# Luckick/EAGCN

Hardware: AMD Instinct MI355X
Metric: molecules/sec fwd+bwd, 2-layer 5-view EAGCN, Tox21 batch (higher is better)
Workload: dtype f32 (bf16x3 split, fp32 accumulate): every fp32 operand leaves its producer as three bf16 planes, six v_mfma_f32_32x32x16_bf16 piece products per 16 k rebuild the fp32 product (csrc/gemm_bx3.hip); aggregation, BatchNorm, head, first layer fp32

## Files before the change

### eagcn_amd/_lib.py

```python
import ctypes as C
import os

_HERE = os.path.dirname(os.path.abspath(__file__))
LIB_PATH = os.path.join(_HERE, 'lib', 'libeagcn_hip.so')

MAX_VIEWS = 8
MAX_SEGS = 8
META_WORDS = 16
META_NLOG = 8
META_T, META_NMAX, META_NTILES, META_BAD_ADJ, META_BAD_REL, META_NEDGE, META_OVERFLOW, META_EDGE_OVERFLOW = range(8)
META_NBLK = 9
STRUCT_CONCATE, STRUCT_WEIGHTED = 0, 1

_fp = C.c_void_p


class Batch(C.Structure):
    _fields_ = [('B', C.c_int32), ('N', C.c_int32), ('K', C.c_int32), ('ldc', C.c_int32),
                ('T', C.c_int32), ('n_max', C.c_int32), ('n_tiles', C.c_int32),
                ('channels', C.c_int32 * MAX_VIEWS),
                ('code', _fp), ('deg_bn', _fp), ('nat', _fp), ('row0', _fp), ('tile0', _fp),
                ('meta', _fp), ('row_mol', _fp), ('row_loc', _fp), ('row_m', _fp), ('row_deg', _fp),
                ('tile_mol', _fp), ('row_info', _fp), ('tile_info', _fp),
                ('rel_vec', _fp * MAX_VIEWS), ('rel_c', C.c_int32 * MAX_VIEWS),
# ... 63 lines not shown

class HeadParams(C.Structure):
    _fields_ = [('f_in', C.c_int32), ('n_den1', C.c_int32), ('n_den2', C.c_int32), ('nclass', C.c_int32),
                ('dropout', C.c_float), ('bn_eps', C.c_float), ('bn_momentum', C.c_float),
                ('den1_w', _fp), ('den2_w', _fp), ('den3_w', _fp),
                ('gbn_w', _fp), ('gbn_b', _fp), ('gbn_rm', _fp), ('gbn_rv', _fp),
                ('bn1_w', _fp), ('bn1_b', _fp), ('bn1_rm', _fp), ('bn1_rv', _fp),
                ('bn2_w', _fp), ('bn2_b', _fp), ('bn2_rm', _fp), ('bn2_rv', _fp)]


class HeadGrads(C.Structure):
    _fields_ = [(n, _fp) for n in ('d_den1_w', 'd_den2_w', 'd_den3_w', 'd_gbn_w', 'd_gbn_b', 'd_bn1_w', 'd_bn1_b',
                                   'd_bn2_w', 'd_bn2_b')]


class Model(C.Structure):
    _fields_ = [('n_layers', C.c_int32), ('molfp_mode', C.c_int32), ('training', C.c_int32),
                ('head_seed', C.c_uint64), ('head_seed_dev', _fp), ('input_packed', C.c_int32), ('aux_stream', _fp),
                ('layer', LayerParams * 4), ('head', HeadParams), ('stats_hook', _fp), ('stats_user', _fp),
                ('stats_world', C.c_int32), ('fuse_readout', C.c_int32), ('fwd_signal', _fp), ('wait_flag', _fp), ('start_signal', _fp)]


class StepLoss(C.Structure):
    _fields_ = [('kind', C.c_int32), ('labels', _fp), ('class_weight', _fp), ('loss', _fp), ('scale', _fp), ('dout', _fp)]


ALLREDUCE_FN = C.CFUNCTYPE(C.c_int, C.c_void_p, C.c_int, C.c_void_p, C.c_void_p)


SIGNATURES = {
    'eagcn_abi_version': (C.c_int, []),
    'eagcn_struct_size': (C.c_size_t, [C.c_int]),
    'eagcn_last_error': (C.c_char_p, []),
    'eagcn_pad16': (C.c_int, [C.c_int]),
    'eagcn_layer_out_ld': (C.c_int, [C.POINTER(LayerParams)]),
    'eagcn_layer_fp': (C.c_int, [C.POINTER(LayerParams)]),
    'eagcn_layer_packed_bytes': (C.c_size_t, [C.POINTER(Batch), C.POINTER(LayerParams)]),
    'eagcn_layer_fwd_scratch_bytes': (C.c_size_t, [C.POINTER(Batch), C.POINTER(LayerParams)]),
    'eagcn_layer_bwd_scratch_bytes': (C.c_size_t, [C.POINTER(Batch), C.POINTER(LayerParams)]),
    'eagcn_index_build': (C.c_int, [_fp, C.POINTER(_fp), C.POINTER(Batch), _fp, _fp]),
    'eagcn_index_from_bonds': (C.c_int, [_fp, _fp, _fp, _fp, C.c_int64, C.POINTER(Batch), _fp, _fp]),
    'eagcn_index_rows': (C.c_int, [C.POINTER(Batch), _fp]),
    'eagcn_set_gemm_mode': (C.c_int, [C.c_int]),
    'eagcn_stream_wait_counter': (C.c_int, [_fp, C.c_uint32, _fp]),
    'eagcn_stream_signal_flag': (C.c_int, [_fp, _fp]),
    'eagcn_stream_wait_flag': (C.c_int, [_fp, C.c_double, _fp]),
    'eagcn_stream_wait_timeouts': (C.c_int, []),
    'eagcn_stream_wait_reset': (None, []),
    'eagcn_adam_step': (C.c_int, [_fp, _fp, _fp, _fp, C.c_int64, _fp, _fp, _fp, _fp]),
    'eagcn_agg_wants_bond_lists': (C.c_int, [C.c_int, C.c_int]),
    'eagcn_agg_wants_bond_lists_for': (C.c_int, [C.c_int, C.c_int, C.c_int]),
    'eagcn_bx3_used_splits': (C.c_int, [C.c_int, C.c_int, C.c_int, C.c_int]),
    'eagcn_set_bx3_wide': (C.c_int, [C.c_int]),
    'eagcn_bx3_pair_used_splits': (C.c_int, [C.c_int] * 7),
    'eagcn_bx3_plane_elems': (C.c_size_t, [C.c_int, C.c_int]),
    'eagcn_bx3_split': (C.c_int, [_fp, C.c_int, C.c_int, _fp, C.c_size_t, C.c_int, C.c_int, _fp]),
    'eagcn_gemm_bx3': (C.c_int, [C.c_int, C.c_int, C.c_int, C.c_int, _fp, C.c_size_t, C.c_int, C.c_int, _fp, C.c_size_t, C.c_int, C.c_int,
                                 _fp, C.c_int, C.c_int, C.c_size_t, C.c_int, _fp]),
    'eagcn_gemm_bx3_pair': (C.c_int, [C.c_int, C.c_int, C.c_int, _fp, C.c_size_t, C.c_int, C.c_int, _fp, C.c_size_t, C.c_int, C.c_int, _fp, C.c_int,
                                      C.c_int, C.c_int, C.c_int, _fp, C.c_size_t, C.c_int, C.c_int, _fp, C.c_size_t, C.c_int, C.c_int, _fp, C.c_int,
                                      C.c_int, C.c_size_t, C.c_int, _fp]),
    'eagcn_pack_rows': (C.c_int, [C.POINTER(Batch), _fp, C.c_int, C.POINTER(Layout), _fp, _fp]),
    'eagcn_unpack_rows': (C.c_int, [C.POINTER(Batch), _fp, C.POINTER(Layout), _fp, _fp, C.c_int, _fp]),
    'eagcn_pad_rows': (C.c_int, [_fp, _fp, C.c_int, C.c_int, C.c_int, _fp, _fp]),
    'eagcn_gat_scratch_bytes': (C.c_size_t, [C.POINTER(Batch), C.c_int]),
    'eagcn_gat_forward': (C.c_int, [C.POINTER(Batch), C.POINTER(GatParams), _fp, _fp, _fp, _fp, _fp]),
    'eagcn_gat_backward': (C.c_int, [C.POINTER(Batch), C.POINTER(GatParams), _fp, _fp, _fp, _fp, _fp, _fp, _fp, _fp, _fp,
                                     C.c_size_t, _fp]),
    'eagcn_pool_scratch_bytes': (C.c_size_t, []),
    'eagcn_pool_attention_forward': (C.c_int, [C.POINTER(Batch), C.POINTER(PoolAtt), _fp, C.c_int, _fp, _fp, _fp]),
    'eagcn_pool_attention_backward': (C.c_int, [C.POINTER(Batch), C.POINTER(PoolAtt), _fp, C.c_int, _fp, _fp, _fp, C.c_size_t,
                                                _fp]),
    'eagcn_pool_mix_forward': (C.c_int, [C.POINTER(Batch), C.POINTER(Layout), _fp, C.c_int, _fp, _fp, _fp, _fp, C.c_int, _fp]),
    'eagcn_pool_mix_backward': (C.c_int, [C.POINTER(Batch), C.POINTER(Layout), _fp, C.c_int, _fp, _fp, _fp, _fp, C.c_int, _fp,
                                          _fp, _fp, _fp]),
    'eagcn_pool_reduce_forward': (C.c_int, [C.POINTER(Batch), _fp, C.c_int, C.c_int, C.c_int, _fp, _fp, _fp, _fp]),
    'eagcn_pool_reduce_backward': (C.c_int, [C.POINTER(Batch), _fp, C.c_int, C.c_int, C.c_int, _fp, _fp, _fp, _fp, _fp]),
    'eagcn_layer_forward': (C.c_int, [C.POINTER(Batch), C.POINTER(LayerParams), C.POINTER(LayerBufs), _fp]),
    'eagcn_layer_backward': (C.c_int, [C.POINTER(Batch), C.POINTER(LayerParams), C.POINTER(LayerBufs),
                                       _fp, _fp, _fp, C.POINTER(LayerGrads), _fp]),
    'eagcn_attention_dense': (C.c_int, [C.POINTER(Batch), C.POINTER(LayerParams), _fp, _fp]),
    'eagcn_readout_forward': (C.c_int, [C.POINTER(Batch), _fp, C.POINTER(Layout), _fp, _fp, C.c_int, _fp,
                                        C.c_int, _fp]),
    'eagcn_readout_backward': (C.c_int, [C.POINTER(Batch), _fp, C.POINTER(Layout), _fp, C.c_int, C.c_int,
                                         _fp, _fp, _fp]),
    'eagcn_gemm_f32': (C.c_int, [C.c_int, C.c_int, C.c_int, C.c_int, C.c_int, _fp, C.c_int, _fp, C.c_int,
                                 _fp, C.c_int, _fp]),
    'eagcn_gemm_f32_dev': (C.c_int, [C.c_int, C.c_int, C.c_int, C.c_int, C.c_int, _fp, C.c_int, _fp, C.c_int,
                                     _fp, C.c_int, _fp, C.c_int, _fp]),
    'eagcn_gemm_sk_workspace_bytes': (C.c_size_t, []),
    'eagcn_gemm_f32_sk': (C.c_int, [C.c_int, C.c_int, C.c_int, C.c_int, C.c_int, _fp, C.c_int, _fp, C.c_int,
                                    _fp, C.c_int, _fp, C.c_size_t, _fp]),
    'eagcn_gemm_pair_sk': (C.c_int, [C.c_int, C.c_int, C.c_int, _fp, C.c_int, _fp, C.c_int, _fp, C.c_int,
                                     C.c_int, C.c_int, C.c_int, _fp, C.c_int, _fp, C.c_int, _fp, C.c_int,
                                     _fp, C.c_size_t, _fp]),
    'eagcn_gemm_pair_sk_slabs': (C.c_int, [C.c_int, C.c_int, C.c_int, _fp, C.c_int, _fp, C.c_int, _fp, C.c_int,
                                           C.c_int, C.c_int, C.c_int, _fp, C.c_int, _fp, C.c_int, _fp, C.c_int,
                                           C.c_size_t, _fp, C.c_size_t, _fp]),
    'eagcn_gemm_sk_plan': (C.c_int, [C.c_int] * 7 + [C.POINTER(C.c_int), C.POINTER(C.c_int)]),
    'eagcn_gemm_sk_timeouts': (C.c_int, []),
    'eagcn_gemm_sk_failed': (C.c_int, []),
    'eagcn_gemm_sk_reset_failed': (None, []),
    'eagcn_gemm_sk_inject_failure': (None, []),
    'eagcn_model_saved_bytes': (C.c_size_t, [C.POINTER(Batch), C.POINTER(Model)]),
    'eagcn_model_scratch_bytes': (C.c_size_t, [C.POINTER(Batch), C.POINTER(Model)]),
    'eagcn_model_atom_rep': (C.c_int, [C.POINTER(Batch), C.POINTER(Model), C.POINTER(C.c_size_t),
# ... 95 lines not shown
```

### eagcn_amd/csrc/gemm.hip

```cpp
#include <stdlib.h>

#include <algorithm>

#include "common.h"
#include "gemm_x6.h"

namespace eagcn {

constexpr int gemm_lds_floats(int BM, int BN, int BK, bool a_kc, bool b_kc) {
    return 2 * ((a_kc ? BM * (BK + 2) : BK * (BM + 16)) + (b_kc ? BN * (BK + 2) : BK * (BN + 16)));
}

template <int BM, int BN, int BK, bool A_KC, bool B_KC, int D, bool EXT_LDS = false>
__device__ __forceinline__ void gemm_tile(const GemmDesc& g, const int Mx, const int Kx, const int tile_x,
                                          const int tile_y, const int z, const int nsp, float* shared = nullptr) {
    constexpr int WM = BM / 2, WN = BN / 2;
    constexpr int MR = WM / 16, NR = WN / 16;
    constexpr int LDA_S = A_KC ? (BK + 2) : (BM + 16);
    constexpr int LDB_S = B_KC ? (BK + 2) : (BN + 16);
    constexpr int A_SZ = A_KC ? BM * LDA_S : BK * LDA_S;
    constexpr int B_SZ = B_KC ? BN * LDB_S : BK * LDB_S;
    constexpr int A_TPR = A_KC ? BK / 4 : BM / 4;
    constexpr int A_RPP = 256 / A_TPR;
    constexpr int A_PASS = (A_KC ? BM : BK) / A_RPP;
    constexpr int B_TPR = B_KC ? BK / 4 : BN / 4;
    constexpr int B_RPP = 256 / B_TPR;
    constexpr int B_PASS = (B_KC ? BN : BK) / B_RPP;
    static_assert(A_PASS >= 1 && B_PASS >= 1, "tile too small for 256 threads");

    float* smem;
    if constexpr (EXT_LDS) {
        smem = shared;
    } else {
        __shared__ __attribute__((aligned(16))) float own_smem[2 * (A_SZ + B_SZ)];
        smem = own_smem;
    }
    auto kc_row = [](int x) -> int {
        if constexpr (BK == 16) {
            const int g = x >> 2, rs = x & 3;
            return ((g >> 2) << 4) + ((g & 3) << 1) + (rs & 1) + ((rs >> 1) << 3);
        } else {
            return x;
        }
    };
    auto As = [&](int buf) -> float* { return smem + buf * (A_SZ + B_SZ); };
    auto Bs = [&](int buf) -> float* { return smem + buf * (A_SZ + B_SZ) + A_SZ; };

    const int tid = threadIdx.x, lane = tid & 63, wave = tid >> 6;
    const int li = lane & 15, q = lane >> 4;
    const int wm = (wave >> 1) * WM, wn = (wave & 1) * WN;
    const int m0 = tile_y * BM, n0 = tile_x * BN;
    const int kchunk = ((Kx + nsp - 1) / nsp + BK - 1) / BK * BK;
    const int kbeg = z * kchunk;
    const int kend = min(Kx, kbeg + kchunk);
    float* C = g.C + (size_t)z * g.slab;

    float4 ra_[D][A_PASS], rb_[D][B_PASS];
    auto load_tiles = [&](int k0, float4 (&ra)[A_PASS], float4 (&rb)[B_PASS]) {
// ... 161 lines not shown
    {
        const int gx = gridDim.x;
        const int per_z = gx * ((Mx + BM - 1) / BM);
        const int nwg = per_z * nsp;
        if (blockIdx.y * gx + blockIdx.x >= per_z || (int)blockIdx.z >= nsp) return;
        const int lin = blockIdx.z * per_z + blockIdx.y * gx + blockIdx.x;
        const int nid = xcd_remap(lin, nwg);
        z = nid / per_z;
        const int rem = nid - z * per_z;
        tile_y = rem / gx;
        tile_x = rem - tile_y * gx;
    }
    if constexpr (X6 != 0) {
        constexpr int NP = X6 == 2 ? 1 : 3;
        __shared__ __attribute__((aligned(16))) unsigned char x6_smem[x6_lds_bytes(BM, BN, NP)];
        gemm_tile_x6<A_KC, B_KC, BM, BN, NP>(g, Mx, Kx, tile_x, tile_y, z, nsp, x6_smem);
    }
    else gemm_tile<BM, BN, BK, A_KC, B_KC, D>(g, Mx, Kx, tile_x, tile_y, z, nsp);
}

template <int BM, int BN, int BK, int D, int X6 = 0>
__global__ __launch_bounds__(256) void gemm_f32_pair_kernel(GemmDesc g0, GemmDesc g1, int first1) {
    constexpr int F32_LDS = gemm_lds_floats(BM, BN, BK, true, true) > gemm_lds_floats(BM, BN, BK, false, false)
                                ? gemm_lds_floats(BM, BN, BK, true, true) : gemm_lds_floats(BM, BN, BK, false, false);
    constexpr int NP = X6 == 2 ? 1 : 3;
    __shared__ __attribute__((aligned(16))) unsigned char x6_smem[X6 ? x6_lds_bytes(64, 64, NP) : F32_LDS * 4];
    float* f32_smem = reinterpret_cast<float*>(x6_smem);
    const int b = blockIdx.x;
    if (b < first1) {
        const int Mx = g0.M_dev ? min(*g0.M_dev, g0.M) : g0.M;
        const int gx = (g0.N + BN - 1) / BN;
        const int nreal = gx * ((Mx + BM - 1) / BM);
        if (b >= nreal) return;
        const int nid = xcd_remap(b, nreal);
        const int ty = nid / gx;
        if constexpr (X6 != 0) gemm_tile_x6<true, true, 64, 64, NP>(g0, Mx, g0.K, nid - ty * gx, ty, 0, 1, x6_smem);
        else gemm_tile<BM, BN, BK, true, true, D, true>(g0, Mx, g0.K, nid - ty * gx, ty, 0, 1, f32_smem);
    } else {
        const int lin = b - first1;
        const int Kx = g1.K_dev ? min(*g1.K_dev, g1.K) : g1.K;
        const int gx = (g1.N + BN - 1) / BN;
        const int per_z = gx * ((g1.M + BM - 1) / BM);
        const int nsp = eff_splits(g1, Kx);
        const int nwg = per_z * nsp;
        if (lin >= nwg) return;
        const int nid = xcd_remap(lin, nwg);
        const int z = nid / per_z, rem = nid - z * per_z;
        const int ty = rem / gx;
        if constexpr (X6 != 0) gemm_tile_x6<false, false, 64, 64, NP>(g1, g1.M, Kx, rem - ty * gx, ty, z, nsp, x6_smem);
        else gemm_tile<BM, BN, BK, false, false, D, true>(g1, g1.M, Kx, rem - ty * gx, ty, z, nsp, f32_smem);
    }
}


template <int BM, int BN, int BK, int D>
static int launch_cfg(const GemmDesc& g, hipStream_t s) {
    dim3 grid(cdiv(g.N, BN), cdiv(g.M, BM), g.splits);
    ProfScope ps(g.prof_tag, s, g.work > 0.0 ? g.work : 2.0 * g.M * g.N * g.K);
    if (g.ta == 0 && g.tb == 0) gemm_f32_kernel<BM, BN, BK, true, false, D><<<grid, 256, 0, s>>>(g);
    else if (g.ta == 0 && g.tb == 1) gemm_f32_kernel<BM, BN, BK, true, true, D><<<grid, 256, 0, s>>>(g);
    else if (g.ta == 1 && g.tb == 0) gemm_f32_kernel<BM, BN, BK, false, false, D><<<grid, 256, 0, s>>>(g);
    else gemm_f32_kernel<BM, BN, BK, false, true, D><<<grid, 256, 0, s>>>(g);
    EAGCN_LAUNCH_CHECK();
    return EAGCN_OK;
}

static int g_gemm_x6 = [] { const char* e = getenv("EAGCN_GEMM_X6"); return e ? atoi(e) : 3; }();
static int use_x6(const GemmDesc& g) { return ((g_gemm_x6 == 1 || g_gemm_x6 == 2) && g.K >= 64 && g.prof_tag != PROF_HEAD) ? g_gemm_x6 : 0; }
int gemm_mode() { return g_gemm_x6; }
template <int BM, int BN, int X6>
static int launch_x6_cfg(const GemmDesc& g, hipStream_t s) {
    dim3 grid(cdiv(g.N, BN), cdiv(g.M, BM), g.splits);
    ProfScope ps(g.prof_tag, s, g.work > 0.0 ? g.work : 2.0 * g.M * g.N * g.K);
    if (g.ta == 0 && g.tb == 0) gemm_f32_kernel<BM, BN, 16, true, false, 4, X6><<<grid, 256, 0, s>>>(g);
    else if (g.ta == 0 && g.tb == 1) gemm_f32_kernel<BM, BN, 16, true, true, 4, X6><<<grid, 256, 0, s>>>(g);
    else if (g.ta == 1 && g.tb == 0) gemm_f32_kernel<BM, BN, 16, false, false, 4, X6><<<grid, 256, 0, s>>>(g);
    else gemm_f32_kernel<BM, BN, 16, false, true, 4, X6><<<grid, 256, 0, s>>>(g);
    EAGCN_LAUNCH_CHECK();
    return EAGCN_OK;
}
static int launch_x6(const GemmDesc& g, hipStream_t s, int mode) {
    if (mode == 2) return launch_x6_cfg<64, 64, 2>(g, s);
    static const int tile = [] { const char* e = getenv("EAGCN_X6_TILE"); return e ? atoi(e) : 0; }();
    if (tile == 2 && g.M > 64 && g.N > 64) return launch_x6_cfg<128, 128, 1>(g, s);
    if (tile >= 1 && g.M > 64) return launch_x6_cfg<128, 64, 1>(g, s);
    return launch_x6_cfg<64, 64, 1>(g, s);
}

int launch_gemm(const GemmDesc& g0, hipStream_t s) {
    if (g0.M <= 0 || g0.N <= 0) return EAGCN_OK;
    EAGCN_CHECK_ARG(g0.splits >= 1, "gemm: splits must be >= 1");
    GemmDesc g = g0;
    g.vecA = (g.lda % 4) == 0 && ((g.ta ? g.M : g.K) % 4) == 0 && (reinterpret_cast<uintptr_t>(g.A) % 16) == 0;
    g.vecB = (g.ldb % 4) == 0 && ((g.tb ? g.K : g.N) % 4) == 0 && (reinterpret_cast<uintptr_t>(g.B) % 16) == 0;
    if (g.splits > 1) EAGCN_CHECK_ARG(g.vecA && g.vecB, "gemm: split-K needs float4-aligned operands");
    static const int forced = [] { const char* e = getenv("EAGCN_GEMM_CFG"); return e ? atoi(e) : -1; }();
    int cfg = forced;
    if (cfg < 0 && use_x6(g)) return launch_x6(g, s, use_x6(g));
    if (cfg < 0) {
        const long tiles128 = (long)cdiv(g.M, 128) * cdiv(g.N, 128) * g.splits;
        cfg = (g.K >= 1024 && tiles128 >= 512 && g.M > 64 && g.N > 64) ? 3 : 0;
    }
    switch (cfg) {
        case 1: return launch_cfg<64, 64, 32, 3>(g, s);
        case 2: return launch_cfg<64, 64, 16, 2>(g, s);
        case 3: return launch_cfg<128, 128, 16, 3>(g, s);
        case 4: return launch_cfg<64, 64, 16, 6>(g, s);
        case 5: return launch_cfg<64, 64, 16, 1>(g, s);
        default: return launch_cfg<64, 64, 16, 4>(g, s);
    }
}

int launch_gemm_pair(const GemmDesc& dx, const GemmDesc& dw, hipStream_t s) {
    GemmDesc g0 = dx, g1 = dw;
    g0.vecA = (g0.lda % 4) == 0 && (g0.K % 4) == 0 && (reinterpret_cast<uintptr_t>(g0.A) % 16) == 0;
    g0.vecB = (g0.ldb % 4) == 0 && (g0.K % 4) == 0 && (reinterpret_cast<uintptr_t>(g0.B) % 16) == 0;
    g1.vecA = (g1.lda % 4) == 0 && (g1.M % 4) == 0 && (reinterpret_cast<uintptr_t>(g1.A) % 16) == 0;
    g1.vecB = (g1.ldb % 4) == 0 && (g1.N % 4) == 0 && (reinterpret_cast<uintptr_t>(g1.B) % 16) == 0;
    const bool ok = g0.ta == 0 && g0.tb == 1 && g0.splits == 1 && !g0.K_dev && g1.ta == 1 && g1.tb == 0 && !g1.M_dev &&
                    (g1.splits == 1 || (g1.vecA && g1.vecB)) && g0.M > 0 && g0.N > 0 && g1.M > 0 && g1.N > 0;
    if (!ok) {
        int rc = launch_gemm(dw, s);
        return rc ? rc : launch_gemm(dx, s);
    }
    const int first1 = (cdiv(g0.M, 64) * cdiv(g0.N, 64) + 7) / 8 * 8;
    const int n1 = cdiv(g1.M, 64) * cdiv(g1.N, 64) * g1.splits;
    const double w0 = g0.work > 0.0 ? g0.work : 2.0 * g0.M * g0.N * g0.K;
    const double w1 = g1.work > 0.0 ? g1.work : 2.0 * g1.M * g1.N * g1.K;
    ProfScope ps(PROF_GEMM_PAIR, s, w0 + w1);
    if (use_x6(g0) == 2 && use_x6(g1) == 2) gemm_f32_pair_kernel<64, 64, 16, 4, 2><<<first1 + n1, 256, 0, s>>>(g0, g1, first1);
    else if (use_x6(g0) && use_x6(g1)) gemm_f32_pair_kernel<64, 64, 16, 4, 1><<<first1 + n1, 256, 0, s>>>(g0, g1, first1);
    else gemm_f32_pair_kernel<64, 64, 16, 4><<<first1 + n1, 256, 0, s>>>(g0, g1, first1);
    EAGCN_LAUNCH_CHECK();
    return EAGCN_OK;
}

}

using namespace eagcn;

extern "C" int eagcn_set_gemm_mode(int mode) {
    const int old = eagcn::g_gemm_x6;
    eagcn::g_gemm_x6 = mode;
    return old;
}

extern "C" int eagcn_gemm_f32(int ta, int tb, int M, int N, int K, const float* A, int lda, const float* B,
                              int ldb, float* C, int ldc, void* stream) {
    EAGCN_CHECK_ARG(A && B && C, "eagcn_gemm_f32: null operand");
    GemmDesc g{ta, tb, M, N, K, A, lda, B, ldb, C, ldc, 1, 0};
    return launch_gemm(g, (hipStream_t)stream);
}

extern "C" int eagcn_gemm_f32_dev(int ta, int tb, int M, int N, int K, const float* A, int lda, const float* B,
                                  int ldb, float* C, int ldc, const int32_t* extent_dev, int which, void* stream) {
    EAGCN_CHECK_ARG(A && B && C && extent_dev && (which == 0 || which == 2), "eagcn_gemm_f32_dev: bad argument");
    GemmDesc g{ta, tb, M, N, K, A, lda, B, ldb, C, ldc, 1, 0};
    if (which == 0) g.M_dev = extent_dev; else g.K_dev = extent_dev;
    return launch_gemm(g, (hipStream_t)stream);
}
```

### eagcn_amd/csrc/head.hip

```cpp
#include <stdlib.h>

#include <algorithm>

#include "common.h"
#include "kernels.h"

namespace eagcn {

__global__ void wait_counter_kernel(const uint32_t* __restrict__ word, uint32_t value, int* __restrict__ err,
                                    unsigned long long budget_ticks) {
    if (threadIdx.x == 0) {
        const unsigned long long t0 = wall_clock64();
        while ((int32_t)(__hip_atomic_load(word, __ATOMIC_ACQUIRE, __HIP_MEMORY_SCOPE_AGENT) - value) < 0) {
            __builtin_amdgcn_s_sleep(64);
            if (wall_clock64() - t0 > budget_ticks) {
                if (err) __hip_atomic_store(err, 1, __ATOMIC_RELAXED, __HIP_MEMORY_SCOPE_SYSTEM);
                break;
            }
        }
    }
}



// ... 66 lines not shown

static size_t carve_saved(void* base, const eagcn_batch* b, const eagcn_model* m, ModelSaved* out) {
    Carver2 c(base);
    ModelSaved s;
    const size_t T = (size_t)b->T;
    s.x0 = c.take<float>(T * layout_ld(&m->layer[0].in));
    for (int l = 0; l < m->n_layers; ++l) {
        const eagcn_layer_params* p = &m->layer[l];
        LayerSaved& L = s.L[l];
        L.fp = eagcn_layer_fp(p);
        L.ldo = eagcn_layer_out_ld(p);
        L.ld_in = layout_ld(&p->in);
        L.P = c.take<float>(T * L.fp);
        L.Y = c.take<float>(T * L.fp);
        L.rscale = c.take<float>((size_t)p->K * T);
        L.bn = c.take<float>((size_t)4 * L.fp);
        if (l == m->n_layers - 1) s.xout_last_off = c.off;
        L.xout = c.take<float>(T * L.ldo);
        if (l == m->n_layers - 1) s.pad_last_off = c.off;
        L.pad_row = c.take<float>(L.ldo);
        L.packed_bytes = eagcn_layer_packed_bytes(b, p);
        L.packed = c.take<char>(L.packed_bytes);
        const int np = (l + 1 < m->n_layers && L.ldo >= 128 && (L.ldo & 15) == 0) ? gemm_planes() : 0;
        L.xout_planes = np ? c.take<uint16_t>((size_t)np * bx_plane_elems(T, L.ldo)) : nullptr;
    }
    const eagcn_head_params* h = &m->head;
    const size_t B = (size_t)b->B;
    s.g = c.take<float>(B * h->f_in);
    s.h1 = c.take<float>(B * h->n_den1);
    s.h2 = c.take<float>(B * h->n_den2);
    s.bn_g = c.take<float>((size_t)4 * h->f_in);
    s.bn_1 = c.take<float>((size_t)4 * h->n_den1);
    s.bn_2 = c.take<float>((size_t)4 * h->n_den2);
    {
        const eagcn_layer_params* last = &m->layer[m->n_layers - 1];
        const size_t ldo = (size_t)eagcn_layer_out_ld(last);
        const bool need = last->structure == EAGCN_STRUCT_WEIGHTED;
        s.pad_cnt = c.take<uint16_t>(need ? B * last->K * ldo : 1);
        s.padc = c.take<float>(need ? B * ldo : 1);
        const size_t nt = (size_t)(b->N + 1) * (b->N + 1);
        s.pad_tab = c.take<uint32_t>(need ? nt : 1);
    }
    if (out) *out = s;
    return c.off;
}

struct ModelScratch {
    float *da2, *da1, *dgn, *dg, *dxa, *dxb, *dpad;
    float* hdw; int hdw_ks;
    double* hst; int n_hst;
    double* hws;
    double* hsb;
    void* layer; size_t layer_bytes;
};
static size_t carve_scratch(void* base, const eagcn_batch* b, const eagcn_model* m, ModelScratch* out) {
    Carver2 c(base);
    ModelScratch s;
    const eagcn_head_params* h = &m->head;
    const size_t B = (size_t)b->B, T = (size_t)b->T;
    s.n_hst = 2 * (h->f_in + h->n_den1 + h->n_den2) + 6;
    s.hst = c.take<double>((size_t)(HEAD_COPIES + 1) * s.n_hst + HEAD_WS);
    s.hsb = s.hst + (size_t)HEAD_COPIES * s.n_hst;
    s.hws = s.hsb + s.n_hst;
    s.da2 = c.take<float>(B * h->n_den2);
    s.da1 = c.take<float>(B * h->n_den1);
    s.dgn = c.take<float>(B * h->f_in);
    s.dg = c.take<float>(B * h->f_in);
    s.hdw_ks = head_dw_chunks(b->B);
    s.hdw = c.take<float>(s.hdw_ks > 1 ? (size_t)s.hdw_ks * ((size_t)h->f_in * h->n_den1 + (size_t)h->n_den1 * h->n_den2 +
                                                             (size_t)h->n_den2 * h->nclass) : 1);
    int ldmax = 0;
    size_t lbytes = 0;
    for (int l = 0; l < m->n_layers; ++l) {
        ldmax = std::max(ldmax, eagcn_layer_out_ld(&m->layer[l]));
        lbytes = std::max(lbytes, eagcn_layer_fwd_scratch_bytes(b, &m->layer[l]));
        lbytes = std::max(lbytes, eagcn_layer_bwd_scratch_bytes(b, &m->layer[l]));
    }
    s.dxa = c.take<float>(T * ldmax);
    s.dxb = c.take<float>(T * ldmax);
    s.dpad = c.take<float>((size_t)EAGCN_MAX_VIEWS * ldmax);
    s.layer_bytes = lbytes;
    s.layer = c.take<char>(lbytes);
    if (out) *out = s;
    return c.off;
}

static int check_model(const eagcn_batch* b, const eagcn_model* m, const char* who) {
    EAGCN_CHECK_ARG(b && m, "%s: null argument", who);
    EAGCN_CHECK_ARG(m->n_layers >= 1 && m->n_layers <= 4, "%s: n_layers=%d", who, m->n_layers);
    const eagcn_head_params* h = &m->head;
    EAGCN_CHECK_ARG(h->f_in >= 1 && h->n_den1 >= 1 && h->n_den2 >= 1 && h->nclass >= 1, "%s: bad head sizes", who);
    EAGCN_CHECK_ARG(h->den1_w && h->den2_w && h->den3_w && h->gbn_w && h->gbn_b && h->gbn_rm && h->gbn_rv &&
                        h->bn1_w && h->bn1_b && h->bn1_rm && h->bn1_rv && h->bn2_w && h->bn2_b && h->bn2_rm &&
                        h->bn2_rv, "%s: null head parameter", who);
    const eagcn_layer_params* last = &m->layer[m->n_layers - 1];
    const int f_last = last->structure == EAGCN_STRUCT_CONCATE ? [&] { int s = 0; for (int k = 0; k < last->K; ++k) s += last->width[k]; return s; }()
                                                                 : last->width[0];
    EAGCN_CHECK_ARG(f_last == h->f_in, "%s: head expects %d features, last layer yields %d", who, h->f_in, f_last);
    EAGCN_CHECK_ARG(!m->training || b->B > 1, "%s: BatchNorm in training mode needs more than one molecule", who);
    return EAGCN_OK;
}

static eagcn_layout out_layout(const eagcn_layer_params* p) {
    eagcn_layout l;
    memset(&l, 0, sizeof(l));
    if (p->structure == EAGCN_STRUCT_CONCATE) {
        l.nseg = p->K;
        for (int k = 0; k < p->K; ++k) { l.width[k] = p->width[k]; l.pad[k] = pad16(p->width[k]); }
    } else {
        l.nseg = 1;
        l.width[0] = p->width[0];
        l.pad[0] = pad16(p->width[0]);
    }
    return l;
}

static bool fused_readout(const eagcn_model* m) {
    static const bool env = [] { const char* v = getenv("EAGCN_NO_FUSED_READOUT"); return !(v && v[0] == '1'); }();
    return env && m->fuse_readout && m->layer[m->n_layers - 1].structure == EAGCN_STRUCT_CONCATE;
}

static bool hidden_planes_only(const eagcn_batch* b, const eagcn_model* m, const ModelSaved& sv, int l) {
    return l + 1 < m->n_layers && sv.L[l].xout_planes && layer_reads_planes_only(b, &m->layer[l + 1], m->aux_stream != nullptr);
}

static void fill_drop(float p, int training, int* do_drop, uint32_t* thr, float* inv_keep) {
    *do_drop = (training && p > 0.0f) ? 1 : 0;
    *thr = (uint32_t)std::min(4294967295.0, (double)p * 4294967296.0);
    *inv_keep = 1.0f / (1.0f - p);
}

}

using namespace eagcn;

// ... 74 lines not shown
    if (!hg) return P;
    const double *cn_g = sc.hst + 2 * F, *cn_1 = sc.hst + 2 * F + 2 + 2 * n1, *cn_2 = sc.hst + 2 * (F + n1) + 4 + 2 * n2;
    const float gscale = P.sync && m->stats_world > 1 ? 1.0f / (float)m->stats_world : 1.0f;
    P.b3 = HeadBwd{B, n2, nc, sv.h2, sv.bn_2, 1, nodrop, h->den3_w, dout, nullptr, nullptr, nullptr, nullptr, nullptr, nullptr,
                   sc.da2, P.sb_2, hg->d_den3_w, m->training};
    P.b2 = HeadBwd{B, n1, n2, sv.h1, sv.bn_1, 1, drop1, h->den2_w, sc.da2, sv.h2, sv.bn_2, P.sb_2, dgraph_rep, hg->d_bn2_w, hg->d_bn2_b,
                   sc.da1, P.sb_1, hg->d_den2_w, m->training};
    P.b1 = HeadBwd{B, F, n1, sv.g, sv.bn_g, 0, nodrop, h->den1_w, sc.da1, sv.h1, sv.bn_1, P.sb_1, nullptr, hg->d_bn1_w, hg->d_bn1_b,
                   sc.dgn, P.sb_g, hg->d_den1_w, m->training};
    if (P.sync) { P.b2.cnt_y = cn_2; P.b2.gscale = gscale; P.b1.cnt_y = cn_1; P.b1.gscale = gscale; }
    P.b3.nw = 8;
    const int ks = sc.hdw_ks;
    float* part3 = sc.hdw;
    float* part2 = part3 + (size_t)ks * n2 * nc;
    float* part1 = part2 + (size_t)ks * n1 * n2;
    if (ks > 1) {
        P.b3.ks = ks; P.b3.dW_part = part3;
        P.b2.ks = ks; P.b2.dW_part = part2;
        P.b1.ks = ks; P.b1.dW_part = part1;
    }
    P.bg = HeadGbn{B, F, sc.dgn, sv.g, sv.bn_g, P.sb_g, sc.dg, hg->d_gbn_w, hg->d_gbn_b, m->training};
    if (P.sync) { P.bg.cnt = cn_g; P.bg.gscale = gscale; }
    if (ks > 1) {
        P.bg.sum[0] = HeadDwSum{hg->d_den3_w, part3, n2 * nc, ks};
        P.bg.sum[1] = HeadDwSum{hg->d_den2_w, part2, n1 * n2, ks};
        P.bg.sum[2] = HeadDwSum{hg->d_den1_w, part1, F * n1, ks};
        P.bg.nsum = 3;
    }
    return P;
}

static int model_forward_trunk(const eagcn_batch* b, const eagcn_model* m, const float* afm, const int64_t* size, void* saved,
                               size_t saved_bytes, void* scratch, size_t scratch_bytes, ModelSaved& sv, ModelScratch& sc,
                               void* stream, const char* who) {
    hipStream_t s = (hipStream_t)stream;
    RC(check_model(b, m, who));
    EAGCN_CHECK_GEMM3(who);
    EAGCN_CHECK_ARG((afm || m->input_packed) && saved && scratch, "%s: null buffer", who);
    EAGCN_CHECK_ARG(m->molfp_mode == 0 || size, "%s: 'ave' read-out needs size", who);
    EAGCN_CHECK_ARG(carve_saved(saved, b, m, &sv) <= saved_bytes, "%s: saved block too small", who);
    EAGCN_CHECK_ARG(carve_scratch(scratch, b, m, &sc) <= scratch_bytes, "%s: scratch too small", who);
    const eagcn_head_params* h = &m->head;
    HandOff ho{m->start_signal, m->wait_flag, wait_err_word(), 200000000ull};
    if (!m->input_packed && (m->wait_flag || m->start_signal)) {
        handoff_kernel<<<1, 64, 0, s>>>(ho);
        EAGCN_LAUNCH_CHECK();
        ho.start = nullptr; ho.flag = nullptr;
    }
    ZeroJob zj;
    RC(gemm3_zero_job(sc.layer, sc.layer_bytes, sc.hst, (HEAD_COPIES + 1) * sc.n_hst + HEAD_WS, &zj));
    if (!m->input_packed)
        RC(eagcn_pack_rows(b, afm, layout_width(&m->layer[0].in), &m->layer[0].in, sv.x0, stream));
    const float* x = sv.x0;
    {
        const eagcn_layer_params* ps[4];
        void* pk[4];
        size_t pkb[4];
        for (int l = 0; l < m->n_layers; ++l) { ps[l] = &m->layer[l]; pk[l] = sv.L[l].packed; pkb[l] = sv.L[l].packed_bytes; }
        RC(pack_params_all(b, ps, pk, pkb, m->n_layers, stream, &zj, &ho));
    }
    for (int l = 0; l < m->n_layers; ++l) {
        LayerSaved& L = sv.L[l];
        eagcn_layer_bufs w;
        memset(&w, 0, sizeof(w));
        w.x = x; w.P = L.P; w.Y = L.Y; w.rscale = L.rscale; w.bn = L.bn; w.xout = L.xout; w.pad_row = L.pad_row;
        w.scratch = sc.layer; w.scratch_bytes = sc.layer_bytes; w.packed = L.packed; w.packed_bytes = L.packed_bytes;
        w.stats_hook = m->stats_hook; w.stats_user = m->stats_user;
        w.x_planes = l > 0 ? sv.L[l - 1].xout_planes : nullptr; w.xout_planes = L.xout_planes;
        const bool po = hidden_planes_only(b, m, sv, l);
        RC(layer_forward_impl(b, &m->layer[l], &w, stream, true, l == m->n_layers - 1 && fused_readout(m), po));
        x = po ? nullptr : L.xout;
    }
    const eagcn_layer_params* last = &m->layer[m->n_layers - 1];
    const LayerSaved& LL = sv.L[m->n_layers - 1];
    const eagcn_layout lay = out_layout(last);
    const int B = b->B, F = h->f_in, n1 = h->n_den1, n2 = h->n_den2;
    double *st_g = sc.hst, *st_1 = sc.hst + 2 * F + 2, *st_2 = sc.hst + 2 * (F + n1) + 4;
    const int copies = (m->stats_hook && m->training) ? 1 : HEAD_COPIES;
    if (fused_readout(m)) {
        ReadoutBn rb;
        rb.Y = LL.Y; rb.ldy = LL.fp; rb.bn = LL.bn; rb.fp = LL.fp;
        fill_drop(last->dropout, last->training, &rb.do_drop, &rb.thr, &rb.inv_keep);
        rb.seed = last->seed; rb.seed_dev = last->seed_dev;
        rb.size = size; rb.mode = m->molfp_mode; rb.g = sv.g; rb.F = F; rb.st = st_g;
        rb.cnt0 = st_g + 2 * F; rb.cnt1 = st_1 + 2 * n1; rb.cnt2 = st_2 + 2 * n2;
        rb.st_copies = copies; rb.st_stride = sc.n_hst;
        RC(readout_bn_forward(b, &lay, rb, stream));
    } else if (pad_sampled(m))
        RC(readout_forward_sampled(b, LL.xout, &lay, last, LL.bn + (size_t)LL.fp , size,
                                   m->molfp_mode, sv.g, F, sv.pad_cnt, sv.padc, sv.pad_tab, stream));
    else
        RC(eagcn_readout_forward(b, LL.xout, &lay, last->structure == EAGCN_STRUCT_WEIGHTED ? LL.pad_row : nullptr,
                                 size, m->molfp_mode, sv.g, F, stream));
    if (!fused_readout(m)) RC(head_colstats(sv.g, B, F, st_g, s, st_g + 2 * F, st_1 + 2 * n1, st_2 + 2 * n2));
    return EAGCN_OK;
}

static int stats_hook_call(const eagcn_model* m, bool sync, double* buf, int n, void* stream) {
    if (!sync) return EAGCN_OK;
    if (m->stats_hook(buf, n, stream, m->stats_user)) {
        set_error("eagcn_model: the sync-BatchNorm all-reduce hook failed");
        return EAGCN_ERR_HIP;
    }
    return EAGCN_OK;
}

static int head_forward_launches(const eagcn_model* m, const HeadPlan& P, void* stream) {
    hipStream_t s = (hipStream_t)stream;
    const eagcn_head_params* h = &m->head;
    RC(stats_hook_call(m, P.sync, P.st_g, 2 * h->f_in + 1, stream));
    RC(head_fwd(P.f1, s));
    RC(stats_hook_call(m, P.sync, P.st_1, 2 * h->n_den1 + 1, stream));
    RC(head_fwd(P.f2, s));
    RC(stats_hook_call(m, P.sync, P.st_2, 2 * h->n_den2 + 1, stream));
    RC(head_fwd(P.f3, s));
    return EAGCN_OK;
}
static int head_backward_launches(const eagcn_model* m, const HeadPlan& P, void* stream) {
    hipStream_t s = (hipStream_t)stream;
    const eagcn_head_params* h = &m->head;
    RC(head_bwd(P.b3, s));
    RC(stats_hook_call(m, P.sync, P.sb_2, 2 * h->n_den2, stream));
    RC(head_bwd(P.b2, s));
// ... 173 lines not shown
        else RC(eagcn_mse_loss(out, loss->labels, b->B * h->nclass, loss->loss, loss->dout, stream));
        if (loss->scale) {
            const int n = b->B * h->nclass;
            scale_loss_kernel<<<cdiv(n, 256), 256, 0, s>>>(loss->loss, loss->dout, n, loss->scale);
            EAGCN_LAUNCH_CHECK();
        }
        RC(head_backward_launches(m, P, stream));
    }
    return readout_pad_backward(b, m, size, sv, sc, stream);
}

extern "C" int eagcn_model_backward(const eagcn_batch* b, const eagcn_model* m, const int64_t* size, void* saved,
                                    size_t saved_bytes, void* scratch, size_t scratch_bytes, const float* dout,
                                    const float* dgraph_rep, const eagcn_layer_grads* lg,
                                    const eagcn_head_grads* hg, void* stream) {
    EAGCN_CHECK_ARG(m, "eagcn_model_backward: null model");
    return eagcn_model_backward_range(b, m, size, saved, saved_bytes, scratch, scratch_bytes, dout, dgraph_rep, lg, hg, 1,
                                      m->n_layers - 1, 0, stream);
}

static int model_backward_impl(const eagcn_batch* b, const eagcn_model* m, const int64_t* size, void* saved, size_t saved_bytes,
                               void* scratch, size_t scratch_bytes, const float* dout, const float* dgraph_rep,
                               const eagcn_layer_grads* lg, const eagcn_head_grads* hg, int with_head, int layer_hi, int layer_lo,
                               float* dx0, bool input_only, void* stream) {
    hipStream_t s = (hipStream_t)stream;
    EAGCN_CHECK_ARG(saved && scratch && dout && (lg || input_only) && hg, "eagcn_model_backward: null buffer");
    EAGCN_CHECK_ARG(hg->d_den1_w && hg->d_den2_w && hg->d_den3_w && hg->d_gbn_w && hg->d_gbn_b && hg->d_bn1_w &&
                        hg->d_bn1_b && hg->d_bn2_w && hg->d_bn2_b, "eagcn_model_backward: null head gradient");
    EAGCN_CHECK_ARG(layer_hi < m->n_layers && layer_lo >= 0 && layer_lo <= layer_hi + 1,
                    "eagcn_model_backward_range: layers %d..%d of %d", layer_hi, layer_lo, m->n_layers);
    EAGCN_CHECK_ARG(!with_head || layer_hi == m->n_layers - 1 || layer_hi < layer_lo,
                    "eagcn_model_backward_range: the head's backward is followed by the top layer");
    ModelSaved sv;
    ModelScratch sc;
    EAGCN_CHECK_ARG(carve_saved(saved, b, m, &sv) <= saved_bytes, "eagcn_model_backward: saved block too small");
    EAGCN_CHECK_ARG(carve_scratch(scratch, b, m, &sc) <= scratch_bytes, "eagcn_model_backward: scratch too small");
    const int F = m->head.f_in;
    const ZeroJob zb{nullptr, 0, sc.hsb, sc.n_hst};
    hipStream_t side = m->aux_stream ? (hipStream_t)m->aux_stream : s;
    const bool forked = side != s;
    const eagcn_layer_params* last = &m->layer[m->n_layers - 1];
    const eagcn_layout lay = out_layout(last);
    const bool weighted = last->structure == EAGCN_STRUCT_WEIGHTED;
    const bool sampled = pad_sampled(m);
    if (with_head) {
        const HeadPlan P = head_plan(b, m, sv, sc, nullptr, nullptr, dout, dgraph_rep, hg);
        RC(head_backward_launches(m, P, stream));
        if (!(input_only && !m->training)) RC(readout_pad_backward(b, m, size, sv, sc, stream));
    }
    ReadoutGrad rgd;
    memset(&rgd, 0, sizeof(rgd));
    rgd.dg = sc.dg; rgd.F = F; rgd.size = size; rgd.mode = m->molfp_mode; rgd.map = make_colmap(&lay);
    const int top_l = m->n_layers - 1;
    EdgeDrain pend_in, pend_out;
    pend_in.eacc = nullptr;
    pend_out.eacc = nullptr;
    for (int l = layer_hi; l >= layer_lo; --l) {
        const int t = top_l - l;
        float* cur = (t & 1) ? sc.dxb : sc.dxa;
        float* other = (t & 1) ? sc.dxa : sc.dxb;
        LayerSaved& L = sv.L[l];
        eagcn_layer_bufs w;
        memset(&w, 0, sizeof(w));
        w.x = l == 0 ? sv.x0 : (hidden_planes_only(b, m, sv, l - 1) ? nullptr : sv.L[l - 1].xout);
        w.P = L.P; w.Y = L.Y; w.rscale = L.rscale; w.bn = L.bn; w.xout = L.xout; w.pad_row = L.pad_row;
        w.scratch = sc.layer; w.scratch_bytes = sc.layer_bytes; w.packed = L.packed; w.packed_bytes = L.packed_bytes;
        w.aux_stream = m->aux_stream;
        w.stats_hook = m->stats_hook; w.stats_user = m->stats_user;
        w.x_planes = l > 0 ? sv.L[l - 1].xout_planes : nullptr;
        const bool top = l == top_l;
        const float* dpad = (weighted && top) ? sc.dpad : nullptr;
        RC(layer_backward_impl(b, &m->layer[l], &w, top ? nullptr : cur, top ? &rgd : nullptr, dpad,
                               l > 0 ? other : dx0, input_only ? nullptr : &lg[l], stream, top && sampled, top ? &zb : nullptr,
                               pend_in.eacc ? &pend_in : nullptr, (l > layer_lo && !input_only) ? &pend_out : nullptr, input_only));
        pend_in = pend_out;
        if (l == layer_lo) pend_in.eacc = nullptr;
    }
    if (forked) RC(stream_after(s, side));
    return EAGCN_OK;
}

extern "C" int eagcn_model_backward_range(const eagcn_batch* b, const eagcn_model* m, const int64_t* size, void* saved,
                                          size_t saved_bytes, void* scratch, size_t scratch_bytes, const float* dout,
                                          const float* dgraph_rep, const eagcn_layer_grads* lg,
                                          const eagcn_head_grads* hg, int with_head, int layer_hi, int layer_lo, void* stream) {
    RC(check_model(b, m, "eagcn_model_backward"));
    EAGCN_CHECK_GEMM3("eagcn_model_backward");
    return model_backward_impl(b, m, size, saved, saved_bytes, scratch, scratch_bytes, dout, dgraph_rep, lg, hg, with_head, layer_hi,
                               layer_lo, nullptr, false, stream);
}

struct InputScratch { float* dx0; eagcn_head_grads hg; };
static size_t carve_input_scratch(void* base, const eagcn_batch* b, const eagcn_model* m, InputScratch* out) {
    Carver2 c(base);
    c.off = carve_scratch(nullptr, b, m, nullptr);
    InputScratch t;
    const eagcn_head_params* h = &m->head;
    const size_t F = h->f_in, n1 = h->n_den1, n2 = h->n_den2, nc = h->nclass;
    t.dx0 = c.take<float>((size_t)std::max(b->T, 1) * layout_ld(&m->layer[0].in));
    t.hg.d_den1_w = c.take<float>(F * n1);
    t.hg.d_den2_w = c.take<float>(n1 * n2);
    t.hg.d_den3_w = c.take<float>(n2 * nc);
    t.hg.d_gbn_w = c.take<float>(F);
    t.hg.d_gbn_b = c.take<float>(F);
    t.hg.d_bn1_w = c.take<float>(n1);
    t.hg.d_bn1_b = c.take<float>(n1);
    t.hg.d_bn2_w = c.take<float>(n2);
    t.hg.d_bn2_b = c.take<float>(n2);
    if (out) *out = t;
    return c.off;
}

static int check_engine_model(const eagcn_batch* b, const eagcn_model* m, const char* who) {
    RC(check_model(b, m, who));
    EAGCN_CHECK_ARG(m->molfp_mode == 0 || m->molfp_mode == 1, "%s: read-out mode %d has no engine path", who, m->molfp_mode);
    for (int l = 0; l < m->n_layers; ++l)
        EAGCN_CHECK_ARG(m->layer[l].structure == EAGCN_STRUCT_CONCATE || m->layer[l].structure == EAGCN_STRUCT_WEIGHTED,
                        "%s: layer %d has structure %d, which the engine does not run", who, l, m->layer[l].structure);
    return EAGCN_OK;
}

int eagcn::model_backward_input_packed(const eagcn_batch* b, const eagcn_model* m, const int64_t* size, void* saved, size_t saved_bytes,
                                       void* scratch, size_t scratch_bytes, const float* dout, const float* dgraph_rep,
                                       const eagcn_layer_grads* lg, const eagcn_head_grads* hg, float** dx0, void* stream,
                                       const char* who) {
    EAGCN_CHECK_ARG(b && m, "%s: null argument", who);
    EAGCN_CHECK_ARG((lg == nullptr) == (hg == nullptr), "%s: lg and hg are both given (full backward) or both NULL (input-only)", who);
// ... 57 lines not shown
```

### eagcn_amd/csrc/index.hip

```cpp
#include <algorithm>

#include <stdlib.h>

#include "common.h"
#include "kernels.h"

namespace eagcn {

struct RelPtrs {
    const float* p[EAGCN_MAX_VIEWS];
    int c[EAGCN_MAX_VIEWS];
};

template <int NIT, int RPW>
__global__ __launch_bounds__(256) void index_scan_kernel(const float* __restrict__ adj, RelPtrs rel,
                                                          int B, int N, int Ncap, int K, int ldc,
                                                          uint8_t* __restrict__ code,
                                                          int32_t* __restrict__ deg_bn,
                                                          int32_t* __restrict__ nat,
                                                          int32_t* __restrict__ ecnt,
                                                          int32_t* __restrict__ meta) {
    const int lane = threadIdx.x & 63;
    const long row_first = ((long)blockIdx.x * 4 + (threadIdx.x >> 6)) * RPW;
    const long nrows = (long)B * N;
// ... 566 lines not shown
            __syncthreads();
        }
        int run = s_scan[tid] - tot;
        __syncthreads();
#pragma unroll
        for (int u = 0; u < 4; ++u) {
            const int i = tid * 4 + u;
            if (i < n) {
                int* ptr = (pass ? bt.col_ptr : bt.row_ptr) + (size_t)(r0 + i) * 2;
                const bool fits = e0 + run + v[u] <= bt.E;
                ptr[0] = e0 + run;
                ptr[1] = fits ? v[u] : 0;
                cnt[i] = fits ? e0 + run : -1;
                run += v[u];
            }
        }
        __syncthreads();
    }
    auto codes = [&](int i, int j) -> uint64_t {
        uint8_t c[EAGCN_MAX_VIEWS];
#pragma unroll
        for (int k = 0; k < EAGCN_MAX_VIEWS; ++k) c[k] = k < bt.K ? code0[k * plane + (size_t)i * bt.ldc + j] : 0;
        uint64_t c64 = 0;
#pragma unroll
        for (int k = 0; k < EAGCN_MAX_VIEWS; ++k) c64 |= (uint64_t)c[k] << (8 * k);
        return c64;
    };
    for (int i = tid; i < n; i += 256) {
        int e = s_cnt[i];
        int ec = s_ccnt[i];
        if constexpr (BITMAP) {
            if (s_live[i] && e >= 0)
                for (int w = 0; w < Wn; ++w) {
                    uint32_t m = bits[i * W + w];
                    while (m) { const int j = 32 * w + __ffs(m) - 1; m &= m - 1u; bt.nbr[e] = j; bt.ecode[e] = codes(i, j); ++e; }
                }
            if (ec >= 0)
                for (int w = 0; w < Wn; ++w) {
                    uint32_t m = bitsT[i * W + w];
                    while (m) { const int ii = 32 * w + __ffs(m) - 1; m &= m - 1u; bt.tnbr[ec] = ii; bt.tcode[ec] = codes(ii, i); ++ec; }
                }
        } else {
            if (s_live[i] && e >= 0)
                for (int j = 0; j < n; ++j)
                    if (bond(i, j)) { bt.nbr[e] = j; bt.ecode[e] = codes(i, j); ++e; }
            if (ec >= 0)
                for (int ii = 0; ii < n; ++ii)
                    if (bond(ii, i)) { bt.tnbr[ec] = ii; bt.tcode[ec] = codes(ii, i); ++ec; }
        }
    }
}

typedef ColMapD ColMap;
__device__ __forceinline__ int packed_to_exact(const ColMap& m, int cp) {
    int eo = 0, po = 0;
    for (int s = 0; s < m.nseg; ++s) {
        if (cp < po + m.p[s]) return (cp - po < m.w[s]) ? eo + (cp - po) : -1;
        eo += m.w[s];
        po += m.p[s];
    }
    return -1;
}

__global__ __launch_bounds__(256) void pack_rows_kernel(eagcn_batch bt, const float* __restrict__ dense,
                                                         int F, ColMap m, int ld, float* __restrict__ packed, int Nin) {
    const uint32_t total = (uint32_t)dev_rows(bt) * (uint32_t)ld;
    for (uint32_t e = blockIdx.x * blockDim.x + threadIdx.x; e < total; e += gridDim.x * blockDim.x) {
        int r = (int)(e / (uint32_t)ld), cp = (int)(e - (uint32_t)r * (uint32_t)ld);
        int ce = packed_to_exact(m, cp);
        float v = 0.0f;
        if (ce >= 0) v = dense[((size_t)bt.row_mol[r] * Nin + bt.row_loc[r]) * F + ce];
        packed[e] = v;
    }
}

__global__ __launch_bounds__(256) void pad_rows_kernel(const float* __restrict__ rows, const int32_t* __restrict__ off,
                                                        int B, int N, int F, float* __restrict__ out) {
    const size_t total = (size_t)B * N * F;
    for (size_t e = (size_t)blockIdx.x * blockDim.x + threadIdx.x; e < total; e += (size_t)gridDim.x * blockDim.x) {
        const int f = (int)(e % F);
        const size_t bi = e / F;
        const int i = (int)(bi % N), b = (int)(bi / N);
        const int o = off[b], n = off[b + 1] - o;
        out[e] = i < n ? rows[(size_t)(o + i) * F + f] : 0.0f;
    }
}

__global__ __launch_bounds__(256) void unpack_rows_kernel(eagcn_batch bt, const float* __restrict__ packed,
                                                           ColMap m, int ld, const float* __restrict__ pad_row,
                                                           float* __restrict__ dense, int F) {
    const size_t total = (size_t)bt.B * bt.N * F;
    for (size_t e = (size_t)blockIdx.x * blockDim.x + threadIdx.x; e < total;
         e += (size_t)gridDim.x * blockDim.x) {
        int ce = (int)(e % F);
        size_t bi = e / F;
        int i = (int)(bi % bt.N), b = (int)(bi / bt.N);
        int eo = 0, po = 0, cp = -1;
        for (int s = 0; s < m.nseg; ++s) {
            if (ce < eo + m.w[s]) { cp = po + (ce - eo); break; }
            eo += m.w[s];
            po += m.p[s];
        }
        float v;
        if (i < bt.nat[b]) v = packed[(size_t)(bt.row0[b] + i) * ld + cp];
        else v = pad_row ? pad_row[cp] : 0.0f;
        dense[e] = v;
    }
}

}

using namespace eagcn;

extern "C" int eagcn_index_build(const float* adj, const float* const* rel, eagcn_batch* b,
                                 int32_t* host_meta, void* stream) {
// ... 168 lines not shown
```

### eagcn_amd/csrc/kernels.h

```cpp
#pragma once
#include "bx3.h"
#include "common.h"

namespace eagcn {

struct AggArgs {
    eagcn_batch bt;
    ViewCols vc;
    const float* src; int lds;
    float* dst; int ldd;
    const float* sig;
    const float* rsig;
    float* rscale;
    double* stats;
    int nchunk;
    int cpw = 1;
    int xcd = 0;
    bool w_rowm = false;
    BxOut planes = {nullptr, 0, 0, 0};
    const float* bn_tab = nullptr; const float* bn_cc = nullptr; int bn_fp = 0;
    const float* w_aw = nullptr;
    int w_drop = 0; uint32_t w_thr = 0; float w_inv_keep = 1.0f; uint64_t w_seed = 0; const uint64_t* w_seed_dev = nullptr;
};
int agg_grid_x(const eagcn_batch* b);
// ... 122 lines not shown
        __hip_atomic_store(h.flag, 0u, __ATOMIC_RELAXED, __HIP_MEMORY_SCOPE_AGENT);
    }
}
int gemm3_zero_job(void* workspace, size_t bytes, double* zero, int nzero, ZeroJob* out);
int zero_fill(void* p, size_t bytes, hipStream_t s);
bool gemm3_ok(const GemmDesc& g);
int launch_gemm3(const GemmDesc& g, const DwScatter* sc, void* workspace, size_t bytes, hipStream_t s);
int launch_gemm3_pair(const GemmDesc& dx, const GemmDesc& dw, const DwScatter* sc, void* workspace, size_t bytes, hipStream_t s,
                      size_t xk_slab = 0);

constexpr int HEAD_COPIES = 8;
struct HeadDrop { int on; uint32_t thr; float inv_keep; uint64_t seed; const uint64_t* seed_dev; };
struct HeadFwd {
    int B, K, N;
    const float* x; const double* st_in; const float *gamma, *beta; float *run_mean, *run_var; float* bn;
    const float* W; float* y; float* y2; double* st_out;
    int training, relu; float eps, momentum; HeadDrop drop;
    const double* cnt_in = nullptr;
    int st_copies = 1, st_stride = 0;
    const float* lab = nullptr; int nlab = 0; unsigned* lab_cnt = nullptr;
    int nw = 0;
    uint32_t* signal = nullptr;
};
struct HeadBwd {
    int B, K, N;
    const float* x; const float* bnp; int relu_p; HeadDrop drop; const float* W;
    const float* dy; const float* y; const float* bny; const double* sb_y; const float* extra;
    float *dgamma_y, *dbeta_y; float* dyp; double* sb_p; float* dW; int training;
    const double* cnt_y = nullptr;
    float gscale = 1.0f;
    int ks = 1; float* dW_part = nullptr;
    int nw = 0;
};
inline int head_dw_chunks(int B) { return B > 256 ? (B + 255) / 256 < 16 ? (B + 255) / 256 : 16 : 1; }
struct HeadDwSum { float* dst; const float* part; int n, ks; };
struct HeadGbn { int B, F; const float *dgn, *g, *bn; const double* sb; float *dg, *dgamma, *dbeta; int training;
                 const double* cnt = nullptr; float gscale = 1.0f;
                 HeadDwSum sum[3] = {}; int nsum = 0; };
struct HeadLoss { int kind;
                  const float* labels; const float* weight; float* loss; const float* scale; float* dout; };
struct HeadMid { HeadFwd f3; HeadBwd b3; HeadLoss L;
                 double* ws; };
constexpr int HEAD_WS = 4;
struct HeadLossFin { float* loss; const double* ws; const float* scale; int kind, n; };
bool head_mid_ok(int n_den2, int nclass);
int head_mid(const HeadMid& a, hipStream_t s);
int head_bwd_pair(const HeadBwd& a, const HeadBwd& e, const HeadLossFin& lf, hipStream_t s);
int head_colstats(const float* g, int B, int F, double* st, hipStream_t s, double* cnt0 = nullptr, double* cnt1 = nullptr,
                  double* cnt2 = nullptr);
int head_fwd(const HeadFwd& a, hipStream_t s);
int head_bwd(const HeadBwd& a, hipStream_t s);
int head_gbn_bwd(const HeadGbn& a, hipStream_t s);

struct EdgeDrain {
    double* eacc; int K;
    float* datt_w[EAGCN_MAX_VIEWS]; float* dself_r[EAGCN_MAX_VIEWS]; int channels[EAGCN_MAX_VIEWS];
    const float* rsig;
};
int layer_backward_impl(const eagcn_batch* b, const eagcn_layer_params* p, const eagcn_layer_bufs* w,
                        const float* dxout, const ReadoutGrad* rg, const float* dpad_row, float* dx,
                        const eagcn_layer_grads* g, void* stream, bool dpad_views = false,
                        const ZeroJob* zero_after = nullptr, const EdgeDrain* drain_in = nullptr, EdgeDrain* drain_out = nullptr,
                        bool input_only = false);
int model_backward_input_packed(const eagcn_batch* b, const eagcn_model* m, const int64_t* size, void* saved, size_t saved_bytes,
                                void* scratch, size_t scratch_bytes, const float* dout, const float* dgraph_rep,
                                const eagcn_layer_grads* lg, const eagcn_head_grads* hg, float** dx0, void* stream, const char* who);
int launch_attr_dense(const eagcn_batch* b, const eagcn_layout* in, const float* acc, const float* x, const float* base, float* attr,
                      float* score, hipStream_t s);
int model_input_slot(const eagcn_batch* b, const eagcn_model* m, void* saved, size_t saved_bytes, float** x0, const char* who);
int layer_forward_impl(const eagcn_batch* b, const eagcn_layer_params* p, const eagcn_layer_bufs* w, void* stream,
                       bool prepacked, bool skip_apply = false, bool planes_only = false);
bool layer_reads_planes_only(const eagcn_batch* b, const eagcn_layer_params* p, bool aux_stream);
int layer_apply_impl(const eagcn_batch* b, const eagcn_layer_params* p, const eagcn_layer_bufs* w, void* stream);
int pack_params_all(const eagcn_batch* b, const eagcn_layer_params* const* ps, void* const* packed,
                    const size_t* packed_bytes, int n, void* stream, const ZeroJob* zj = nullptr, const HandOff* ho = nullptr);
struct ReadoutBn {
    const float* Y; int ldy;
    const float* bn; int fp;
    int do_drop; uint32_t thr; float inv_keep; uint64_t seed; const uint64_t* seed_dev;
    const int64_t* size; int mode;
    float* g; int F;
    double* st;
    int st_copies = 1, st_stride = 0;
    bool pair = false;
    double *cnt0, *cnt1, *cnt2;
};
int readout_bn_forward(const eagcn_batch* b, const eagcn_layout* lay, const ReadoutBn& a, void* stream);
int readout_forward_sampled(const eagcn_batch* b, const float* x, const eagcn_layout* lay, const eagcn_layer_params* p,
                            const float* bn_sh, const int64_t* size, int mode, float* g, int F, uint16_t* cnt, float* padc,
                            uint32_t* tab, void* stream);
int readout_backward_pad_views(const eagcn_batch* b, const float* dg, const eagcn_layout* lay, const int64_t* size, int mode,
                               int F, int K, const uint16_t* cnt, float dropout, float* dpad, void* stream);
int readout_backward_pad(const eagcn_batch* b, const float* dg, const eagcn_layout* lay, const int64_t* size,
                         int mode, int F, float* dpad_row, void* stream);

}
```

### eagcn_amd/csrc/layer.hip

```cpp
#include <algorithm>

#include <stdlib.h>

#include "common.h"
#include "kernels.h"

namespace eagcn {

struct ParamPtrs {
    const float* att_w[EAGCN_MAX_VIEWS];
    const float* self_r[EAGCN_MAX_VIEWS];
    const float* W[EAGCN_MAX_VIEWS];
    const float* bias[EAGCN_MAX_VIEWS];
    const float* gamma[EAGCN_MAX_VIEWS];
    const float* beta[EAGCN_MAX_VIEWS];
    float* run_mean[EAGCN_MAX_VIEWS];
    float* run_var[EAGCN_MAX_VIEWS];
    const float* ave_w;
    int channels[EAGCN_MAX_VIEWS];
    const float* rel_vec[EAGCN_MAX_VIEWS];
    int rel_c[EAGCN_MAX_VIEWS];
};
__device__ __forceinline__ float att_logit(const ParamPtrs& pp, int k, int c) {
    if (!pp.rel_vec[k]) return pp.att_w[k][c - 1];
    const float* v = pp.rel_vec[k] + (size_t)(c - 1) * pp.rel_c[k];
    float s = 0.0f;
    for (int ch = 0; ch < pp.rel_c[k]; ++ch) s = fmaf(pp.att_w[k][ch], v[ch], s);
    return s;
}
struct GradPtrs {
    float* dW[EAGCN_MAX_VIEWS];
    float* dbias[EAGCN_MAX_VIEWS];
    float* dgamma[EAGCN_MAX_VIEWS];
    float* dbeta[EAGCN_MAX_VIEWS];
    float* datt_w[EAGCN_MAX_VIEWS];
    float* dself_r[EAGCN_MAX_VIEWS];
    float* dave_w;
};

enum { CP_GAMMA = 0, CP_BETA, CP_BIAS, CP_RMEAN, CP_RVAR, CP_AVEW, CP_ROWS = 8 };

__device__ __forceinline__ int col_view(const ViewCols& vc, int cp) {
    int k = 0;
#pragma unroll
    for (int v = 1; v < EAGCN_MAX_VIEWS; ++v) k += (v < vc.K && cp >= vc.off[v]) ? 1 : 0;
    return k;
}
__device__ __forceinline__ int packed_to_exact(const ColMapD& m, int cp) {
    int eo = 0, po = 0;
    for (int s = 0; s < m.nseg; ++s) {
        if (cp < po + m.p[s]) return (cp - po < m.w[s]) ? eo + (cp - po) : -1;
        eo += m.w[s];
        po += m.p[s];
    }
    return -1;
}

__device__ __forceinline__ void pack_params_body(const ParamPtrs& pp, const ViewCols& vc, const ColMapD& in, int ld_in,
                                                 int fp, float* __restrict__ Wcat, float* __restrict__ WcatT,
                                                 float* __restrict__ colp, float* __restrict__ sig, float* __restrict__ rsig,
                                                 const BxOut wp = BxOut{nullptr, 0, 0, 0}, const BxOut wtp = BxOut{nullptr, 0, 0, 0}) {
    __shared__ float tile[32][33];
    const int tx = threadIdx.x & 31, ty = threadIdx.x >> 5;
    const int ntx = (fp + 31) >> 5, nty = (ld_in + 31) >> 5;
    for (int t = blockIdx.x; t < ntx * nty; t += gridDim.x) {
        const int ip0 = (t / ntx) << 5, cp0 = (t % ntx) << 5;
        {
            const int cp = cp0 + tx;
            const int k = cp < fp ? col_view(vc, cp) : 0;
            const int f = cp - vc.off[k];
#pragma unroll
            for (int j = 0; j < 4; ++j) {
                const int ip = ip0 + ty + 8 * j;
                float v = 0.0f;
                if (ip < ld_in && cp < fp) {
                    const int fi = packed_to_exact(in, ip);
                    if (fi >= 0 && f < vc.width[k]) v = pp.W[k][(size_t)fi * vc.width[k] + f];
                    Wcat[(size_t)ip * fp + cp] = v;
                }
                tile[ty + 8 * j][tx] = v;
            }
        }
        __syncthreads();
#pragma unroll
        for (int j = 0; j < 4; ++j) {
            const int cp = cp0 + ty + 8 * j, ip = ip0 + tx;
            if (cp < fp && ip < ld_in) WcatT[(size_t)cp * ld_in + ip] = tile[tx][ty + 8 * j];
        }
        if (wp.p) {
            const int r = threadIdx.x >> 3, c4 = (threadIdx.x & 7) << 2;
            if (ip0 + r < ld_in && cp0 + c4 < fp)
                bx_store4(wp, ip0 + r, cp0 + c4, make_float4(tile[r][c4], tile[r][c4 + 1], tile[r][c4 + 2], tile[r][c4 + 3]));
            if (cp0 + r < fp && ip0 + c4 < ld_in)
                bx_store4(wtp, cp0 + r, ip0 + c4, make_float4(tile[c4][r], tile[c4 + 1][r], tile[c4 + 2][r], tile[c4 + 3][r]));
        }
        __syncthreads();
    }
    for (int cp = blockIdx.x * blockDim.x + threadIdx.x; cp < fp; cp += gridDim.x * blockDim.x) {
        const int k = col_view(vc, cp), f = cp - vc.off[k];
        const bool ok = f < vc.width[k];
        colp[CP_GAMMA * fp + cp] = ok ? pp.gamma[k][f] : 0.0f;
        colp[CP_BETA * fp + cp] = ok ? pp.beta[k][f] : 0.0f;
        colp[CP_BIAS * fp + cp] = ok ? pp.bias[k][f] : 0.0f;
        colp[CP_RMEAN * fp + cp] = ok ? pp.run_mean[k][f] : 0.0f;
        colp[CP_RVAR * fp + cp] = ok ? pp.run_var[k][f] : 1.0f;
        colp[CP_AVEW * fp + cp] = pp.ave_w ? pp.ave_w[k] : 1.0f;
    }
    for (int e = blockIdx.x * blockDim.x + threadIdx.x; e < vc.K * 256; e += gridDim.x * blockDim.x) {
        const int k = e >> 8, c = e & 255;
        sig[e] = (c >= 1 && c <= pp.channels[k]) ? sigmoidf_(att_logit(pp, k, c)) : 0.0f;
    }
    if (blockIdx.x == 0 && threadIdx.x < vc.K) rsig[threadIdx.x] = sigmoidf_(pp.self_r[threadIdx.x][0]);
}
__global__ __launch_bounds__(256) void pack_params_kernel(ParamPtrs pp, ViewCols vc, ColMapD in, int ld_in, int fp,
                                                           float* __restrict__ Wcat, float* __restrict__ WcatT,
                                                           float* __restrict__ colp, float* __restrict__ sig,
                                                           float* __restrict__ rsig, BxOut wp, BxOut wtp) {
    pack_params_body(pp, vc, in, ld_in, fp, Wcat, WcatT, colp, sig, rsig, wp, wtp);
}
struct PackJob {
    ParamPtrs pp; ViewCols vc; ColMapD in; int ld_in, fp;
    float *Wcat, *WcatT, *colp, *sig, *rsig;
    BxOut wp, wtp;
};
struct PackJobs { PackJob j0, j1, j2, j3; };
__global__ __launch_bounds__(256) void pack_params_multi_kernel(PackJobs jobs, ZeroJob zj, HandOff ho) {
    if (blockIdx.y == 0) {
        for (int i = blockIdx.x * blockDim.x + threadIdx.x; i < max(zj.nu, zj.nd); i += gridDim.x * blockDim.x) {
            if (i < zj.nu) zj.u[i] = 0u;
            if (i < zj.nd) zj.d[i] = 0.0;
        }
    }
    if (blockIdx.y == 0) pack_params_body(jobs.j0.pp, jobs.j0.vc, jobs.j0.in, jobs.j0.ld_in, jobs.j0.fp, jobs.j0.Wcat, jobs.j0.WcatT, jobs.j0.colp, jobs.j0.sig, jobs.j0.rsig, jobs.j0.wp, jobs.j0.wtp);
    else if (blockIdx.y == 1) pack_params_body(jobs.j1.pp, jobs.j1.vc, jobs.j1.in, jobs.j1.ld_in, jobs.j1.fp, jobs.j1.Wcat, jobs.j1.WcatT, jobs.j1.colp, jobs.j1.sig, jobs.j1.rsig, jobs.j1.wp, jobs.j1.wtp);
    else if (blockIdx.y == 2) pack_params_body(jobs.j2.pp, jobs.j2.vc, jobs.j2.in, jobs.j2.ld_in, jobs.j2.fp, jobs.j2.Wcat, jobs.j2.WcatT, jobs.j2.colp, jobs.j2.sig, jobs.j2.rsig, jobs.j2.wp, jobs.j2.wtp);
    else pack_params_body(jobs.j3.pp, jobs.j3.vc, jobs.j3.in, jobs.j3.ld_in, jobs.j3.fp, jobs.j3.Wcat, jobs.j3.WcatT, jobs.j3.colp, jobs.j3.sig, jobs.j3.rsig, jobs.j3.wp, jobs.j3.wtp);
    if (blockIdx.x == 0 && blockIdx.y == 0 && threadIdx.x == 0) handoff_body(ho);
}

template <int L>
__device__ __forceinline__ void slab_sum(const double* __restrict__ slab, int nslab, int fp, int cp, int sl,
                                           double& s1, double& s2) {
    s1 = 0.0;
    s2 = 0.0;
    for (int s0 = sl; s0 < nslab; s0 += L * 8) {
        double2 v[8];
#pragma unroll
        for (int u = 0; u < 8; ++u) {
            const int s = s0 + L * u;
            v[u] = s < nslab ? *reinterpret_cast<const double2*>(slab + ((size_t)s * fp + cp) * 2) : make_double2(0.0, 0.0);
        }
#pragma unroll
        for (int u = 0; u < 8; ++u) { s1 += v[u].x; s2 += v[u].y; }
    }
#pragma unroll
    for (int o = L / 2; o > 0; o >>= 1) {
        s1 += __shfl_xor(s1, o);
        s2 += __shfl_xor(s2, o);
    }
}

constexpr int BWD_ROWS = 7;
template <int L>
__global__ __launch_bounds__(256) void bn_stats_sum_kernel(const double* __restrict__ slab, int nslab, int fp, double M,
                                                            double* __restrict__ out, const int32_t* __restrict__ meta,
                                                            int mode, int tiles_per_wg, int nvirt, int batch_B) {
    if (meta[EAGCN_META_NLOG] > 0) M = (double)batch_B * (double)meta[EAGCN_META_NLOG];
    if (mode == 1 && tiles_per_wg > 0) nslab = min(nslab, (meta[EAGCN_META_NTILES] + tiles_per_wg - 1) / tiles_per_wg);
    if (mode == 1 && tiles_per_wg < 0) nslab = min(nslab, meta[EAGCN_META_NBLK]);
    if (mode == 2) nslab = max(1, min(nslab, (meta[EAGCN_META_T] + nvirt + BWD_ROWS - 1) / BWD_ROWS));
    const int cpr = blockIdx.x * (256 / L) + threadIdx.x / L, sl = threadIdx.x % L;
    const int cp = min(cpr, fp - 1);
    double s1, s2;
    slab_sum<L>(slab, nslab, fp, cp, sl, s1, s2);
    if (cpr < fp && sl == 0) { out[2 * cp] = s1; out[2 * cp + 1] = s2; }
    if (blockIdx.x == 0 && threadIdx.x == 0) out[2 * fp] = M;
}

template <int L>
__global__ __launch_bounds__(256) void bn_finalize_kernel(const double* __restrict__ slab, int nslab, int fp,
                                                           double M, int training, float eps, float momentum,
                                                           const float* __restrict__ colp, ParamPtrs pp,
                                                           ViewCols vc, float* __restrict__ bn,
                                                           const int32_t* __restrict__ meta, int tiles_per_wg, int batch_B,
                                                           const double* __restrict__ M_dev) {
    if (meta[EAGCN_META_NLOG] > 0) M = (double)batch_B * (double)meta[EAGCN_META_NLOG];
    if (M_dev) M = *M_dev;
    if (tiles_per_wg > 0) nslab = min(nslab, (meta[EAGCN_META_NTILES] + tiles_per_wg - 1) / tiles_per_wg);
    if (tiles_per_wg < 0) nslab = min(nslab, meta[EAGCN_META_NBLK]);
// ... 96 lines not shown
                r = (int)(rg * 8u + ((e >> 3) & 7u)); f = (int)((it - rg * g4) * 32u + (e & 7u) * 4u);
                if (r >= T || f >= a.ldo) continue;
            } else {
                r = (int)(e / g4); f = (int)(e - (uint32_t)r * g4) * 4;
            }
            float4 y[EAGCN_MAX_VIEWS];
#pragma unroll
            for (int k = 0; k < EAGCN_MAX_VIEWS; ++k)
                if (k < a.vc.K) y[k] = *reinterpret_cast<const float4*>(a.Y + (size_t)r * a.ldy + a.vc.off[k] + f);
            float4 acc = {0.0f, 0.0f, 0.0f, 0.0f};
#pragma unroll
            for (int k = 0; k < EAGCN_MAX_VIEWS; ++k)
                if (k < a.vc.K) {
                    const int cp = a.vc.off[k] + f;
                    const float4 sc = *reinterpret_cast<const float4*>(a.bn + BN_SC * fp + cp);
                    const float4 sh = *reinterpret_cast<const float4*>(a.bn + BN_SH * fp + cp);
                    const float4 w = *reinterpret_cast<const float4*>(a.colp + CP_AVEW * fp + cp);
                    float4 p;
                    p.x = fmaxf(y[k].x * sc.x + sh.x, 0.0f);
                    p.y = fmaxf(y[k].y * sc.y + sh.y, 0.0f);
                    p.z = fmaxf(y[k].z * sc.z + sh.z, 0.0f);
                    p.w = fmaxf(y[k].w * sc.w + sh.w, 0.0f);
                    if (a.do_drop) {
                        float ds[4];
                        drop_scale4(seed, (uint64_t)r * fp + cp, a.thr, a.inv_keep, ds);
                        p.x *= ds[0]; p.y *= ds[1]; p.z *= ds[2]; p.w *= ds[3];
                    }
                    acc.x += w.x * p.x; acc.y += w.y * p.y; acc.z += w.z * p.z; acc.w += w.w * p.w;
                }
            if (a.out) *reinterpret_cast<float4*>(a.out + (size_t)r * a.ldo + f) = acc;
            if (a.planes.p) bx_store4(a.planes, r, f, acc);
        }
    }
}

struct BwdArgs {
    const int32_t* meta; int Tcap;
    const int32_t* row_mol;
    const float* row_m;
    ViewCols vc;
    int structure, fp, nvirt;
    const float* dxout; int ldo;
    ReadoutGrad rg;
    const float* dpad;
    int dpad_views;
    const float* Y; int ldy;
    const float* bn;
    const float* colp;
    float* dH;
    double* slab;
    double* slab_da;
    int do_drop; uint32_t thr; float inv_keep; uint64_t seed; const uint64_t* seed_dev;
    double* zero; int nzero;
    EdgeDrain drain;
    const float* cc;
    int store_dh;
};

template <bool WEIGHTED, bool DG, bool DROP, bool APPLY>
__global__ __launch_bounds__(256) void bn_bwd_reduce_kernel(BwdArgs a) {
    __shared__ double da_s[EAGCN_MAX_VIEWS];
    const uint64_t seed = DROP ? (a.seed_dev ? *a.seed_dev : a.seed) : 0ull;
    const int fp = a.fp, T = min(a.meta[EAGCN_META_T], a.Tcap);
    const int rows = T + (APPLY ? 0 : a.nvirt);
    const int nwg = max(1, min((int)gridDim.x, (rows + BWD_ROWS - 1) / BWD_ROWS));
    if (!APPLY && a.drain.eacc && blockIdx.x == 0 && blockIdx.y == 0) {
        const int K = a.drain.K;
        for (int e = threadIdx.x; e < K * EDGE_SLAB; e += blockDim.x) {
            const int k = e / EDGE_SLAB, c = e - k * EDGE_SLAB;
            if (c > 256) continue;
            double v[EDGE_COPIES];
#pragma unroll
            for (int z = 0; z < EDGE_COPIES; ++z) v[z] = a.drain.eacc[((size_t)z * K + k) * EDGE_SLAB + c];
            double t = 0.0;
#pragma unroll
            for (int z = 0; z < EDGE_COPIES; ++z) { t += v[z]; a.drain.eacc[((size_t)z * K + k) * EDGE_SLAB + c] = 0.0; }
            float* dw = nullptr;
            float* dr = nullptr;
            int ch = 0;
#pragma unroll
            for (int q = 0; q < EAGCN_MAX_VIEWS; ++q)
                if (q == k) { dw = a.drain.datt_w[q]; dr = a.drain.dself_r[q]; ch = a.drain.channels[q]; }
            if (c == 256) {
                const double r = (double)a.drain.rsig[k];
                dr[0] = (float)(t * r * (1.0 - r));
            } else if (c >= 1 && c <= ch) {
                dw[c - 1] = (float)t;
            }
        }
    }
    if ((int)blockIdx.x >= nwg || (APPLY && T == 0)) return;
    if constexpr (!APPLY) {
        if (threadIdx.x < EAGCN_MAX_VIEWS) da_s[threadIdx.x] = 0.0;
        __syncthreads();
    }
    constexpr bool weighted = WEIGHTED;
    double da[EAGCN_MAX_VIEWS];
#pragma unroll
    for (int k = 0; k < EAGCN_MAX_VIEWS; ++k) da[k] = 0.0;
    const int c_lo = blockIdx.y * (int)blockDim.x * 4;
    for (int cp = c_lo + threadIdx.x * 4; cp < min(fp, c_lo + (int)blockDim.x * 4); cp += blockDim.x * 4) {
        const int k = col_view(a.vc, cp), f = cp - a.vc.off[k];
        const float4 sc = *reinterpret_cast<const float4*>(a.bn + BN_SC * fp + cp);
        const float4 sh = *reinterpret_cast<const float4*>(a.bn + BN_SH * fp + cp);
        const float4 mu = *reinterpret_cast<const float4*>(a.bn + BN_MU * fp + cp);
        const float4 iv = *reinterpret_cast<const float4*>(a.bn + BN_INV * fp + cp);
        const float4 aw = *reinterpret_cast<const float4*>(a.colp + CP_AVEW * fp + cp);
        float4 c1 = make_float4(0.f, 0.f, 0.f, 0.f), c2 = c1;
        if constexpr (APPLY) {
            c1 = *reinterpret_cast<const float4*>(a.cc + cp);
            c2 = *reinterpret_cast<const float4*>(a.cc + fp + cp);
        }
        const int cu = weighted ? f : cp;
        auto exact = [&](int c) {
            int eo = 0, po = 0, res = -1;
            bool done = false;
#pragma unroll
            for (int sg = 0; sg < EAGCN_MAX_SEGS; ++sg) {
                if (sg < a.rg.map.nseg && !done) {
                    if (c < po + a.rg.map.p[sg]) { res = (c - po < a.rg.map.w[sg]) ? eo + (c - po) : -1; done = true; }
                    eo += a.rg.map.w[sg];
                    po += a.rg.map.p[sg];
                }
            }
            return res;
        };
        int ce0 = -1, ce1 = -1, ce2 = -1, ce3 = -1;
        bool ce4 = false;
        if constexpr (DG) {
            ce0 = exact(cu); ce1 = exact(cu + 1); ce2 = exact(cu + 2); ce3 = exact(cu + 3);
            ce4 = ce0 >= 0 && ce3 == ce0 + 3 && (ce0 & 3) == 0 && (a.rg.F & 3) == 0 &&
                  (reinterpret_cast<uintptr_t>(a.rg.dg) & 15) == 0;
        }
        double s1[4] = {0.0, 0.0, 0.0, 0.0}, s2[4] = {0.0, 0.0, 0.0, 0.0}, dak = 0.0;
        for (int rb = blockIdx.x; rb < rows; rb += BWD_ROWS * nwg) {
            float4 yv[BWD_ROWS], upv[BWD_ROWS];
#pragma unroll
            for (int u = 0; u < BWD_ROWS; ++u) {
                const int r = rb + u * nwg;
                yv[u] = make_float4(0.f, 0.f, 0.f, 0.f);
                upv[u] = make_float4(0.f, 0.f, 0.f, 0.f);
// ... 26 lines not shown
                } else if (r < rows) {
                    upv[u] = *reinterpret_cast<const float4*>(a.dpad + (size_t)(a.dpad_views ? k : (r - T)) * a.ldo + cu);
                }
            }
#pragma unroll
            for (int u = 0; u < BWD_ROWS; ++u) {
                const int r = rb + u * nwg;
                if (r >= rows) continue;
                const float yy[4] = {yv[u].x, yv[u].y, yv[u].z, yv[u].w};
                const float uu[4] = {upv[u].x, upv[u].y, upv[u].z, upv[u].w};
                const float scv[4] = {sc.x, sc.y, sc.z, sc.w}, shv[4] = {sh.x, sh.y, sh.z, sh.w};
                const float muv[4] = {mu.x, mu.y, mu.z, mu.w}, ivv[4] = {iv.x, iv.y, iv.z, iv.w};
                const float awv[4] = {aw.x, aw.y, aw.z, aw.w};
                const float c1v[4] = {c1.x, c1.y, c1.z, c1.w}, c2v[4] = {c2.x, c2.y, c2.z, c2.w};
                float dh[4], dsv[4] = {1.0f, 1.0f, 1.0f, 1.0f};
                if (DROP && r < T) drop_scale4(seed, (uint64_t)r * fp + cp, a.thr, a.inv_keep, dsv);
#pragma unroll
                for (int j = 0; j < 4; ++j) {
                    float up = uu[j];
                    const float ds = dsv[j];
                    const float h = yy[j] * scv[j] + shv[j];
                    if (weighted) { if constexpr (!APPLY) dak += (double)(up * ds * fmaxf(h, 0.0f)); up *= awv[j]; }
                    dh[j] = h > 0.0f ? up * ds : 0.0f;
                    const float xh = (yy[j] - muv[j]) * ivv[j];
                    if constexpr (APPLY) {
                        dh[j] = scv[j] * (dh[j] - c1v[j] - xh * c2v[j]);
                    } else {
                        s1[j] += (double)dh[j];
                        s2[j] += (double)(dh[j] * xh);
                    }
                }
                if ((APPLY || a.store_dh) && r < T)
                    *reinterpret_cast<float4*>(a.dH + (size_t)r * fp + cp) = make_float4(dh[0], dh[1], dh[2], dh[3]);
            }
        }
        if constexpr (!APPLY) {
            double* sl = a.slab + ((size_t)blockIdx.x * fp + cp) * 2;
            *reinterpret_cast<double4*>(sl) = make_double4(s1[0], s2[0], s1[1], s2[1]);
            *reinterpret_cast<double4*>(sl + 4) = make_double4(s1[2], s2[2], s1[3], s2[3]);
            if (weighted) {
#pragma unroll
                for (int v = 0; v < EAGCN_MAX_VIEWS; ++v) da[v] += (v == k) ? dak : 0.0;
            }
        }
    }
    if (weighted && !APPLY) {
#pragma unroll
        for (int v = 0; v < EAGCN_MAX_VIEWS; ++v) {
            const double t = wave_sum(da[v]);
            if ((threadIdx.x & 63) == 0 && t != 0.0) atomicAdd(&da_s[v], t);
        }
        __syncthreads();
        if (threadIdx.x < EAGCN_MAX_VIEWS)
            a.slab_da[((size_t)blockIdx.y * gridDim.x + blockIdx.x) * EAGCN_MAX_VIEWS + threadIdx.x] = da_s[threadIdx.x];
    }
}

template <int L>
__global__ __launch_bounds__(256) void bn_bwd_finalize_kernel(const double* __restrict__ slab,
                                                               const double* __restrict__ slab_da, int nslab,
                                                               int fp, double M, int training,
                                                               const float* __restrict__ bn, ViewCols vc,
                                                               GradPtrs gp, float* __restrict__ cc, const int32_t* __restrict__ meta, int nvirt,
                                                               int batch_B, int da_chunks, int da_stride,
                                                               const double* __restrict__ gsum, double* __restrict__ zero, int nzero) {
    if (blockIdx.x == 0 && zero)
        for (int i = threadIdx.x; i < nzero; i += blockDim.x) zero[i] = 0.0;
    if (meta[EAGCN_META_NLOG] > 0) M = (double)batch_B * (double)meta[EAGCN_META_NLOG];
    nslab = max(1, min(nslab, (meta[EAGCN_META_T] + nvirt + BWD_ROWS - 1) / BWD_ROWS));
    const int cpr = blockIdx.x * (256 / L) + threadIdx.x / L, sl = threadIdx.x % L;
    const int cp = min(cpr, fp - 1);
    if (blockIdx.x == 0 && gp.dave_w) {
        const int v = threadIdx.x >> 5, l = threadIdx.x & 31;
        double t = 0.0;
        if (v < vc.K)
            for (int y = 0; y < da_chunks; ++y)
                for (int s = l; s < nslab; s += 32) t += slab_da[((size_t)y * da_stride + s) * EAGCN_MAX_VIEWS + v];
#pragma unroll
        for (int o = 16; o > 0; o >>= 1) t += __shfl_xor(t, o);
        if (v < vc.K && l == 0) gp.dave_w[v] = (float)t;
    }
    double s1, s2;
    slab_sum<L>(slab, nslab, fp, cp, sl, s1, s2);
    if (cpr >= fp || sl != 0) return;
    {
        double g1 = s1, g2 = s2;
        if (gsum) { g1 = gsum[2 * cp]; g2 = gsum[2 * cp + 1]; M = gsum[2 * fp]; }
        cc[cp] = training ? (float)(g1 / M) : 0.0f;
        cc[fp + cp] = training ? (float)(g2 / M) : 0.0f;
    }
    const int k = col_view(vc, cp), f = cp - vc.off[k];
    if (f < vc.width[k]) {
        gp.dgamma[k][f] = (float)s2;
        gp.dbeta[k][f] = (float)s1;
        gp.dbias[k][f] = training ? 0.0f : (float)((double)bn[BN_SC * fp + cp] * s1);
    }
}

__global__ __launch_bounds__(256) void bn_bwd_apply_kernel(eagcn_batch bt, int fp, const float* __restrict__ Y, int ldy,
                                                            const float* __restrict__ bn,
                                                            const float* __restrict__ cc, float* __restrict__ dH) {
    const uint32_t g4 = fp / 4;
    const uint32_t total = (uint32_t)dev_rows(bt) * g4;
    for (uint32_t e = blockIdx.x * blockDim.x + threadIdx.x; e < total; e += gridDim.x * blockDim.x) {
        const int r = (int)(e / g4), c = (int)(e - (uint32_t)r * g4) * 4;
        const float4 y = *reinterpret_cast<const float4*>(Y + (size_t)r * ldy + c);
        float4 d = *reinterpret_cast<float4*>(dH + (size_t)r * fp + c);
        const float4 sc = *reinterpret_cast<const float4*>(bn + BN_SC * fp + c);
        const float4 mu = *reinterpret_cast<const float4*>(bn + BN_MU * fp + c);
        const float4 iv = *reinterpret_cast<const float4*>(bn + BN_INV * fp + c);
        const float4 c1 = *reinterpret_cast<const float4*>(cc + c);
        const float4 c2 = *reinterpret_cast<const float4*>(cc + fp + c);
        d.x = sc.x * (d.x - c1.x - (y.x - mu.x) * iv.x * c2.x);
        d.y = sc.y * (d.y - c1.y - (y.y - mu.y) * iv.y * c2.y);
        d.z = sc.z * (d.z - c1.z - (y.z - mu.z) * iv.z * c2.z);
        d.w = sc.w * (d.w - c1.w - (y.w - mu.w) * iv.w * c2.w);
        *reinterpret_cast<float4*>(dH + (size_t)r * fp + c) = d;
    }
}

__global__ __launch_bounds__(256) void unpack_grads_kernel(GradPtrs gp, ParamPtrs pp, ViewCols vc, ColMapD in,
                                                            int ld_in, int fp, const float* __restrict__ dWcat,
                                                            int nsplit, size_t slab, double* __restrict__ datt,
                                                            int nedge, const float* __restrict__ rsig, int wblocks,
                                                            const int32_t* __restrict__ meta, int xk_G, int edge_drain, int bx_per, int bx_wide) {
    nedge = nedge < 0 ? -nedge : min(nedge, (meta[EAGCN_META_T] + 15) / 16);
    const int bxm = bx_wide ? BX3W_BM : BX3_BM, bxn = bx_wide ? BX3W_BN : BX3_BN;
    nsplit = nsplit < 0 ? bx3_used_splits_wave(-nsplit, meta[EAGCN_META_T], ((ld_in + bxm - 1) / bxm) * ((fp + bxn - 1) / bxn),
                                          bx_per > 0 ? ((meta[EAGCN_META_T] + bxm - 1) / bxm) * ((ld_in + bxn - 1) / bxn) : 0, max(1, (fp + 31) >> 5), bx_per)
                        : max(1, min(nsplit, meta[EAGCN_META_T] >> 7));
    if ((int)blockIdx.x < wblocks) {
        const int tid = blockIdx.x * blockDim.x + threadIdx.x;
        if (xk_G > 0) {
            const int e = tid;
            if (e >= ld_in * fp) return;
            const int ip = e / fp, cp = e % fp;
            const int k = col_view(vc, cp), f = cp - vc.off[k];
            const int fi = packed_to_exact(in, ip);
            if (fi < 0 || f >= vc.width[k]) return;
            const int T = meta[EAGCN_META_T];
            G3Plan pl;
            g3_plan((T + 63) / 64, (ld_in + 63) / 64, max(1, (fp + 15) / 16), ((ld_in + 63) / 64) * ((fp + 63) / 64),
                    max(1, (T + 15) / 16), xk_G, pl);
            float v[G3_XSEG];
#pragma unroll
            for (int x = 0; x < G3_XSEG; ++x) v[x] = pl.c[x + 1] > pl.c[x] ? dWcat[(size_t)x * slab + e] : 0.0f;
            float t = 0.0f;
#pragma unroll
            for (int x = 0; x < G3_XSEG; ++x) t += v[x];
            gp.dW[k][(size_t)fi * vc.width[k] + f] = T > 0 ? t : 0.0f;
            return;
        }
        const int sub = tid & 3;
        const int e = (tid >> 2) * 4;
        if (e >= ld_in * fp) return;
        const int ip = e / fp, cp = e % fp;
        const int k = col_view(vc, cp), f = cp - vc.off[k];
        const int fi = packed_to_exact(in, ip);
        if (fi < 0 || f >= vc.width[k]) return;
        float4 s0 = make_float4(0.f, 0.f, 0.f, 0.f), s1 = s0;
        int z = sub;
#pragma unroll 4
        for (; z + 4 < nsplit; z += 8) {
            const float4 a0 = *reinterpret_cast<const float4*>(dWcat + (size_t)z * slab + e);
            const float4 a1 = *reinterpret_cast<const float4*>(dWcat + (size_t)(z + 4) * slab + e);
            s0.x += a0.x; s0.y += a0.y; s0.z += a0.z; s0.w += a0.w;
            s1.x += a1.x; s1.y += a1.y; s1.z += a1.z; s1.w += a1.w;
        }
        if (z < nsplit) {
            const float4 a0 = *reinterpret_cast<const float4*>(dWcat + (size_t)z * slab + e);
            s0.x += a0.x; s0.y += a0.y; s0.z += a0.z; s0.w += a0.w;
        }
        float t[4] = {s0.x + s1.x, s0.y + s1.y, s0.z + s1.z, s0.w + s1.w};
#pragma unroll
        for (int j = 0; j < 4; ++j) { t[j] += __shfl_xor(t[j], 1); t[j] += __shfl_xor(t[j], 2); }
        const float tv = sub == 0 ? t[0] : sub == 1 ? t[1] : sub == 2 ? t[2] : t[3];
        if (f + sub < vc.width[k]) gp.dW[k][(size_t)fi * vc.width[k] + f + sub] = tv;
        return;
    }
    const int er = ((int)blockIdx.x - wblocks) * 16 + (threadIdx.x >> 4), sl = threadIdx.x & 15;
    const int tot = vc.K * EDGE_SLAB;
    const int e = min(er, tot - 1);
    const int k = e / EDGE_SLAB, c = e % EDGE_SLAB;
    const bool general = pp.rel_vec[k] != nullptr && c != 256;
    double t = 0.0;
    if (!general) {
        for (int z0 = sl; z0 < nedge; z0 += 16 * 8) {
            double v[8];
#pragma unroll
            for (int u = 0; u < 8; ++u) {
                const int z = z0 + 16 * u;
                v[u] = z < nedge ? datt[(size_t)z * tot + e] : 0.0;
            }
#pragma unroll
            for (int u = 0; u < 8; ++u) t += v[u];
            if (edge_drain && er < tot) {
#pragma unroll
                for (int u = 0; u < 8; ++u) {
                    const int z = z0 + 16 * u;
                    if (z < nedge) datt[(size_t)z * tot + e] = 0.0;
                }
            }
        }
    } else if (c >= 1 && c <= pp.rel_c[k]) {
        const float* vec = pp.rel_vec[k];
        const int C = pp.rel_c[k], D = pp.channels[k];
        for (int z = sl; z < nedge; z += 16)
            for (int code = 1; code <= D; ++code)
                t += datt[(size_t)z * tot + k * EDGE_SLAB + code] * (double)vec[(size_t)(code - 1) * C + (c - 1)];
    }
#pragma unroll
    for (int o = 8; o > 0; o >>= 1) t += __shfl_xor(t, o);
    if (er >= tot || sl != 0) return;
    if (c == 256) {
        const double r = (double)rsig[k];
        gp.dself_r[k][0] = (float)(t * r * (1.0 - r));
    } else if (c >= 1 && c <= (pp.rel_vec[k] ? pp.rel_c[k] : pp.channels[k])) {
        gp.datt_w[k][c - 1] = (float)t;
    }
}

__global__ __launch_bounds__(256) void attention_dense_kernel(eagcn_batch bt, ParamPtrs pp, float* __restrict__ out) {
    const size_t total = (size_t)bt.K * bt.B * bt.N * bt.N;
    for (size_t e = (size_t)blockIdx.x * blockDim.x + threadIdx.x; e < total;
         e += (size_t)gridDim.x * blockDim.x) {
        const int j = (int)(e % bt.N);
        const size_t kbi = e / bt.N;
        const int k = (int)(kbi / ((size_t)bt.B * bt.N));
        const size_t bi = kbi - (size_t)k * bt.B * bt.N;
        const uint32_t c = bt.deg_bn[bi] > 0 ? bt.code[kbi * bt.ldc + j] : 0u;
        out[e] = (c >= 1 && (int)c <= pp.channels[k]) ? sigmoidf_(att_logit(pp, k, (int)c)) : 0.0f;
    }
}

struct Carver {
    char* base;
    size_t off = 0;
    explicit Carver(void* p) : base((char*)p) {}
    template <typename T>
    T* take(size_t n) {
        T* p = base ? (T*)(base + off) : nullptr;
        off = align256(off + n * sizeof(T));
        return p;
    }
};

struct LayerDims {
    ViewCols vc;
    int fp, ld_in, fin, ldo, gx, gxb, nsplit;
    int gslab;
    size_t wslab;
    size_t wpslab, wtpslab;
    int np;
    int bx_splits;
};
static LayerDims layer_dims(const eagcn_batch* b, const eagcn_layer_params* p) {
    LayerDims d;
    d.vc = view_cols(p);
    d.fp = d.vc.off[p->K];
    d.ld_in = layout_ld(&p->in);
    d.fin = layout_width(&p->in);
    d.ldo = p->structure == EAGCN_STRUCT_CONCATE ? d.fp : pad16(p->width[0]);
    d.gx = agg_grid_x(b);
    d.gslab = std::max(d.gx, lagg_use(b, 0, false, &d.vc) ? lagg_slabs(b) : 0);
    {
        const long by_rows = cdiv(b->T + 1, BWD_ROWS);
        const long by_bytes = std::max<long>(64, (32L << 20) / ((long)d.fp * 16));
        d.gxb = (int)std::max<long>(1, std::min<long>(std::min<long>(by_rows, 2048), by_bytes));
    }
    const int tiles = cdiv(d.ld_in, 64) * cdiv(d.fp, 64);
    d.nsplit = std::max(1, std::min(std::max(1, 1024 / tiles), cdiv(std::max(b->T, 1), 128)));
    d.wslab = (size_t)d.ld_in * d.fp;
    d.wpslab = bx_plane_elems(d.ld_in, d.fp);
    d.wtpslab = bx_plane_elems(d.fp, d.ld_in);
    d.np = (d.ld_in >= 128 && (d.ld_in & 15) == 0 && (d.fp & 15) == 0) ? gemm_planes() : 0;
    d.bx_splits = std::max(1, std::min(std::min(1023, std::max(64, cdiv(std::max(b->T, 1), 4096))), std::max(cdiv(std::max(b->T, 1), 4096), cdiv(std::max(b->T, 1), 256))));
    return d;
}

static bool gemm3_layer(int ld_in) {
    static const bool on = [] { const char* v = getenv("EAGCN_NO_GEMM3"); return !(v && v[0] == '1'); }();
    return on && ld_in >= 128 && gemm_mode() != 2;
}

struct Packed { float *Wcat, *WcatT, *colp, *sig, *rsig; uint16_t *Wp, *WTp; };
struct FwdScratch { void* gws; double* eacc; float *Wcat, *WcatT, *colp, *sig, *rsig; uint16_t *Wp, *WTp; double* stats; double* gsum;
                    uint16_t* xp; };
static size_t carve_packed(void* base, const LayerDims& d, Packed* s) {
    Carver c(base);
    Packed t;
    t.Wcat = c.take<float>(d.wslab);
    t.WcatT = c.take<float>(d.wslab);
    t.colp = c.take<float>((size_t)CP_ROWS * d.fp);
    t.sig = c.take<float>(EAGCN_MAX_VIEWS * 256);
    t.rsig = c.take<float>(EAGCN_MAX_VIEWS);
    t.Wp = c.take<uint16_t>(d.np ? (size_t)d.np * d.wpslab : 1);
    t.WTp = c.take<uint16_t>(d.np ? (size_t)d.np * d.wtpslab : 1);
    if (s) *s = t;
    return c.off;
}
struct BwdScratch {
    void* gws;
    double* eacc;
    float *Wcat, *WcatT, *colp, *sig, *rsig, *dY, *dP, *cc, *dWcat;
    uint16_t *Wp, *WTp;
    double *slab, *slab_da, *datt, *gsum;
    uint16_t *dPp, *xp;
};
static size_t carve_fwd(void* base, const eagcn_batch* b, const LayerDims& d, FwdScratch* s) {
    Carver c(base);
    FwdScratch t;
    t.gws = c.take<char>(gemm3_workspace_bytes());
    t.eacc = (double*)c.take<char>(edge_acc_bytes());
    t.Wcat = c.take<float>(d.wslab);
    t.WcatT = c.take<float>(d.wslab);
    t.colp = c.take<float>((size_t)CP_ROWS * d.fp);
    t.sig = c.take<float>(EAGCN_MAX_VIEWS * 256);
    t.rsig = c.take<float>(EAGCN_MAX_VIEWS);
    t.Wp = c.take<uint16_t>(d.np ? (size_t)d.np * d.wpslab : 1);
    t.WTp = c.take<uint16_t>(d.np ? (size_t)d.np * d.wtpslab : 1);
    t.stats = c.take<double>((size_t)d.gslab * d.fp * 2);
    t.gsum = c.take<double>((size_t)2 * d.fp + 8);
    t.xp = c.take<uint16_t>(d.np ? (size_t)d.np * bx_plane_elems(b->T, d.ld_in) : 1);
    if (s) *s = t;
    return c.off;
}
static size_t carve_bwd(void* base, const eagcn_batch* b, const LayerDims& d, BwdScratch* s) {
    Carver c(base);
    BwdScratch t;
    t.gws = c.take<char>(gemm3_workspace_bytes());
    t.eacc = (double*)c.take<char>(edge_acc_bytes());
    t.Wcat = c.take<float>(d.wslab);
// ... 6 lines not shown
    t.dY = c.take<float>((size_t)std::max(b->T, 1) * d.fp);
    t.dP = c.take<float>((size_t)std::max(b->T, 1) * d.fp);
    t.cc = c.take<float>((size_t)2 * d.fp);
    t.dWcat = c.take<float>(d.wslab * std::max(std::max(d.nsplit, G3_XSEG), d.np ? d.bx_splits : 1));
    t.slab = c.take<double>((size_t)d.gxb * d.fp * 2);
    t.slab_da = c.take<double>((size_t)d.gxb * cdiv(d.fp, 1024) * EAGCN_MAX_VIEWS);
    t.datt = c.take<double>((size_t)edge_grid_x(b) * EAGCN_MAX_VIEWS * EDGE_SLAB);
    t.gsum = c.take<double>((size_t)2 * d.fp + 8);
    t.dPp = c.take<uint16_t>(d.np ? (size_t)d.np * bx_plane_elems(b->T, d.fp) : 1);
    t.xp = c.take<uint16_t>(d.np ? (size_t)d.np * bx_plane_elems(b->T, d.ld_in) : 1);
    if (s) *s = t;
    return c.off;
}

static int check_layer(const eagcn_batch* b, const eagcn_layer_params* p, const char* who) {
    EAGCN_CHECK_ARG(b && p, "%s: null argument", who);
    EAGCN_CHECK_ARG(p->K >= 1 && p->K <= EAGCN_MAX_VIEWS && p->K == b->K,
                    "%s: layer has %d views, batch index has %d", who, p->K, b->K);
    EAGCN_CHECK_ARG(p->structure == EAGCN_STRUCT_CONCATE || p->structure == EAGCN_STRUCT_WEIGHTED,
                    "%s: unknown structure %d", who, p->structure);
    EAGCN_CHECK_ARG(p->in.nseg >= 1 && p->in.nseg <= EAGCN_MAX_SEGS, "%s: bad input layout", who);
    for (int s = 0; s < p->in.nseg; ++s)
        EAGCN_CHECK_ARG(p->in.width[s] >= 1 && p->in.pad[s] >= p->in.width[s] && (p->in.pad[s] % 4) == 0,
                        "%s: input segment %d: width %d pad %d (pad must be a multiple of 4 >= width)", who, s,
                        p->in.width[s], p->in.pad[s]);
    for (int k = 0; k < p->K; ++k) {
        EAGCN_CHECK_ARG(p->width[k] >= 1, "%s: view %d has width %d", who, k, p->width[k]);
        EAGCN_CHECK_ARG(p->att_w[k] && p->self_r[k] && p->W[k] && p->bias[k] && p->gamma[k] && p->beta[k] &&
                            p->run_mean[k] && p->run_var[k], "%s: view %d has a null parameter", who, k);
        if (p->structure == EAGCN_STRUCT_WEIGHTED)
            EAGCN_CHECK_ARG(p->width[k] == p->width[0], "%s: Weighted_sum needs equal view widths", who);
    }
    if (p->structure == EAGCN_STRUCT_WEIGHTED) EAGCN_CHECK_ARG(p->ave_w, "%s: Weighted_sum needs ave_w", who);
    EAGCN_CHECK_ARG(p->dropout >= 0.0f && p->dropout < 1.0f, "%s: dropout %f out of [0,1)", who, p->dropout);
    EAGCN_CHECK_ARG((uint64_t)std::max(b->T, 0) * (uint64_t)view_cols(p).off[p->K] / 4 < (1ull << 32),
                    "%s: %d rows x %d packed columns exceed the 32-bit element index of the BatchNorm passes", who, b->T,
                    view_cols(p).off[p->K]);
    return EAGCN_OK;
}

static ParamPtrs param_ptrs(const eagcn_batch* b, const eagcn_layer_params* p) {
    ParamPtrs pp;
    memset(&pp, 0, sizeof(pp));
    for (int k = 0; k < p->K; ++k) {
        pp.att_w[k] = p->att_w[k]; pp.self_r[k] = p->self_r[k]; pp.W[k] = p->W[k]; pp.bias[k] = p->bias[k];
        pp.gamma[k] = p->gamma[k]; pp.beta[k] = p->beta[k]; pp.run_mean[k] = p->run_mean[k];
        pp.run_var[k] = p->run_var[k]; pp.channels[k] = b->channels[k];
        pp.rel_vec[k] = b->rel_vec[k]; pp.rel_c[k] = b->rel_c[k];
    }
    pp.ave_w = p->structure == EAGCN_STRUCT_WEIGHTED ? p->ave_w : nullptr;
    return pp;
}

static inline int ew_grid(size_t n) { return (int)std::max<size_t>(1, std::min<size_t>((n + 255) / 256, 2048)); }

}

static int apply_launch_(const eagcn_batch* b, const eagcn_layer_params* p, const eagcn_layer_bufs* w, const eagcn::LayerDims& d,
                         const float* colp, hipStream_t s, bool planes_only = false);
#define apply_launch apply_launch_

using namespace eagcn;

extern "C" int eagcn_pad16(int w) { return pad16(w); }
extern "C" int eagcn_layer_fp(const eagcn_layer_params* p) { return view_cols(p).off[p->K]; }
extern "C" int eagcn_layer_out_ld(const eagcn_layer_params* p) {
    return p->structure == EAGCN_STRUCT_CONCATE ? eagcn_layer_fp(p) : pad16(p->width[0]);
}
extern "C" size_t eagcn_layer_packed_bytes(const eagcn_batch* b, const eagcn_layer_params* p) {
    LayerDims d = layer_dims(b, p);
    return carve_packed(nullptr, d, nullptr);
}
extern "C" size_t eagcn_layer_fwd_scratch_bytes(const eagcn_batch* b, const eagcn_layer_params* p) {
    LayerDims d = layer_dims(b, p);
    return carve_fwd(nullptr, b, d, nullptr);
}
extern "C" size_t eagcn_layer_bwd_scratch_bytes(const eagcn_batch* b, const eagcn_layer_params* p) {
    LayerDims d = layer_dims(b, p);
    return carve_bwd(nullptr, b, d, nullptr);
}

extern "C" int eagcn_layer_forward(const eagcn_batch* b, const eagcn_layer_params* p, const eagcn_layer_bufs* w,
                                   void* stream) {
    EAGCN_CHECK_GEMM3("eagcn_layer_forward");
    if (w && w->scratch && w->scratch_bytes >= gemm3_workspace_bytes()) {
        int rc = gemm3_clear_flags(w->scratch, w->scratch_bytes, (hipStream_t)stream);
        if (rc) return rc;
    }
    return layer_forward_impl(b, p, w, stream, false);
}

int eagcn::pack_params_all(const eagcn_batch* b, const eagcn_layer_params* const* ps, void* const* packed,
                           const size_t* packed_bytes, int n, void* stream, const ZeroJob* zj, const HandOff* ho) {
    hipStream_t s = (hipStream_t)stream;
    EAGCN_CHECK_ARG(n >= 1 && n <= 4, "pack_params_all: 1..4 layers");
    PackJob jobs[4];
    size_t wmax = 0;
    for (int l = 0; l < 4; ++l) {
        const int ll = l < n ? l : n - 1;
        int rc = check_layer(b, ps[ll], "eagcn_model_forward");
        if (rc) return rc;
        const LayerDims d = layer_dims(b, ps[ll]);
        Packed pk;
        const size_t pneed = carve_packed(packed[ll], d, &pk);
        if (pneed > packed_bytes[ll]) {
            set_error("pack_params_all: packed buffer of layer %d too small (%zu < %zu)", ll, packed_bytes[ll], pneed);
            return EAGCN_ERR_SCRATCH;
        }
        jobs[l].pp = param_ptrs(b, ps[ll]); jobs[l].vc = d.vc; jobs[l].in = make_colmap(&ps[ll]->in);
        jobs[l].ld_in = d.ld_in; jobs[l].fp = d.fp;
        jobs[l].Wcat = pk.Wcat; jobs[l].WcatT = pk.WcatT; jobs[l].colp = pk.colp; jobs[l].sig = pk.sig; jobs[l].rsig = pk.rsig;
        jobs[l].wp = BxOut{d.np ? pk.Wp : nullptr, d.wpslab, d.np, d.ld_in};
        jobs[l].wtp = BxOut{d.np ? pk.WTp : nullptr, d.wtpslab, d.np, d.fp};
        if (l < n) wmax = std::max(wmax, d.wslab);
    }
    PackJobs pj{jobs[0], jobs[1], jobs[2], jobs[3]};
    ProfScope ps_(PROF_PACK, s);
    const ZeroJob none{nullptr, 0, nullptr, 0};
    const HandOff noho{nullptr, nullptr, nullptr, 0};
    pack_params_multi_kernel<<<dim3(ew_grid(wmax), n), 256, 0, s>>>(pj, zj ? *zj : none, ho ? *ho : noho);
    EAGCN_LAUNCH_CHECK();
    return EAGCN_OK;
}

int eagcn::layer_forward_impl(const eagcn_batch* b, const eagcn_layer_params* p, const eagcn_layer_bufs* w,
                              void* stream, bool prepacked, bool skip_apply, bool planes_only) {
    hipStream_t s = (hipStream_t)stream;
    int rc = check_layer(b, p, "eagcn_layer_forward");
    if (rc) return rc;
    EAGCN_CHECK_ARG(w && w->bn && w->xout && w->pad_row && w->scratch, "eagcn_layer_forward: null buffer");
    EAGCN_CHECK_ARG(b->T == 0 || ((w->x || w->x_planes) && w->P && w->Y && w->rscale), "eagcn_layer_forward: null activation buffer");
    EAGCN_CHECK_ARG(!planes_only || (w->xout_planes && gemm_planes()), "eagcn_layer_forward: planes-only output without plane images");
    const LayerDims d = layer_dims(b, p);
    FwdScratch sc;
    const size_t need = carve_fwd(w->scratch, b, d, &sc);
    if (need > w->scratch_bytes) {
        set_error("eagcn_layer_forward: scratch too small (%zu < %zu)", w->scratch_bytes, need);
        return EAGCN_ERR_SCRATCH;
    }
    const ParamPtrs pp = param_ptrs(b, p);
    const ColMapD in = make_colmap(&p->in);
    if (w->packed) {
        Packed pk;
        const size_t pneed = carve_packed(w->packed, d, &pk);
        if (pneed > w->packed_bytes) {
            set_error("eagcn_layer_forward: packed buffer too small (%zu < %zu)", w->packed_bytes, pneed);
            return EAGCN_ERR_SCRATCH;
        }
        sc.Wcat = pk.Wcat; sc.WcatT = pk.WcatT; sc.colp = pk.colp; sc.sig = pk.sig; sc.rsig = pk.rsig;
        sc.Wp = pk.Wp; sc.WTp = pk.WTp;
    }
    EAGCN_CHECK_ARG(!prepacked || w->packed, "eagcn_layer_forward: prepacked parameters need the packed block");
    if (!prepacked) {
        ProfScope ps(PROF_PACK, s);
        pack_params_kernel<<<ew_grid(d.wslab), 256, 0, s>>>(pp, d.vc, in, d.ld_in, d.fp, sc.Wcat, sc.WcatT, sc.colp, sc.sig, sc.rsig,
                                                            BxOut{d.np ? sc.Wp : nullptr, d.wpslab, d.np, d.ld_in},
                                                            BxOut{d.np ? sc.WTp : nullptr, d.wtpslab, d.np, d.fp});
    }
    EAGCN_LAUNCH_CHECK();
    double fsum = 0.0;
    for (int k = 0; k < p->K; ++k) fsum += p->width[k];
    const double gemm_work = 2.0 * (double)b->T * (double)d.fin * fsum;
    int nslab = 0, tiles_per_wg = agg_ksplit(b) ? 1 : 4;
    if (b->T > 0) {
        GemmDesc g3{0, 1, b->T, d.fp, d.ld_in, w->x, d.ld_in, sc.WcatT, d.ld_in, w->P, d.fp, 1, 0, gemm_work};
        g3.M_dev = b->meta + EAGCN_META_T;
        BxProb bp;
        memset(&bp, 0, sizeof(bp));
        if (d.np) {
            const size_t xstride = bx_plane_elems(b->T, d.ld_in);
            const uint16_t* xp = w->x_planes;
            if (!xp) {
                EAGCN_CHECK_ARG(w->x, "eagcn_layer_forward: neither an fp32 input nor its plane images");
                rc = launch_bx3_split(w->x, b->T, b->meta + EAGCN_META_T, d.ld_in, sc.xp, xstride, b->T, d.np, s);
                if (rc) return rc;
                xp = sc.xp;
            }
            bp.A = BxPlanes{xp, xstride, d.ld_in, b->T}; bp.B = BxPlanes{sc.WTp, d.wtpslab, d.ld_in, d.fp}; bp.C = w->P; bp.ldc = d.fp;
            bp.M = b->T; bp.N = d.fp; bp.K = d.ld_in; bp.M_dev = b->meta + EAGCN_META_T; bp.tn = 0; bp.splits = 1;
        }
        if (d.np && bx3_ok(bp)) {
            rc = launch_bx3(bp, nullptr, d.np, s, gemm_work, PROF_GEMM, bx3_pick_wide(bp, nullptr, b->t_hint));
        } else if (!w->x) {
            set_error("eagcn_layer_forward: the input exists as plane images only and the plane product does not apply");
            return EAGCN_ERR_ARG;
        } else if (gemm3_layer(d.ld_in) && gemm3_ok(g3)) {
            rc = launch_gemm3(g3, nullptr, sc.gws, gemm3_workspace_bytes(), s);
        } else {
            GemmDesc g{0, 0, b->T, d.fp, d.ld_in, w->x, d.ld_in, sc.Wcat, d.fp, w->P, d.fp, 1, 0, gemm_work};
            g.M_dev = b->meta + EAGCN_META_T;
            rc = launch_gemm(g, s);
        }
        if (rc) return rc;
        {
            AggArgs a;
            a.bt = *b; a.vc = d.vc; a.src = w->P; a.lds = d.fp; a.dst = w->Y; a.ldd = d.fp;
            a.sig = sc.sig; a.rsig = sc.rsig; a.rscale = w->rscale; a.stats = sc.stats; a.nchunk = 1;
            if (lagg_use(b, 0, false, &d.vc)) {
                rc = launch_lagg_fwd(a, s);
                nslab = lagg_slabs(b);
                tiles_per_wg = -1;
            } else {
                rc = launch_agg(a, false, s);
                nslab = d.gx;
            }
            if (rc) return rc;
        }
    }
    const double M = (double)b->B * (double)b->N;
    {
    ProfScope psbn(PROF_BN, s);
    if (w->stats_hook && p->training) {
        if (nslab > 64) bn_stats_sum_kernel<64><<<cdiv(d.fp, 4), 256, 0, s>>>(sc.stats, nslab, d.fp, M, sc.gsum, b->meta, 1, tiles_per_wg, 0, b->B);
        else bn_stats_sum_kernel<16><<<cdiv(d.fp, 16), 256, 0, s>>>(sc.stats, nslab, d.fp, M, sc.gsum, b->meta, 1, tiles_per_wg, 0, b->B);
        EAGCN_LAUNCH_CHECK();
        if (w->stats_hook(sc.gsum, 2 * d.fp + 1, stream, w->stats_user)) {
            set_error("eagcn_layer_forward: the sync-BatchNorm all-reduce hook failed");
            return EAGCN_ERR_HIP;
        }
        bn_finalize_kernel<16><<<cdiv(d.fp, 16), 256, 0, s>>>(sc.gsum, 1, d.fp, M, p->training, p->bn_eps, p->bn_momentum, sc.colp,
                                                                pp, d.vc, w->bn, b->meta, 0, b->B, sc.gsum + 2 * d.fp);
    } else if (nslab > 64)
        bn_finalize_kernel<64><<<cdiv(d.fp, 4), 256, 0, s>>>(sc.stats, nslab, d.fp, M, p->training, p->bn_eps,
                                                               p->bn_momentum, sc.colp, pp, d.vc, w->bn, b->meta, tiles_per_wg, b->B, nullptr);
    else
        bn_finalize_kernel<16><<<cdiv(d.fp, 16), 256, 0, s>>>(sc.stats, nslab, d.fp, M, p->training, p->bn_eps,
                                                                p->bn_momentum, sc.colp, pp, d.vc, w->bn, b->meta, tiles_per_wg, b->B, nullptr);
    EAGCN_LAUNCH_CHECK();
    }
    if (skip_apply) return EAGCN_OK;
    return apply_launch(b, p, w, d, sc.colp, s, planes_only);
}

bool eagcn::layer_reads_planes_only(const eagcn_batch* b, const eagcn_layer_params* p, bool aux_stream) {
    static const bool on = [] { const char* v = getenv("EAGCN_PLANES_ONLY"); return !(v && v[0] == '0'); }();
    if (!on || aux_stream || !b || !p || b->T <= 0) return false;
    const LayerDims d = layer_dims(b, p);
    if (!d.np) return false;
    const uint16_t* pl = reinterpret_cast<const uint16_t*>(static_cast<uintptr_t>(4096));
    float* fo = reinterpret_cast<float*>(static_cast<uintptr_t>(4096));
    const size_t xstride = bx_plane_elems(b->T, d.ld_in), pstride = bx_plane_elems(b->T, d.fp);
    BxProb bp, bx, bw;
    memset(&bp, 0, sizeof(bp)); memset(&bx, 0, sizeof(bx)); memset(&bw, 0, sizeof(bw));
    bp.A = BxPlanes{pl, xstride, d.ld_in, b->T}; bp.B = BxPlanes{pl, d.wtpslab, d.ld_in, d.fp}; bp.C = fo; bp.ldc = d.fp;
    bp.M = b->T; bp.N = d.fp; bp.K = d.ld_in; bp.M_dev = b->meta + EAGCN_META_T; bp.tn = 0; bp.splits = 1;
    bx.A = BxPlanes{pl, pstride, d.fp, b->T}; bx.B = BxPlanes{pl, d.wpslab, d.fp, d.ld_in}; bx.C = fo; bx.ldc = d.ld_in;
// ... 15 lines not shown
static int apply_launch_(const eagcn_batch* b, const eagcn_layer_params* p, const eagcn_layer_bufs* w, const LayerDims& d,
                         const float* colp, hipStream_t s, bool planes_only) {
    ProfScope psbn(PROF_BN, s);
    ApplyArgs aa;
    aa.bt = *b; aa.vc = d.vc; aa.structure = p->structure; aa.fp = d.fp; aa.Y = w->Y; aa.ldy = d.fp;
    aa.bn = w->bn; aa.colp = colp; aa.out = w->xout; aa.ldo = d.ldo; aa.pad_row = w->pad_row;
    aa.do_drop = (p->training && p->dropout > 0.0f) ? 1 : 0;
    aa.thr = (uint32_t)std::min(4294967295.0, (double)p->dropout * 4294967296.0);
    aa.inv_keep = 1.0f / (1.0f - p->dropout);
    aa.seed = p->seed;
    aa.seed_dev = p->seed_dev;
    aa.planes = BxOut{gemm_planes() ? w->xout_planes : nullptr, bx_plane_elems(b->T, d.ldo), gemm_planes(), b->T};
    if (planes_only && aa.planes.p) aa.out = nullptr;
    static const int map_env = [] { const char* v = getenv("EAGCN_BN_APPLY_MAP"); return v ? atoi(v) : -1; }();
    aa.tile_map = map_env >= 0 ? map_env : (aa.planes.p ? 1 : 0);
    const size_t nthr = aa.tile_map ? (size_t)cdiv(std::max(b->T, 1), 8) * cdiv(d.ldo, 32) * 64 : (size_t)std::max(b->T, 1) * d.ldo / 4;
    bn_apply_kernel<<<ew_grid(nthr), 256, 0, s>>>(aa);
    EAGCN_LAUNCH_CHECK();
    return EAGCN_OK;
}

static bool lagg_fuses_bn() {
    static const bool on = [] { const char* v = getenv("EAGCN_LAGG_FUSE_BN"); return !(v && v[0] == '0'); }();
    return on;
}
static bool bn_bwd_two_pass(bool weighted) {
    static const int force = [] { const char* v = getenv("EAGCN_BWD_STORE_DH"); return v ? (v[0] == '1' ? 1 : 0) : -1; }();
    return force < 0 ? weighted : force == 0;
}
static void launch_bn_bwd_pass(bool apply, bool wt, bool dg, bool dr, dim3 grid, const BwdArgs& ba, hipStream_t s) {
#define EAGCN_BWD(W, G, D) do { if (apply) bn_bwd_reduce_kernel<W, G, D, true><<<grid, 256, 0, s>>>(ba); \
                                else bn_bwd_reduce_kernel<W, G, D, false><<<grid, 256, 0, s>>>(ba); } while (0)
    if (wt) { if (dg) { if (dr) EAGCN_BWD(true, true, true); else EAGCN_BWD(true, true, false); }
              else    { if (dr) EAGCN_BWD(true, false, true); else EAGCN_BWD(true, false, false); } }
    else    { if (dg) { if (dr) EAGCN_BWD(false, true, true); else EAGCN_BWD(false, true, false); }
              else    { if (dr) EAGCN_BWD(false, false, true); else EAGCN_BWD(false, false, false); } }
#undef EAGCN_BWD
}

extern "C" int eagcn_layer_backward(const eagcn_batch* b, const eagcn_layer_params* p, const eagcn_layer_bufs* w,
                                    const float* dxout, const float* dpad_row, float* dx,
                                    const eagcn_layer_grads* g, void* stream) {
    EAGCN_CHECK_GEMM3("eagcn_layer_backward");
    if (w && w->scratch && w->scratch_bytes >= gemm3_workspace_bytes()) {
        int rc = gemm3_clear_flags(w->scratch, w->scratch_bytes, (hipStream_t)stream);
        if (rc) return rc;
    }
    return layer_backward_impl(b, p, w, dxout, nullptr, dpad_row, dx, g, stream);
}

int eagcn::layer_backward_impl(const eagcn_batch* b, const eagcn_layer_params* p, const eagcn_layer_bufs* w,
                               const float* dxout, const ReadoutGrad* rg, const float* dpad_row, float* dx,
                               const eagcn_layer_grads* g, void* stream, bool dpad_views, const ZeroJob* zero_after,
                               const EdgeDrain* drain_in, EdgeDrain* drain_out, bool input_only) {
    if (drain_out) drain_out->eacc = nullptr;
    hipStream_t s = (hipStream_t)stream;
    int rc = check_layer(b, p, "eagcn_layer_backward");
    if (rc) return rc;
    EAGCN_CHECK_ARG(w && (g || input_only) && w->bn && w->scratch, "eagcn_layer_backward: null buffer");
    EAGCN_CHECK_ARG(!input_only || (dx && !drain_in), "eagcn_layer_backward: the input-only form needs dx and takes no edge reduction");
    EAGCN_CHECK_ARG(b->T == 0 || ((dxout || rg) && (input_only || w->x || w->x_planes) && w->P && w->Y && w->rscale),
                    "eagcn_layer_backward: null activation buffer");
    if (!input_only)
        for (int k = 0; k < p->K; ++k)
            EAGCN_CHECK_ARG(g->dW[k] && g->dbias[k] && g->dgamma[k] && g->dbeta[k] && g->datt_w[k] && g->dself_r[k],
                            "eagcn_layer_backward: view %d has a null gradient buffer", k);
    const LayerDims d = layer_dims(b, p);
    BwdScratch sc;
    const size_t need = carve_bwd(w->scratch, b, d, &sc);
    if (need > w->scratch_bytes) {
        set_error("eagcn_layer_backward: scratch too small (%zu < %zu)", w->scratch_bytes, need);
        return EAGCN_ERR_SCRATCH;
    }
    const ParamPtrs pp = param_ptrs(b, p);
    GradPtrs gp;
    memset(&gp, 0, sizeof(gp));
    if (input_only) {
        EAGCN_CHECK_ARG(d.wslab >= (size_t)3 * d.fp + EAGCN_MAX_VIEWS, "eagcn_layer_backward: no room for the discarded BatchNorm gradients");
        for (int k = 0; k < p->K; ++k) {
            gp.dgamma[k] = sc.dWcat + d.vc.off[k];
            gp.dbeta[k] = sc.dWcat + d.fp + d.vc.off[k];
            gp.dbias[k] = sc.dWcat + 2 * d.fp + d.vc.off[k];
        }
        gp.dave_w = p->structure == EAGCN_STRUCT_WEIGHTED ? sc.dWcat + 3 * d.fp : nullptr;
    } else {
        for (int k = 0; k < p->K; ++k) {
            gp.dW[k] = g->dW[k]; gp.dbias[k] = g->dbias[k]; gp.dgamma[k] = g->dgamma[k]; gp.dbeta[k] = g->dbeta[k];
            gp.datt_w[k] = g->datt_w[k]; gp.dself_r[k] = g->dself_r[k];
        }
        gp.dave_w = p->structure == EAGCN_STRUCT_WEIGHTED ? g->dave_w : nullptr;
    }
    const ColMapD in = make_colmap(&p->in);
    if (w->packed) {
        Packed pk;
        const size_t pneed = carve_packed(w->packed, d, &pk);
        if (pneed > w->packed_bytes) {
            set_error("eagcn_layer_backward: packed buffer too small (%zu < %zu)", w->packed_bytes, pneed);
            return EAGCN_ERR_SCRATCH;
        }
        sc.Wcat = pk.Wcat; sc.WcatT = pk.WcatT; sc.colp = pk.colp; sc.sig = pk.sig; sc.rsig = pk.rsig;
        sc.Wp = pk.Wp; sc.WTp = pk.WTp;
    } else {
        ProfScope ps(PROF_PACK, s);
        pack_params_kernel<<<ew_grid(d.wslab), 256, 0, s>>>(pp, d.vc, in, d.ld_in, d.fp, sc.Wcat, sc.WcatT, sc.colp, sc.sig, sc.rsig,
                                                            BxOut{d.np ? sc.Wp : nullptr, d.wpslab, d.np, d.ld_in},
                                                            BxOut{d.np ? sc.WTp : nullptr, d.wtpslab, d.np, d.fp});
    }
    EAGCN_LAUNCH_CHECK();
    double fsum = 0.0;
    for (int k = 0; k < p->K; ++k) fsum += p->width[k];
    const double gemm_work = 2.0 * (double)b->T * (double)d.fin * fsum;

    BwdArgs ba;
    ba.meta = b->meta; ba.Tcap = b->T; ba.row_mol = b->row_mol; ba.row_m = b->row_m;
    ba.vc = d.vc; ba.structure = p->structure; ba.fp = d.fp;
    ba.nvirt = (dpad_row && p->structure == EAGCN_STRUCT_WEIGHTED) ? 1 : 0;
    ba.dxout = dxout; ba.ldo = d.ldo; ba.dpad = dpad_row; ba.dpad_views = dpad_views ? 1 : 0;
    if (rg) ba.rg = *rg; else memset(&ba.rg, 0, sizeof(ba.rg)); ba.Y = w->Y; ba.ldy = d.fp; ba.bn = w->bn;
    ba.colp = sc.colp; ba.dH = sc.dY; ba.slab = sc.slab; ba.slab_da = sc.slab_da;
    ba.do_drop = (p->training && p->dropout > 0.0f) ? 1 : 0;
    ba.thr = (uint32_t)std::min(4294967295.0, (double)p->dropout * 4294967296.0);
    ba.inv_keep = 1.0f / (1.0f - p->dropout);
    ba.seed = p->seed;
    ba.seed_dev = p->seed_dev;
    ba.zero = zero_after ? zero_after->d : nullptr;
    ba.nzero = zero_after ? zero_after->nd : 0;
    if (drain_in && drain_in->eacc) ba.drain = *drain_in; else memset(&ba.drain, 0, sizeof(ba.drain));
    const int rows = b->T + ba.nvirt;
    const int gxb = std::max(1, std::min(rows, d.gxb));
    bool fused_bn_apply = false, fused_w_apply = false, w_rows = false, fused_c_apply = false;
    bool lagg_bwd = false;
    {
        static const bool edge_atomic0 = [] { const char* v = getenv("EAGCN_EDGE_SLABS"); return !(v && v[0] == '1'); }();
        bool general0 = false;
        for (int k = 0; k < p->K; ++k) general0 = general0 || pp.rel_vec[k] != nullptr;
        const bool wt0 = p->structure == EAGCN_STRUCT_WEIGHTED;
        const bool absorbs = lagg_fuses_bn() && (!bn_bwd_two_pass(wt0) || (wt0 && lagg_wfuse()));
        lagg_bwd = b->T > 0 && edge_atomic0 && !general0 && lagg_use(b, 1, absorbs);
        if (input_only) lagg_bwd = b->T > 0 && lagg_use(b, 1, true);
    }
    const double M = (double)b->B * (double)b->N;
    const bool eval_in = input_only && !p->training;
    if (eval_in) {
        const bool wt = p->structure == EAGCN_STRUCT_WEIGHTED, dg = ba.rg.dg != nullptr;
        if (b->T > 0 && lagg_bwd) {
            if (dg) {
                rc = launch_readout_bwd_rows(b, ba.rg, d.ldo, sc.dY, s);
                if (rc) return rc;
                w_rows = true;
            }
            if (wt) fused_w_apply = true; else fused_c_apply = true;
        } else if (b->T > 0) {
            rc = zero_fill(sc.cc, (size_t)2 * d.fp * sizeof(float), s);
            if (rc) return rc;
            ba.cc = sc.cc;
            launch_bn_bwd_pass(true, wt, dg, false, dim3(std::max(1, std::min(b->T, d.gxb)), cdiv(d.fp, 1024)), ba, s);
            EAGCN_LAUNCH_CHECK();
        }
        if (zero_after && zero_after->nd) { rc = zero_fill(zero_after->d, (size_t)zero_after->nd * sizeof(double), s); if (rc) return rc; }
    } else {
        ProfScope ps(PROF_BN, s);
        const int ny = cdiv(d.fp, 1024);
        {
            const bool wt = p->structure == EAGCN_STRUCT_WEIGHTED, dr = ba.do_drop != 0;
            bool dg = ba.rg.dg != nullptr;
            const dim3 grid(gxb, ny);
            ba.cc = sc.cc;
            ba.store_dh = bn_bwd_two_pass(wt) ? 0 : 1;
            static const bool rows_first = [] { const char* v = getenv("EAGCN_W_ROWS_FIRST"); return !(v && v[0] == '0'); }();
            if (wt && dg && b->T > 0 && bn_bwd_two_pass(wt) && lagg_bwd && lagg_fuses_bn() && lagg_wfuse() && rows_first) {
                rc = launch_readout_bwd_rows(b, ba.rg, d.ldo, sc.dY, s);
                if (rc) return rc;
                w_rows = true;
                ba.dxout = sc.dY;
                dg = false;
            }
            launch_bn_bwd_pass(false, wt, dg, dr, grid, ba, s);
        }
        EAGCN_LAUNCH_CHECK();
        const double* gsum = nullptr;
        if (w->stats_hook && p->training) {
            if (gxb > 64) bn_stats_sum_kernel<64><<<cdiv(d.fp, 4), 256, 0, s>>>(sc.slab, gxb, d.fp, M, sc.gsum, b->meta, 2, 0, ba.nvirt, b->B);
            else bn_stats_sum_kernel<16><<<cdiv(d.fp, 16), 256, 0, s>>>(sc.slab, gxb, d.fp, M, sc.gsum, b->meta, 2, 0, ba.nvirt, b->B);
            EAGCN_LAUNCH_CHECK();
            if (w->stats_hook(sc.gsum, 2 * d.fp + 1, stream, w->stats_user)) {
                set_error("eagcn_layer_backward: the sync-BatchNorm all-reduce hook failed");
                return EAGCN_ERR_HIP;
            }
            gsum = sc.gsum;
        }
        if (gxb > 64)
            bn_bwd_finalize_kernel<64><<<cdiv(d.fp, 4), 256, 0, s>>>(sc.slab, sc.slab_da, gxb, d.fp, M, p->training, w->bn,
                                                                       d.vc, gp, sc.cc, b->meta, ba.nvirt, b->B, ny, gxb, gsum, ba.zero, ba.nzero);
        else
            bn_bwd_finalize_kernel<16><<<cdiv(d.fp, 16), 256, 0, s>>>(sc.slab, sc.slab_da, gxb, d.fp, M, p->training, w->bn,
                                                                        d.vc, gp, sc.cc, b->meta, ba.nvirt, b->B, ny, gxb, gsum, ba.zero, ba.nzero);
        EAGCN_LAUNCH_CHECK();
        if (b->T > 0) {
            const bool wt = p->structure == EAGCN_STRUCT_WEIGHTED, dg = ba.rg.dg != nullptr, dr = ba.do_drop != 0;
            if (bn_bwd_two_pass(wt) && wt && lagg_bwd && lagg_fuses_bn() && lagg_wfuse()) {
                fused_w_apply = true;
                if (dg && !w_rows) {
                    rc = launch_readout_bwd_rows(b, ba.rg, d.ldo, sc.dY, s);
                    if (rc) return rc;
                }
            } else if (bn_bwd_two_pass(wt)) launch_bn_bwd_pass(true, wt, dg, dr, dim3(std::max(1, std::min(b->T, d.gxb)), ny), ba, s);
            else if (lagg_bwd && lagg_fuses_bn()) fused_bn_apply = true;
            else bn_bwd_apply_kernel<<<ew_grid((size_t)b->T * d.fp / 4), 256, 0, s>>>(*b, d.fp, w->Y, d.fp, w->bn, sc.cc, sc.dY);
            EAGCN_LAUNCH_CHECK();
        }
    }
    int nsplit = 0, nedge = 0, xk_G = 0;
    bool bx_slabs = false;
    int bx_per = 0;
    int bx_wide = 0;
    hipStream_t side = w->aux_stream ? (hipStream_t)w->aux_stream : s;
    const bool forked = side != s;
    if (b->T > 0) {
        AggArgs a;
        a.bt = *b; a.vc = d.vc; a.src = sc.dY; a.lds = d.fp; a.dst = sc.dP; a.ldd = d.fp;
        a.sig = sc.sig; a.rsig = sc.rsig; a.rscale = w->rscale; a.stats = nullptr; a.nchunk = 1;
        const size_t xstride = bx_plane_elems(b->T, d.ld_in), pstride = bx_plane_elems(b->T, d.fp);
        BxProb bx, bw;
        memset(&bx, 0, sizeof(bx));
        memset(&bw, 0, sizeof(bw));
        bool use_bx = false;
        if (d.np && !w->aux_stream) {
            bx.A = BxPlanes{sc.dPp, pstride, d.fp, b->T}; bx.B = BxPlanes{sc.Wp, d.wpslab, d.fp, d.ld_in}; bx.C = dx; bx.ldc = d.ld_in;
            bx.M = b->T; bx.N = d.ld_in; bx.K = d.fp; bx.M_dev = b->meta + EAGCN_META_T; bx.tn = 0; bx.splits = 1;
            bw.A = BxPlanes{w->x_planes ? w->x_planes : sc.xp, xstride, d.ld_in, b->T}; bw.B = BxPlanes{sc.dPp, pstride, d.fp, b->T};
            bw.C = sc.dWcat; bw.ldc = d.fp; bw.M = d.ld_in; bw.N = d.fp; bw.K = b->T; bw.K_dev = b->meta + EAGCN_META_T; bw.tn = 1;
            bw.splits = d.bx_splits; bw.slab = d.wslab;
            use_bx = bx3_ok(bw) && (!dx || bx3_ok(bx));
        }
        if (use_bx) {
            a.planes = BxOut{sc.dPp, pstride, d.np, b->T};
            if (!w->x_planes && !input_only) {
                rc = launch_bx3_split(w->x, b->T, b->meta + EAGCN_META_T, d.ld_in, sc.xp, xstride, b->T, d.np, s);
                if (rc) return rc;
            }
        } else if (!w->x && !input_only) {
            set_error("eagcn_layer_backward: the input exists as plane images only and the plane products do not apply");
            return EAGCN_ERR_ARG;
        }
        EdgeArgs e;
        e.bt = *b; e.vc = d.vc; e.dY = sc.dY; e.Y = w->Y; e.P = w->P; e.ld = d.fp; e.sig = sc.sig;
        e.rsig = sc.rsig; e.rscale = w->rscale; e.datt = sc.datt; e.atomic = 0;
        static const bool edge_atomic = [] { const char* v = getenv("EAGCN_EDGE_SLABS"); return !(v && v[0] == '1'); }();
        bool general_rel = false;
        for (int k = 0; k < p->K; ++k) general_rel = general_rel || pp.rel_vec[k] != nullptr;
        if (edge_atomic && !general_rel) { e.datt = sc.eacc; e.atomic = 1; }
        static const bool colaunch = [] { const char* v = getenv("EAGCN_NO_COLAUNCH"); return !(v && v[0] == '1'); }();
        nedge = e.atomic ? -EDGE_COPIES : edge_grid_x(b);
        if (input_only) {
            if (lagg_bwd) {
                if (fused_bn_apply || fused_w_apply || fused_c_apply) { a.bn_tab = w->bn; a.bn_cc = eval_in ? nullptr : sc.cc; a.bn_fp = d.fp; }
                if (fused_w_apply || fused_c_apply) {
                    a.src = (ba.rg.dg || w_rows) ? sc.dY : dxout; a.lds = d.ldo;
                    a.w_aw = sc.colp + (size_t)CP_AVEW * d.fp;
                    a.w_rowm = fused_c_apply;
                    a.w_drop = ba.do_drop; a.w_thr = ba.thr; a.w_inv_keep = ba.inv_keep; a.w_seed = ba.seed; a.w_seed_dev = ba.seed_dev;
                }
                rc = launch_lagg_bwd(a, e, s, false);
            } else {
                rc = launch_agg(a, true, s);
            }
            if (rc) return rc;
            if (use_bx) {
                rc = launch_bx3(bx, nullptr, d.np, s, gemm_work, PROF_GEMM, bx3_pick_wide(bx, nullptr, b->t_hint));
            } else {
                GemmDesc gx{0, 1, b->T, d.ld_in, d.fp, sc.dP, d.fp, sc.Wcat, d.fp, dx, d.ld_in, 1, 0, gemm_work};
                gx.M_dev = b->meta + EAGCN_META_T;
                rc = launch_gemm(gx, s);
            }
            return rc;
        }
        if (lagg_bwd && e.atomic) {
            if (fused_bn_apply || fused_w_apply) { a.bn_tab = w->bn; a.bn_cc = sc.cc; a.bn_fp = d.fp; }
            if (fused_w_apply) {
                a.src = (ba.rg.dg || w_rows) ? sc.dY : dxout; a.lds = d.ldo;
                a.w_aw = sc.colp + (size_t)CP_AVEW * d.fp;
                a.w_drop = ba.do_drop; a.w_thr = ba.thr; a.w_inv_keep = ba.inv_keep; a.w_seed = ba.seed; a.w_seed_dev = ba.seed_dev;
            }
            rc = launch_lagg_bwd(a, e, s);
            if (rc) return rc;
        } else if (!forked && colaunch) {
            rc = launch_agg_edge(a, e, s);
            if (rc) return rc;
        } else {
            if (forked) { rc = stream_after(side, s); if (rc) return rc; }
            rc = launch_edge_grad(e, side);
            if (rc) return rc;
            rc = launch_agg(a, true, s);
            if (rc) return rc;
        }
        if (forked) { rc = stream_after(side, s); if (rc) return rc; }
        nsplit = d.nsplit;
        GemmDesc gw{1, 0, d.ld_in, d.fp, b->T, w->x, d.ld_in, sc.dP, d.fp, sc.dWcat, d.fp, nsplit, d.wslab, gemm_work};
        gw.K_dev = b->meta + EAGCN_META_T;
        GemmDesc gx{0, 1, b->T, d.ld_in, d.fp, sc.dP, d.fp, sc.Wcat, d.fp, dx, d.ld_in, 1, 0, gemm_work};
        gx.M_dev = b->meta + EAGCN_META_T;
        static const bool pair = [] { const char* v = getenv("EAGCN_NO_PAIR"); return !(v && v[0] == '1'); }();
        static const bool use3 = [] { const char* v = getenv("EAGCN_NO_GEMM3"); return !(v && v[0] == '1'); }();
        DwScatter dsc;
        for (int k = 0; k < EAGCN_MAX_VIEWS; ++k) dsc.dW[k] = gp.dW[k];
        dsc.vc = d.vc;
        dsc.in = in;
        if (use_bx) {
            bx_wide = dx ? bx3_pick_wide(bx, &bw, b->t_hint) : bx3_pick_wide(bw, nullptr, b->t_hint);
            rc = dx ? launch_bx3(bx, &bw, d.np, s, 2.0 * gemm_work, PROF_GEMM_PAIR, bx_wide) : launch_bx3(bw, nullptr, d.np, s, gemm_work, PROF_GEMM, bx_wide);
            if (rc) return rc;
            nsplit = d.bx_splits;
            bx_slabs = true;
            bx_per = (dx && bx3_pair_policy()) ? std::max(1, bx3_grid() >> 3) : 0;
        } else if (use3 && !forked && dx && gemm3_layer(d.ld_in) && gemm3_ok(gw) && gemm3_ok(gx) && gemm3_xk_enabled()) {
            rc = launch_gemm3_pair(gx, gw, nullptr, sc.gws, gemm3_workspace_bytes(), s, d.wslab);
            if (rc) return rc;
            nsplit = 1;
            xk_G = gemm3_grid();
        } else if (use3 && !forked && dx && gemm3_layer(d.ld_in) && gemm3_ok(gw) && gemm3_ok(gx)) {
            rc = launch_gemm3_pair(gx, gw, &dsc, sc.gws, gemm3_workspace_bytes(), s);
            if (rc) return rc;
            nsplit = 0;
        } else if (dx && !forked && colaunch && pair) {
            rc = launch_gemm_pair(gx, gw, s);
            if (rc) return rc;
        } else {
            rc = launch_gemm(gw, side);
            if (rc) return rc;
            if (dx) { rc = launch_gemm(gx, s); if (rc) return rc; }
        }
    }
    if (b->T == 0 && input_only) return EAGCN_OK;
    if (b->T == 0) {
        for (int k = 0; k < p->K; ++k)
            { int rcz = zero_fill(gp.dW[k], (size_t)d.fin * p->width[k] * sizeof(float), side); if (rcz) return rcz; }
    }
    {
        const int wblocks = nsplit > 0 ? cdiv((int)d.wslab, 256) : 0;
        double* edge_src = nedge == -EDGE_COPIES ? sc.eacc : sc.datt;
        const int edge_drain = edge_src == sc.eacc ? 1 : 0;
        static const bool defer_env = [] { const char* v = getenv("EAGCN_NO_EDGE_DEFER"); return !(v && v[0] == '1'); }();
        if (defer_env && drain_out && edge_drain && wblocks == 0 && !forked && b->T > 0) {
            drain_out->eacc = sc.eacc; drain_out->K = p->K; drain_out->rsig = sc.rsig;
            for (int k = 0; k < EAGCN_MAX_VIEWS; ++k) {
                drain_out->datt_w[k] = gp.datt_w[k]; drain_out->dself_r[k] = gp.dself_r[k]; drain_out->channels[k] = pp.channels[k];
            }
            return EAGCN_OK;
        }
        ProfScope psu(PROF_PACK, side);
        unpack_grads_kernel<<<wblocks + cdiv(p->K * EDGE_SLAB, 16), 256, 0, side>>>(gp, pp, d.vc, in, d.ld_in, d.fp, sc.dWcat,
                                                                                    bx_slabs ? -nsplit : nsplit, d.wslab, edge_src, nedge, sc.rsig,
                                                                                    wblocks, b->meta, xk_G, edge_drain, bx_per, bx_wide);
        EAGCN_LAUNCH_CHECK();
    }
    if (forked) { rc = stream_after(s, side); if (rc) return rc; }
    return EAGCN_OK;
}

extern "C" int eagcn_attention_dense(const eagcn_batch* b, const eagcn_layer_params* p, float* out, void* stream) {
    hipStream_t s = (hipStream_t)stream;
    EAGCN_CHECK_ARG(b && p && out, "eagcn_attention_dense: null argument");
    EAGCN_CHECK_ARG(p->K == b->K, "eagcn_attention_dense: view count mismatch");
    EAGCN_CHECK_ARG(b->code, "eagcn_attention_dense: batch has no code map");
    ParamPtrs pp;
    memset(&pp, 0, sizeof(pp));
    for (int k = 0; k < p->K; ++k) {
        EAGCN_CHECK_ARG(p->att_w[k], "eagcn_attention_dense: view %d has no attention weight", k);
        pp.att_w[k] = p->att_w[k];
        pp.channels[k] = b->channels[k];
        pp.rel_vec[k] = b->rel_vec[k]; pp.rel_c[k] = b->rel_c[k];
    }
    const size_t total = (size_t)b->K * b->B * b->N * b->N;
    attention_dense_kernel<<<ew_grid(total), 256, 0, s>>>(*b, pp, out);
    EAGCN_LAUNCH_CHECK();
    return EAGCN_OK;
}
```

### include/eagcn_hip.h

```cpp
#ifndef EAGCN_HIP_H
#define EAGCN_HIP_H

#include <stddef.h>
#include <stdint.h>

#ifdef __cplusplus
extern "C" {
#endif

#define EAGCN_MAX_VIEWS 8
#define EAGCN_MAX_SEGS 8
#define EAGCN_MAX_CHANNELS 255
#define EAGCN_STRUCT_CONCATE 0
#define EAGCN_STRUCT_WEIGHTED 1

#define EAGCN_OK 0
#define EAGCN_ERR_ARG (-1)
#define EAGCN_ERR_HIP (-2)
#define EAGCN_ERR_SCRATCH (-3)

#define EAGCN_META_T 0
#define EAGCN_META_NMAX 1
#define EAGCN_META_NTILES 2
#define EAGCN_META_BAD_ADJ 3
// ... 247 lines not shown
                               size_t saved_bytes, void* scratch, size_t scratch_bytes, const float* dout,
                               const float* dgraph_rep, const eagcn_layer_grads* lg, const eagcn_head_grads* hg,
                               float* dafm, void* stream);

float eagcn_attr_alpha(int step, int steps);
float eagcn_attr_weight(int steps);
size_t eagcn_attr_acc_elems(const eagcn_batch* b, const eagcn_model* m);
int eagcn_attr_pack_input(const eagcn_batch* b, const eagcn_model* m, const float* afm, const float* baseline, float alpha,
                          void* saved, size_t saved_bytes, void* stream);
int eagcn_attr_step(const eagcn_batch* b, const eagcn_model* m, const int64_t* size, void* saved, size_t saved_bytes,
                    void* scratch, size_t scratch_bytes, const float* dout, const float* dgraph_rep, float weight, int first,
                    float* acc, void* stream);
int eagcn_attr_finalize(const eagcn_batch* b, const eagcn_model* m, const float* afm, const float* baseline, const float* acc,
                        float* attr, float* score, void* stream);

typedef struct eagcn_step_loss {
    int32_t kind;
    const float* labels;
    const float* class_weight;
    float* loss;
    const float* scale;
    float* dout;
} eagcn_step_loss;
int eagcn_model_forward_step(const eagcn_batch* b, const eagcn_model* m, const float* afm, const int64_t* size,
                             void* saved, size_t saved_bytes, void* scratch, size_t scratch_bytes, float* out,
                             float* graph_rep, const eagcn_step_loss* loss, const float* dgraph_rep,
                             const eagcn_head_grads* hg, void* stream);

size_t eagcn_head_saved_bytes(const eagcn_head_params* h, int B);
size_t eagcn_head_scratch_bytes(const eagcn_head_params* h, int B);
int eagcn_head_forward(const eagcn_head_params* h, int B, int training, uint64_t seed, const uint64_t* seed_dev, const float* g,
                       void* saved, size_t saved_bytes, void* scratch, size_t scratch_bytes, float* out, float* graph_rep,
                       void* stream);
int eagcn_head_backward(const eagcn_head_params* h, int B, int training, uint64_t seed, const uint64_t* seed_dev, const float* g,
                        void* saved, size_t saved_bytes, void* scratch, size_t scratch_bytes, const float* dout,
                        const float* dgraph_rep, const eagcn_head_grads* hg, float* dg, void* stream);

int eagcn_bce_loss(const float* logits, const float* labels, const float* class_weight, int B, int T,
                   float* loss, float* dlogits, void* stream);
int eagcn_mse_loss(const float* pred, const float* target, int n, float* loss, float* dpred, void* stream);

int eagcn_adam_step(float* param, const float* grad, float* exp_avg, float* exp_avg_sq, int64_t n, const double* hyper_dev,
                    int64_t* step_dev, uint32_t* ticket_dev, void* stream);

int eagcn_eval_append(const float* logits, const float* labels, int B, int T, int classification, float* scores,
                      float* targets, uint8_t* valid, int64_t row_offset, void* stream);

int eagcn_set_gemm_mode(int mode);

size_t eagcn_bx3_plane_elems(int rows_cap, int ld);
int eagcn_bx3_split(const float* x, int rows, int ld, uint16_t* planes, size_t plane_stride, int rows_cap, int np, void* stream);
int eagcn_bx3_used_splits(int splits, int M, int N, int K);
int eagcn_set_bx3_wide(int mode);
int eagcn_bx3_pair_used_splits(int splits, int M, int N, int K, int M0, int N0, int K0);
int eagcn_gemm_bx3(int tn, int M, int N, int K, const uint16_t* A, size_t a_pstride, int lda, int a_rows, const uint16_t* B,
                   size_t b_pstride, int ldb, int b_rows, float* C, int ldc, int splits, size_t slab, int np, void* stream);
int eagcn_gemm_bx3_pair(int M0, int N0, int K0, const uint16_t* A0, size_t a0_pstride, int lda0, int a0_rows, const uint16_t* B0,
                        size_t b0_pstride, int ldb0, int b0_rows, float* C0, int ldc0, int M1, int N1, int K1, const uint16_t* A1,
                        size_t a1_pstride, int lda1, int a1_rows, const uint16_t* B1, size_t b1_pstride, int ldb1, int b1_rows,
                        float* C1, int ldc1, int splits, size_t slab, int np, void* stream);

int eagcn_gemm_f32(int ta, int tb, int M, int N, int K, const float* A, int lda, const float* B,
                   int ldb, float* C, int ldc, void* stream);
int eagcn_gemm_f32_dev(int ta, int tb, int M, int N, int K, const float* A, int lda, const float* B,
                       int ldb, float* C, int ldc, const int32_t* extent_dev, int which, void* stream);

size_t eagcn_gemm_sk_workspace_bytes(void);
int eagcn_gemm_f32_sk(int ta, int tb, int M, int N, int K, const float* A, int lda, const float* B, int ldb, float* C,
                      int ldc, void* workspace, size_t workspace_bytes, void* stream);
int eagcn_gemm_pair_sk(int M0, int N0, int K0, const float* A0, int lda0, const float* B0, int ldb0, float* C0, int ldc0,
                       int M1, int N1, int K1, const float* A1, int lda1, const float* B1, int ldb1, float* C1, int ldc1,
                       void* workspace, size_t workspace_bytes, void* stream);
int eagcn_gemm_pair_sk_slabs(int M0, int N0, int K0, const float* A0, int lda0, const float* B0, int ldb0, float* C0, int ldc0,
                             int M1, int N1, int K1, const float* A1, int lda1, const float* B1, int ldb1, float* C1, int ldc1,
                             size_t slab, void* workspace, size_t workspace_bytes, void* stream);
int eagcn_gemm_sk_plan(int M0, int N0, int K0, int M1, int N1, int K1, int wgs, int* a, int* c);
int eagcn_gemm_sk_timeouts(void);
int eagcn_gemm_sk_failed(void);
void eagcn_gemm_sk_reset_failed(void);
void eagcn_gemm_sk_inject_failure(void);

void eagcn_prof_enable(int on);
void eagcn_prof_reset(void);
int eagcn_prof_ntags(void);
const char* eagcn_prof_tag_name(int tag);
int eagcn_prof_read(int tag, double* total_ms, double* work, int64_t* launches);

#ifdef __cplusplus
}
#endif
#endif
```

Before: 692,400.

## Ride parameter packing and weight-grad unpack along with neighbouring kernels

After: 685,200. 1.0% lower.

```diff
diff --git a/eagcn_amd/_lib.py b/eagcn_amd/_lib.py
--- a/eagcn_amd/_lib.py
+++ b/eagcn_amd/_lib.py
@@ -139,6 +139,7 @@
     'eagcn_agg_wants_bond_lists_for': (C.c_int, [C.c_int, C.c_int, C.c_int]),
     'eagcn_bx3_used_splits': (C.c_int, [C.c_int, C.c_int, C.c_int, C.c_int]),
     'eagcn_set_bx3_wide': (C.c_int, [C.c_int]),
+    'eagcn_set_ride_along': (C.c_int, [C.c_int]),
     'eagcn_bx3_pair_used_splits': (C.c_int, [C.c_int] * 7),
     'eagcn_bx3_plane_elems': (C.c_size_t, [C.c_int, C.c_int]),
     'eagcn_bx3_split': (C.c_int, [_fp, C.c_int, C.c_int, _fp, C.c_size_t, C.c_int, C.c_int, _fp]),
diff --git a/eagcn_amd/csrc/gemm.hip b/eagcn_amd/csrc/gemm.hip
--- a/eagcn_amd/csrc/gemm.hip
+++ b/eagcn_amd/csrc/gemm.hip
@@ -4,6 +4,7 @@
 
 #include "common.h"
 #include "gemm_x6.h"
+#include "kernels.h"
 
 namespace eagcn {
 
@@ -271,6 +272,24 @@
     }
 }
 
+struct GemmPackArgs { GemmDesc g; int gx, gy; int njobs, per; PackJobs jobs; };
+template <int BM, int BN, int BK, bool A_KC, bool B_KC, int D>
+__global__ __launch_bounds__(256) void gemm_f32_pack_kernel(GemmPackArgs a) {
+    const int b = blockIdx.x, ntile = a.gx * a.gy;
+    if (b >= ntile) {
+        const int per = a.per, vb = b - ntile, job = vb / per;
+        const GemmPackArgs* ka = reinterpret_cast<const GemmPackArgs*>((const void*)__builtin_amdgcn_kernarg_segment_ptr());
+        if (job < a.njobs) EAGCN_PACK_JOBS(ka->jobs, job, vb - job * per, per);
+        return;
+    }
+    const int gx = a.gx;
+    const int Mx = a.g.M_dev ? min(*a.g.M_dev, a.g.M) : a.g.M;
+    const int per_z = gx * ((Mx + BM - 1) / BM);
+    if (b >= per_z) return;
+    const int nid = xcd_remap(b, per_z);
+    const int tile_y = nid / gx;
+    gemm_tile<BM, BN, BK, A_KC, B_KC, D>(a.g, Mx, a.g.K, nid - tile_y * gx, tile_y, 0, 1);
+}
 
 template <int BM, int BN, int BK, int D>
 static int launch_cfg(const GemmDesc& g, hipStream_t s) {
@@ -330,6 +349,30 @@
     }
 }
 
+static bool gemm_cfg_forced() {
+    static const int forced = [] { const char* e = getenv("EAGCN_GEMM_CFG"); return e ? atoi(e) : -1; }();
+    return forced >= 0;
+}
+bool gemm_pack_ok(const GemmDesc& g) {
+    if (g.M <= 0 || g.N <= 0 || g.ta != 0 || g.tb != 0 || g.splits != 1 || g.K_dev || gemm_cfg_forced() || use_x6(g)) return false;
+    const long tiles128 = (long)cdiv(g.M, 128) * cdiv(g.N, 128);
+    return !(g.K >= 1024 && tiles128 >= 512 && g.M > 64 && g.N > 64);
+}
+int launch_gemm_pack(const GemmDesc& g0, const PackRide& pr, hipStream_t s) {
+    EAGCN_CHECK_ARG(gemm_pack_ok(g0) && pr.n >= 1 && pr.n <= 4 && pr.per >= 1, "gemm: this product cannot carry packing jobs");
+    GemmDesc g = g0;
+    g.vecA = (g.lda % 4) == 0 && (g.K % 4) == 0 && (reinterpret_cast<uintptr_t>(g.A) % 16) == 0;
+    g.vecB = (g.ldb % 4) == 0 && (g.N % 4) == 0 && (reinterpret_cast<uintptr_t>(g.B) % 16) == 0;
+    const int gx = cdiv(g.N, 64), gy = cdiv(g.M, 64);
+    {
+        ProfScope ps(g.prof_tag, s, g.work > 0.0 ? g.work : 2.0 * g.M * g.N * g.K);
+        GemmPackArgs ka{g, gx, gy, pr.n, pr.per, pr.jobs};
+        gemm_f32_pack_kernel<64, 64, 16, true, false, 4><<<gx * gy + pr.n * pr.per, 256, 0, s>>>(ka);
+    }
+    EAGCN_LAUNCH_CHECK();
+    return EAGCN_OK;
+}
+
 int launch_gemm_pair(const GemmDesc& dx, const GemmDesc& dw, hipStream_t s) {
     GemmDesc g0 = dx, g1 = dw;
     g0.vecA = (g0.lda % 4) == 0 && (g0.K % 4) == 0 && (reinterpret_cast<uintptr_t>(g0.A) % 16) == 0;
diff --git a/eagcn_amd/csrc/head.hip b/eagcn_amd/csrc/head.hip
--- a/eagcn_amd/csrc/head.hip
+++ b/eagcn_amd/csrc/head.hip
@@ -142,6 +142,7 @@
     double* hws;
     double* hsb;
     void* layer; size_t layer_bytes;
+    float* dw_down;
 };
 static size_t carve_scratch(void* base, const eagcn_batch* b, const eagcn_model* m, ModelScratch* out) {
     Carver2 c(base);
@@ -171,6 +172,9 @@
     s.dpad = c.take<float>((size_t)EAGCN_MAX_VIEWS * ldmax);
     s.layer_bytes = lbytes;
     s.layer = c.take<char>(lbytes);
+    size_t dwf = 0;
+    for (int l = 1; l < m->n_layers; ++l) dwf = std::max(dwf, layer_dw_slab_floats(b, &m->layer[l]));
+    s.dw_down = c.take<float>(dwf ? dwf : 1);
     if (out) *out = s;
     return c.off;
 }
@@ -351,12 +355,16 @@
     if (!m->input_packed)
         RC(eagcn_pack_rows(b, afm, layout_width(&m->layer[0].in), &m->layer[0].in, sv.x0, stream));
     const float* x = sv.x0;
+    PackRide ride;
+    bool riding = false;
     {
         const eagcn_layer_params* ps[4];
         void* pk[4];
         size_t pkb[4];
         for (int l = 0; l < m->n_layers; ++l) { ps[l] = &m->layer[l]; pk[l] = sv.L[l].packed; pkb[l] = sv.L[l].packed_bytes; }
-        RC(pack_params_all(b, ps, pk, pkb, m->n_layers, stream, &zj, &ho));
+        riding = (ride_along_mode() & 2) && m->n_layers >= 2 && layer_fwd_carries_pack(b, &m->layer[0], x);
+        if (riding) RC(pack_ride_jobs(b, ps, pk, pkb, 1, m->n_layers, &ride));
+        RC(pack_params_all(b, ps, pk, pkb, riding ? 1 : m->n_layers, stream, &zj, &ho));
     }
     for (int l = 0; l < m->n_layers; ++l) {
         LayerSaved& L = sv.L[l];
@@ -367,7 +375,8 @@
         w.stats_hook = m->stats_hook; w.stats_user = m->stats_user;
         w.x_planes = l > 0 ? sv.L[l - 1].xout_planes : nullptr; w.xout_planes = L.xout_planes;
         const bool po = hidden_planes_only(b, m, sv, l);
-        RC(layer_forward_impl(b, &m->layer[l], &w, stream, true, l == m->n_layers - 1 && fused_readout(m), po));
+        RC(layer_forward_impl(b, &m->layer[l], &w, stream, true, l == m->n_layers - 1 && fused_readout(m), po,
+                              (riding && l == 0) ? &ride : nullptr));
         x = po ? nullptr : L.xout;
     }
     const eagcn_layer_params* last = &m->layer[m->n_layers - 1];
@@ -647,7 +656,7 @@
     memset(&rgd, 0, sizeof(rgd));
     rgd.dg = sc.dg; rgd.F = F; rgd.size = size; rgd.mode = m->molfp_mode; rgd.map = make_colmap(&lay);
     const int top_l = m->n_layers - 1;
-    EdgeDrain pend_in, pend_out;
+    PendingGrads pend_in, pend_out;
     pend_in.eacc = nullptr;
     pend_out.eacc = nullptr;
     for (int l = layer_hi; l >= layer_lo; --l) {
@@ -667,7 +676,8 @@
         const float* dpad = (weighted && top) ? sc.dpad : nullptr;
         RC(layer_backward_impl(b, &m->layer[l], &w, top ? nullptr : cur, top ? &rgd : nullptr, dpad,
                                l > 0 ? other : dx0, input_only ? nullptr : &lg[l], stream, top && sampled, top ? &zb : nullptr,
-                               pend_in.eacc ? &pend_in : nullptr, (l > layer_lo && !input_only) ? &pend_out : nullptr, input_only));
+                               pend_in.eacc ? &pend_in : nullptr, (l > layer_lo && !input_only) ? &pend_out : nullptr, input_only,
+                               sc.dw_down));
         pend_in = pend_out;
         if (l == layer_lo) pend_in.eacc = nullptr;
     }
diff --git a/eagcn_amd/csrc/index.hip b/eagcn_amd/csrc/index.hip
--- a/eagcn_amd/csrc/index.hip
+++ b/eagcn_amd/csrc/index.hip
@@ -642,15 +642,6 @@
 }
 
 typedef ColMapD ColMap;
-__device__ __forceinline__ int packed_to_exact(const ColMap& m, int cp) {
-    int eo = 0, po = 0;
-    for (int s = 0; s < m.nseg; ++s) {
-        if (cp < po + m.p[s]) return (cp - po < m.w[s]) ? eo + (cp - po) : -1;
-        eo += m.w[s];
-        po += m.p[s];
-    }
-    return -1;
-}
 
 __global__ __launch_bounds__(256) void pack_rows_kernel(eagcn_batch bt, const float* __restrict__ dense,
                                                          int F, ColMap m, int ld, float* __restrict__ packed, int Nin) {
diff --git a/eagcn_amd/csrc/kernels.h b/eagcn_amd/csrc/kernels.h
--- a/eagcn_amd/csrc/kernels.h
+++ b/eagcn_amd/csrc/kernels.h
@@ -198,16 +198,247 @@
 int head_bwd(const HeadBwd& a, hipStream_t s);
 int head_gbn_bwd(const HeadGbn& a, hipStream_t s);
 
-struct EdgeDrain {
-    double* eacc; int K;
-    float* datt_w[EAGCN_MAX_VIEWS]; float* dself_r[EAGCN_MAX_VIEWS]; int channels[EAGCN_MAX_VIEWS];
+struct ParamPtrs {
+    const float* att_w[EAGCN_MAX_VIEWS];
+    const float* self_r[EAGCN_MAX_VIEWS];
+    const float* W[EAGCN_MAX_VIEWS];
+    const float* bias[EAGCN_MAX_VIEWS];
+    const float* gamma[EAGCN_MAX_VIEWS];
+    const float* beta[EAGCN_MAX_VIEWS];
+    float* run_mean[EAGCN_MAX_VIEWS];
+    float* run_var[EAGCN_MAX_VIEWS];
+    const float* ave_w;
+    int channels[EAGCN_MAX_VIEWS];
+    const float* rel_vec[EAGCN_MAX_VIEWS];
+    int rel_c[EAGCN_MAX_VIEWS];
+};
+__device__ __forceinline__ float att_logit(const ParamPtrs& pp, int k, int c) {
+    if (!pp.rel_vec[k]) return pp.att_w[k][c - 1];
+    const float* v = pp.rel_vec[k] + (size_t)(c - 1) * pp.rel_c[k];
+    float s = 0.0f;
+    for (int ch = 0; ch < pp.rel_c[k]; ++ch) s = fmaf(pp.att_w[k][ch], v[ch], s);
+    return s;
+}
+struct GradPtrs {
+    float* dW[EAGCN_MAX_VIEWS];
+    float* dbias[EAGCN_MAX_VIEWS];
+    float* dgamma[EAGCN_MAX_VIEWS];
+    float* dbeta[EAGCN_MAX_VIEWS];
+    float* datt_w[EAGCN_MAX_VIEWS];
+    float* dself_r[EAGCN_MAX_VIEWS];
+    float* dave_w;
+};
+
+enum { CP_GAMMA = 0, CP_BETA, CP_BIAS, CP_RMEAN, CP_RVAR, CP_AVEW, CP_ROWS = 8 };
+
+__device__ __forceinline__ int col_view(const ViewCols& vc, int cp) {
+    int k = 0;
+#pragma unroll
+    for (int v = 1; v < EAGCN_MAX_VIEWS; ++v) k += (v < vc.K && cp >= vc.off[v]) ? 1 : 0;
+    return k;
+}
+__device__ __forceinline__ int packed_to_exact(const ColMapD& m, int cp) {
+    int eo = 0, po = 0;
+    for (int s = 0; s < m.nseg; ++s) {
+        if (cp < po + m.p[s]) return (cp - po < m.w[s]) ? eo + (cp - po) : -1;
+        eo += m.w[s];
+        po += m.p[s];
+    }
+    return -1;
+}
+
+__device__ __forceinline__ void pack_params_body(const int bid, const int nblk, const ParamPtrs& pp, const ViewCols& vc, const ColMapD& in, int ld_in,
+                                                 int fp, float* __restrict__ Wcat, float* __restrict__ WcatT,
+                                                 float* __restrict__ colp, float* __restrict__ sig, float* __restrict__ rsig,
+                                                 const BxOut wp = BxOut{nullptr, 0, 0, 0}, const BxOut wtp = BxOut{nullptr, 0, 0, 0}) {
+    __shared__ float tile[32][33];
+    const int tx = threadIdx.x & 31, ty = threadIdx.x >> 5;
+    const int ntx = (fp + 31) >> 5, nty = (ld_in + 31) >> 5;
+    for (int t = bid; t < ntx * nty; t += nblk) {
+        const int ip0 = (t / ntx) << 5, cp0 = (t % ntx) << 5;
+        {
+            const int cp = cp0 + tx;
+            const int k = cp < fp ? col_view(vc, cp) : 0;
+            const int f = cp - vc.off[k];
+#pragma unroll
+            for (int j = 0; j < 4; ++j) {
+                const int ip = ip0 + ty + 8 * j;
+                float v = 0.0f;
+                if (ip < ld_in && cp < fp) {
+                    const int fi = packed_to_exact(in, ip);
+                    if (fi >= 0 && f < vc.width[k]) v = pp.W[k][(size_t)fi * vc.width[k] + f];
+                    Wcat[(size_t)ip * fp + cp] = v;
+                }
+                tile[ty + 8 * j][tx] = v;
+            }
+        }
+        __syncthreads();
+#pragma unroll
+        for (int j = 0; j < 4; ++j) {
+            const int cp = cp0 + ty + 8 * j, ip = ip0 + tx;
+            if (cp < fp && ip < ld_in) WcatT[(size_t)cp * ld_in + ip] = tile[tx][ty + 8 * j];
+        }
+        if (wp.p) {
+            const int r = threadIdx.x >> 3, c4 = (threadIdx.x & 7) << 2;
+            if (ip0 + r < ld_in && cp0 + c4 < fp)
+                bx_store4(wp, ip0 + r, cp0 + c4, make_float4(tile[r][c4], tile[r][c4 + 1], tile[r][c4 + 2], tile[r][c4 + 3]));
+            if (cp0 + r < fp && ip0 + c4 < ld_in)
+                bx_store4(wtp, cp0 + r, ip0 + c4, make_float4(tile[c4][r], tile[c4 + 1][r], tile[c4 + 2][r], tile[c4 + 3][r]));
+        }
+        __syncthreads();
+    }
+    for (int cp = bid * blockDim.x + threadIdx.x; cp < fp; cp += nblk * blockDim.x) {
+        const int k = col_view(vc, cp), f = cp - vc.off[k];
+        const bool ok = f < vc.width[k];
+        colp[CP_GAMMA * fp + cp] = ok ? pp.gamma[k][f] : 0.0f;
+        colp[CP_BETA * fp + cp] = ok ? pp.beta[k][f] : 0.0f;
+        colp[CP_BIAS * fp + cp] = ok ? pp.bias[k][f] : 0.0f;
+        colp[CP_RMEAN * fp + cp] = ok ? pp.run_mean[k][f] : 0.0f;
+        colp[CP_RVAR * fp + cp] = ok ? pp.run_var[k][f] : 1.0f;
+        colp[CP_AVEW * fp + cp] = pp.ave_w ? pp.ave_w[k] : 1.0f;
+    }
+    for (int e = bid * blockDim.x + threadIdx.x; e < vc.K * 256; e += nblk * blockDim.x) {
+        const int k = e >> 8, c = e & 255;
+        sig[e] = (c >= 1 && c <= pp.channels[k]) ? sigmoidf_(att_logit(pp, k, c)) : 0.0f;
+    }
+    if (bid == 0 && threadIdx.x < vc.K) rsig[threadIdx.x] = sigmoidf_(pp.self_r[threadIdx.x][0]);
+}
+struct PackJob {
+    ParamPtrs pp; ViewCols vc; ColMapD in; int ld_in, fp;
+    float *Wcat, *WcatT, *colp, *sig, *rsig;
+    BxOut wp, wtp;
+};
+struct PackJobs { PackJob j0, j1, j2, j3; };
+#define EAGCN_PACK_JOB_(J, bid, nblk) pack_params_body(bid, nblk, J.pp, J.vc, J.in, J.ld_in, J.fp, J.Wcat, J.WcatT, J.colp, J.sig, J.rsig, J.wp, J.wtp)
+#define EAGCN_PACK_JOBS(jobs, job, bid, nblk)                          \
+    do {                                                               \
+        if ((job) == 0) EAGCN_PACK_JOB_(jobs.j0, bid, nblk);           \
+        else if ((job) == 1) EAGCN_PACK_JOB_(jobs.j1, bid, nblk);      \
+        else if ((job) == 2) EAGCN_PACK_JOB_(jobs.j2, bid, nblk);      \
+        else EAGCN_PACK_JOB_(jobs.j3, bid, nblk);                      \
+    } while (0)
+struct PackRide { PackJobs jobs; int n; int per; };
+bool gemm_pack_ok(const GemmDesc& g);
+int launch_gemm_pack(const GemmDesc& g, const PackRide& pr, hipStream_t s);
+
+__device__ __forceinline__ void unpack_grads_body(const int vb, const GradPtrs& gp, const ParamPtrs& pp, const ViewCols& vc, const ColMapD& in,
+                                                  int ld_in, int fp, const float* __restrict__ dWcat,
+                                                  int nsplit, size_t slab, double* __restrict__ datt,
+                                                  int nedge, const float* __restrict__ rsig, int wblocks,
+                                                  const int32_t* __restrict__ meta, int xk_G, int edge_drain, int bx_per, int bx_wide) {
+    nedge = nedge < 0 ? -nedge : min(nedge, (meta[EAGCN_META_T] + 15) / 16);
+    const int bxm = bx_wide ? BX3W_BM : BX3_BM, bxn = bx_wide ? BX3W_BN : BX3_BN;
+    nsplit = nsplit < 0 ? bx3_used_splits_wave(-nsplit, meta[EAGCN_META_T], ((ld_in + bxm - 1) / bxm) * ((fp + bxn - 1) / bxn),
+                                          bx_per > 0 ? ((meta[EAGCN_META_T] + bxm - 1) / bxm) * ((ld_in + bxn - 1) / bxn) : 0, max(1, (fp + 31) >> 5), bx_per)
+                        : max(1, min(nsplit, meta[EAGCN_META_T] >> 7));
+    if (vb < wblocks) {
+        const int tid = vb * blockDim.x + threadIdx.x;
+        if (xk_G > 0) {
+            const int e = tid;
+            if (e >= ld_in * fp) return;
+            const int ip = e / fp, cp = e % fp;
+            const int k = col_view(vc, cp), f = cp - vc.off[k];
+            const int fi = packed_to_exact(in, ip);
+            if (fi < 0 || f >= vc.width[k]) return;
+            const int T = meta[EAGCN_META_T];
+            G3Plan pl;
+            g3_plan((T + 63) / 64, (ld_in + 63) / 64, max(1, (fp + 15) / 16), ((ld_in + 63) / 64) * ((fp + 63) / 64),
+                    max(1, (T + 15) / 16), xk_G, pl);
+            float v[G3_XSEG];
+#pragma unroll
+            for (int x = 0; x < G3_XSEG; ++x) v[x] = pl.c[x + 1] > pl.c[x] ? dWcat[(size_t)x * slab + e] : 0.0f;
+            float t = 0.0f;
+#pragma unroll
+            for (int x = 0; x < G3_XSEG; ++x) t += v[x];
+            gp.dW[k][(size_t)fi * vc.width[k] + f] = T > 0 ? t : 0.0f;
+            return;
+        }
+        const int sub = tid & 3;
+        const int e = (tid >> 2) * 4;
+        if (e >= ld_in * fp) return;
+        const int ip = e / fp, cp = e % fp;
+        const int k = col_view(vc, cp), f = cp - vc.off[k];
+        const int fi = packed_to_exact(in, ip);
+        if (fi < 0 || f >= vc.width[k]) return;
+        float4 s0 = make_float4(0.f, 0.f, 0.f, 0.f), s1 = s0;
+        int z = sub;
+#pragma unroll 4
+        for (; z + 4 < nsplit; z += 8) {
+            const float4 a0 = *reinterpret_cast<const float4*>(dWcat + (size_t)z * slab + e);
+            const float4 a1 = *reinterpret_cast<const float4*>(dWcat + (size_t)(z + 4) * slab + e);
+            s0.x += a0.x; s0.y += a0.y; s0.z += a0.z; s0.w += a0.w;
+            s1.x += a1.x; s1.y += a1.y; s1.z += a1.z; s1.w += a1.w;
+        }
+        if (z < nsplit) {
+            const float4 a0 = *reinterpret_cast<const float4*>(dWcat + (size_t)z * slab + e);
+            s0.x += a0.x; s0.y += a0.y; s0.z += a0.z; s0.w += a0.w;
+        }
+        float t[4] = {s0.x + s1.x, s0.y + s1.y, s0.z + s1.z, s0.w + s1.w};
+#pragma unroll
+        for (int j = 0; j < 4; ++j) { t[j] += __shfl_xor(t[j], 1); t[j] += __shfl_xor(t[j], 2); }
+        const float tv = sub == 0 ? t[0] : sub == 1 ? t[1] : sub == 2 ? t[2] : t[3];
+        if (f + sub < vc.width[k]) gp.dW[k][(size_t)fi * vc.width[k] + f + sub] = tv;
+        return;
+    }
+    const int er = (vb - wblocks) * 16 + (threadIdx.x >> 4), sl = threadIdx.x & 15;
+    const int tot = vc.K * EDGE_SLAB;
+    const int e = min(er, tot - 1);
+    const int k = e / EDGE_SLAB, c = e % EDGE_SLAB;
+    const bool general = pp.rel_vec[k] != nullptr && c != 256;
+    double t = 0.0;
+    if (!general) {
+        for (int z0 = sl; z0 < nedge; z0 += 16 * 8) {
+            double v[8];
+#pragma unroll
+            for (int u = 0; u < 8; ++u) {
+                const int z = z0 + 16 * u;
+                v[u] = z < nedge ? datt[(size_t)z * tot + e] : 0.0;
+            }
+#pragma unroll
+            for (int u = 0; u < 8; ++u) t += v[u];
+            if (edge_drain && er < tot) {
+#pragma unroll
+                for (int u = 0; u < 8; ++u) {
+                    const int z = z0 + 16 * u;
+                    if (z < nedge) datt[(size_t)z * tot + e] = 0.0;
+                }
+            }
+        }
+    } else if (c >= 1 && c <= pp.rel_c[k]) {
+        const float* vec = pp.rel_vec[k];
+        const int C = pp.rel_c[k], D = pp.channels[k];
+        for (int z = sl; z < nedge; z += 16)
+            for (int code = 1; code <= D; ++code)
+                t += datt[(size_t)z * tot + k * EDGE_SLAB + code] * (double)vec[(size_t)(code - 1) * C + (c - 1)];
+    }
+#pragma unroll
+    for (int o = 8; o > 0; o >>= 1) t += __shfl_xor(t, o);
+    if (er >= tot || sl != 0) return;
+    if (c == 256) {
+        const double r = (double)rsig[k];
+        gp.dself_r[k][0] = (float)(t * r * (1.0 - r));
+    } else if (c >= 1 && c <= (pp.rel_vec[k] ? pp.rel_c[k] : pp.channels[k])) {
+        gp.datt_w[k][c - 1] = (float)t;
+    }
+}
+
+int ride_along_mode();
+
+struct PendingGrads {
+    double* eacc;
+    GradPtrs gp; ParamPtrs pp; ViewCols vc; ColMapD in;
+    int ld_in, fp;
+    const float* dWcat; int nsplit; size_t wslab;
+    int nedge;
     const float* rsig;
-};
+    int wblocks, xk_G, edge_drain, bx_per, bx_wide;
+};
+inline int pending_blocks(const PendingGrads& p) { return p.wblocks + cdiv(p.vc.K * EDGE_SLAB, 16); }
 int layer_backward_impl(const eagcn_batch* b, const eagcn_layer_params* p, const eagcn_layer_bufs* w,
                         const float* dxout, const ReadoutGrad* rg, const float* dpad_row, float* dx,
                         const eagcn_layer_grads* g, void* stream, bool dpad_views = false,
-                        const ZeroJob* zero_after = nullptr, const EdgeDrain* drain_in = nullptr, EdgeDrain* drain_out = nullptr,
-                        bool input_only = false);
+                        const ZeroJob* zero_after = nullptr, const PendingGrads* drain_in = nullptr, PendingGrads* drain_out = nullptr,
+                        bool input_only = false, float* dw_down = nullptr);
 int model_backward_input_packed(const eagcn_batch* b, const eagcn_model* m, const int64_t* size, void* saved, size_t saved_bytes,
                                 void* scratch, size_t scratch_bytes, const float* dout, const float* dgraph_rep,
                                 const eagcn_layer_grads* lg, const eagcn_head_grads* hg, float** dx0, void* stream, const char* who);
@@ -215,7 +446,11 @@
                       float* score, hipStream_t s);
 int model_input_slot(const eagcn_batch* b, const eagcn_model* m, void* saved, size_t saved_bytes, float** x0, const char* who);
 int layer_forward_impl(const eagcn_batch* b, const eagcn_layer_params* p, const eagcn_layer_bufs* w, void* stream,
-                       bool prepacked, bool skip_apply = false, bool planes_only = false);
+                       bool prepacked, bool skip_apply = false, bool planes_only = false, const PackRide* ride = nullptr);
+bool layer_fwd_carries_pack(const eagcn_batch* b, const eagcn_layer_params* p, const float* x);
+int pack_ride_jobs(const eagcn_batch* b, const eagcn_layer_params* const* ps, void* const* packed, const size_t* packed_bytes,
+                   int lo, int n, PackRide* out);
+size_t layer_dw_slab_floats(const eagcn_batch* b, const eagcn_layer_params* p);
 bool layer_reads_planes_only(const eagcn_batch* b, const eagcn_layer_params* p, bool aux_stream);
 int layer_apply_impl(const eagcn_batch* b, const eagcn_layer_params* p, const eagcn_layer_bufs* w, void* stream);
 int pack_params_all(const eagcn_batch* b, const eagcn_layer_params* const* ps, void* const* packed,
diff --git a/eagcn_amd/csrc/layer.hip b/eagcn_amd/csrc/layer.hip
--- a/eagcn_amd/csrc/layer.hip
+++ b/eagcn_amd/csrc/layer.hip
@@ -7,123 +7,12 @@
 
 namespace eagcn {
 
-struct ParamPtrs {
-    const float* att_w[EAGCN_MAX_VIEWS];
-    const float* self_r[EAGCN_MAX_VIEWS];
-    const float* W[EAGCN_MAX_VIEWS];
-    const float* bias[EAGCN_MAX_VIEWS];
-    const float* gamma[EAGCN_MAX_VIEWS];
-    const float* beta[EAGCN_MAX_VIEWS];
-    float* run_mean[EAGCN_MAX_VIEWS];
-    float* run_var[EAGCN_MAX_VIEWS];
-    const float* ave_w;
-    int channels[EAGCN_MAX_VIEWS];
-    const float* rel_vec[EAGCN_MAX_VIEWS];
-    int rel_c[EAGCN_MAX_VIEWS];
-};
-__device__ __forceinline__ float att_logit(const ParamPtrs& pp, int k, int c) {
-    if (!pp.rel_vec[k]) return pp.att_w[k][c - 1];
-    const float* v = pp.rel_vec[k] + (size_t)(c - 1) * pp.rel_c[k];
-    float s = 0.0f;
-    for (int ch = 0; ch < pp.rel_c[k]; ++ch) s = fmaf(pp.att_w[k][ch], v[ch], s);
-    return s;
-}
-struct GradPtrs {
-    float* dW[EAGCN_MAX_VIEWS];
-    float* dbias[EAGCN_MAX_VIEWS];
-    float* dgamma[EAGCN_MAX_VIEWS];
-    float* dbeta[EAGCN_MAX_VIEWS];
-    float* datt_w[EAGCN_MAX_VIEWS];
-    float* dself_r[EAGCN_MAX_VIEWS];
-    float* dave_w;
-};
-
-enum { CP_GAMMA = 0, CP_BETA, CP_BIAS, CP_RMEAN, CP_RVAR, CP_AVEW, CP_ROWS = 8 };
-
-__device__ __forceinline__ int col_view(const ViewCols& vc, int cp) {
-    int k = 0;
-#pragma unroll
-    for (int v = 1; v < EAGCN_MAX_VIEWS; ++v) k += (v < vc.K && cp >= vc.off[v]) ? 1 : 0;
-    return k;
-}
-__device__ __forceinline__ int packed_to_exact(const ColMapD& m, int cp) {
-    int eo = 0, po = 0;
-    for (int s = 0; s < m.nseg; ++s) {
-        if (cp < po + m.p[s]) return (cp - po < m.w[s]) ? eo + (cp - po) : -1;
-        eo += m.w[s];
-        po += m.p[s];
-    }
-    return -1;
-}
-
-__device__ __forceinline__ void pack_params_body(const ParamPtrs& pp, const ViewCols& vc, const ColMapD& in, int ld_in,
-                                                 int fp, float* __restrict__ Wcat, float* __restrict__ WcatT,
-                                                 float* __restrict__ colp, float* __restrict__ sig, float* __restrict__ rsig,
-                                                 const BxOut wp = BxOut{nullptr, 0, 0, 0}, const BxOut wtp = BxOut{nullptr, 0, 0, 0}) {
-    __shared__ float tile[32][33];
-    const int tx = threadIdx.x & 31, ty = threadIdx.x >> 5;
-    const int ntx = (fp + 31) >> 5, nty = (ld_in + 31) >> 5;
-    for (int t = blockIdx.x; t < ntx * nty; t += gridDim.x) {
-        const int ip0 = (t / ntx) << 5, cp0 = (t % ntx) << 5;
-        {
-            const int cp = cp0 + tx;
-            const int k = cp < fp ? col_view(vc, cp) : 0;
-            const int f = cp - vc.off[k];
-#pragma unroll
-            for (int j = 0; j < 4; ++j) {
-                const int ip = ip0 + ty + 8 * j;
-                float v = 0.0f;
-                if (ip < ld_in && cp < fp) {
-                    const int fi = packed_to_exact(in, ip);
-                    if (fi >= 0 && f < vc.width[k]) v = pp.W[k][(size_t)fi * vc.width[k] + f];
-                    Wcat[(size_t)ip * fp + cp] = v;
-                }
-                tile[ty + 8 * j][tx] = v;
-            }
-        }
-        __syncthreads();
-#pragma unroll
-        for (int j = 0; j < 4; ++j) {
-            const int cp = cp0 + ty + 8 * j, ip = ip0 + tx;
-            if (cp < fp && ip < ld_in) WcatT[(size_t)cp * ld_in + ip] = tile[tx][ty + 8 * j];
-        }
-        if (wp.p) {
-            const int r = threadIdx.x >> 3, c4 = (threadIdx.x & 7) << 2;
-            if (ip0 + r < ld_in && cp0 + c4 < fp)
-                bx_store4(wp, ip0 + r, cp0 + c4, make_float4(tile[r][c4], tile[r][c4 + 1], tile[r][c4 + 2], tile[r][c4 + 3]));
-            if (cp0 + r < fp && ip0 + c4 < ld_in)
-                bx_store4(wtp, cp0 + r, ip0 + c4, make_float4(tile[c4][r], tile[c4 + 1][r], tile[c4 + 2][r], tile[c4 + 3][r]));
-        }
-        __syncthreads();
-    }
-    for (int cp = blockIdx.x * blockDim.x + threadIdx.x; cp < fp; cp += gridDim.x * blockDim.x) {
-        const int k = col_view(vc, cp), f = cp - vc.off[k];
-        const bool ok = f < vc.width[k];
-        colp[CP_GAMMA * fp + cp] = ok ? pp.gamma[k][f] : 0.0f;
-        colp[CP_BETA * fp + cp] = ok ? pp.beta[k][f] : 0.0f;
-        colp[CP_BIAS * fp + cp] = ok ? pp.bias[k][f] : 0.0f;
-        colp[CP_RMEAN * fp + cp] = ok ? pp.run_mean[k][f] : 0.0f;
-        colp[CP_RVAR * fp + cp] = ok ? pp.run_var[k][f] : 1.0f;
-        colp[CP_AVEW * fp + cp] = pp.ave_w ? pp.ave_w[k] : 1.0f;
-    }
-    for (int e = blockIdx.x * blockDim.x + threadIdx.x; e < vc.K * 256; e += gridDim.x * blockDim.x) {
-        const int k = e >> 8, c = e & 255;
-        sig[e] = (c >= 1 && c <= pp.channels[k]) ? sigmoidf_(att_logit(pp, k, c)) : 0.0f;
-    }
-    if (blockIdx.x == 0 && threadIdx.x < vc.K) rsig[threadIdx.x] = sigmoidf_(pp.self_r[threadIdx.x][0]);
-}
 __global__ __launch_bounds__(256) void pack_params_kernel(ParamPtrs pp, ViewCols vc, ColMapD in, int ld_in, int fp,
                                                            float* __restrict__ Wcat, float* __restrict__ WcatT,
                                                            float* __restrict__ colp, float* __restrict__ sig,
                                                            float* __restrict__ rsig, BxOut wp, BxOut wtp) {
-    pack_params_body(pp, vc, in, ld_in, fp, Wcat, WcatT, colp, sig, rsig, wp, wtp);
-}
-struct PackJob {
-    ParamPtrs pp; ViewCols vc; ColMapD in; int ld_in, fp;
-    float *Wcat, *WcatT, *colp, *sig, *rsig;
-    BxOut wp, wtp;
-};
-struct PackJobs { PackJob j0, j1, j2, j3; };
+    pack_params_body((int)blockIdx.x, (int)gridDim.x, pp, vc, in, ld_in, fp, Wcat, WcatT, colp, sig, rsig, wp, wtp);
+}
 __global__ __launch_bounds__(256) void pack_params_multi_kernel(PackJobs jobs, ZeroJob zj, HandOff ho) {
     if (blockIdx.y == 0) {
         for (int i = blockIdx.x * blockDim.x + threadIdx.x; i < max(zj.nu, zj.nd); i += gridDim.x * blockDim.x) {
@@ -131,10 +20,7 @@
             if (i < zj.nd) zj.d[i] = 0.0;
         }
     }
-    if (blockIdx.y == 0) pack_params_body(jobs.j0.pp, jobs.j0.vc, jobs.j0.in, jobs.j0.ld_in, jobs.j0.fp, jobs.j0.Wcat, jobs.j0.WcatT, jobs.j0.colp, jobs.j0.sig, jobs.j0.rsig, jobs.j0.wp, jobs.j0.wtp);
-    else if (blockIdx.y == 1) pack_params_body(jobs.j1.pp, jobs.j1.vc, jobs.j1.in, jobs.j1.ld_in, jobs.j1.fp, jobs.j1.Wcat, jobs.j1.WcatT, jobs.j1.colp, jobs.j1.sig, jobs.j1.rsig, jobs.j1.wp, jobs.j1.wtp);
-    else if (blockIdx.y == 2) pack_params_body(jobs.j2.pp, jobs.j2.vc, jobs.j2.in, jobs.j2.ld_in, jobs.j2.fp, jobs.j2.Wcat, jobs.j2.WcatT, jobs.j2.colp, jobs.j2.sig, jobs.j2.rsig, jobs.j2.wp, jobs.j2.wtp);
-    else pack_params_body(jobs.j3.pp, jobs.j3.vc, jobs.j3.in, jobs.j3.ld_in, jobs.j3.fp, jobs.j3.Wcat, jobs.j3.WcatT, jobs.j3.colp, jobs.j3.sig, jobs.j3.rsig, jobs.j3.wp, jobs.j3.wtp);
+    EAGCN_PACK_JOBS(jobs, (int)blockIdx.y, (int)blockIdx.x, (int)gridDim.x);
     if (blockIdx.x == 0 && blockIdx.y == 0 && threadIdx.x == 0) handoff_body(ho);
 }
 
@@ -337,7 +223,8 @@
     double* slab_da;
     int do_drop; uint32_t thr; float inv_keep; uint64_t seed; const uint64_t* seed_dev;
     double* zero; int nzero;
-    EdgeDrain drain;
+    int gxb;
+    PendingGrads pend;
     const float* cc;
     int store_dh;
 };
@@ -348,30 +235,14 @@
     const uint64_t seed = DROP ? (a.seed_dev ? *a.seed_dev : a.seed) : 0ull;
     const int fp = a.fp, T = min(a.meta[EAGCN_META_T], a.Tcap);
     const int rows = T + (APPLY ? 0 : a.nvirt);
-    const int nwg = max(1, min((int)gridDim.x, (rows + BWD_ROWS - 1) / BWD_ROWS));
-    if (!APPLY && a.drain.eacc && blockIdx.x == 0 && blockIdx.y == 0) {
-        const int K = a.drain.K;
-        for (int e = threadIdx.x; e < K * EDGE_SLAB; e += blockDim.x) {
-            const int k = e / EDGE_SLAB, c = e - k * EDGE_SLAB;
-            if (c > 256) continue;
-            double v[EDGE_COPIES];
-#pragma unroll
-            for (int z = 0; z < EDGE_COPIES; ++z) v[z] = a.drain.eacc[((size_t)z * K + k) * EDGE_SLAB + c];
-            double t = 0.0;
-#pragma unroll
-            for (int z = 0; z < EDGE_COPIES; ++z) { t += v[z]; a.drain.eacc[((size_t)z * K + k) * EDGE_SLAB + c] = 0.0; }
-            float* dw = nullptr;
-            float* dr = nullptr;
-            int ch = 0;
-#pragma unroll
-            for (int q = 0; q < EAGCN_MAX_VIEWS; ++q)
-                if (q == k) { dw = a.drain.datt_w[q]; dr = a.drain.dself_r[q]; ch = a.drain.channels[q]; }
-            if (c == 256) {
-                const double r = (double)a.drain.rsig[k];
-                dr[0] = (float)(t * r * (1.0 - r));
-            } else if (c >= 1 && c <= ch) {
-                dw[c - 1] = (float)t;
-            }
+    const int nwg = max(1, min(APPLY ? (int)gridDim.x : a.gxb, (rows + BWD_ROWS - 1) / BWD_ROWS));
+    if constexpr (!APPLY) {
+        if ((int)blockIdx.x >= a.gxb) {
+            if (blockIdx.y == 0 && a.pend.eacc)
+                unpack_grads_body((int)blockIdx.x - a.gxb, a.pend.gp, a.pend.pp, a.pend.vc, a.pend.in, a.pend.ld_in, a.pend.fp, a.pend.dWcat,
+                                  a.pend.nsplit, a.pend.wslab, a.pend.eacc, a.pend.nedge, a.pend.rsig, a.pend.wblocks, a.meta, a.pend.xk_G,
+                                  a.pend.edge_drain, a.pend.bx_per, a.pend.bx_wide);
+            return;
         }
     }
     if ((int)blockIdx.x >= nwg || (APPLY && T == 0)) return;
@@ -504,7 +375,7 @@
         }
         __syncthreads();
         if (threadIdx.x < EAGCN_MAX_VIEWS)
-            a.slab_da[((size_t)blockIdx.y * gridDim.x + blockIdx.x) * EAGCN_MAX_VIEWS + threadIdx.x] = da_s[threadIdx.x];
+            a.slab_da[((size_t)blockIdx.y * a.gxb + blockIdx.x) * EAGCN_MAX_VIEWS + threadIdx.x] = da_s[threadIdx.x];
     }
 }
 
@@ -576,100 +447,7 @@
                                                             int nsplit, size_t slab, double* __restrict__ datt,
                                                             int nedge, const float* __restrict__ rsig, int wblocks,
                                                             const int32_t* __restrict__ meta, int xk_G, int edge_drain, int bx_per, int bx_wide) {
-    nedge = nedge < 0 ? -nedge : min(nedge, (meta[EAGCN_META_T] + 15) / 16);
-    const int bxm = bx_wide ? BX3W_BM : BX3_BM, bxn = bx_wide ? BX3W_BN : BX3_BN;
-    nsplit = nsplit < 0 ? bx3_used_splits_wave(-nsplit, meta[EAGCN_META_T], ((ld_in + bxm - 1) / bxm) * ((fp + bxn - 1) / bxn),
-                                          bx_per > 0 ? ((meta[EAGCN_META_T] + bxm - 1) / bxm) * ((ld_in + bxn - 1) / bxn) : 0, max(1, (fp + 31) >> 5), bx_per)
-                        : max(1, min(nsplit, meta[EAGCN_META_T] >> 7));
-    if ((int)blockIdx.x < wblocks) {
-        const int tid = blockIdx.x * blockDim.x + threadIdx.x;
-        if (xk_G > 0) {
-            const int e = tid;
-            if (e >= ld_in * fp) return;
-            const int ip = e / fp, cp = e % fp;
-            const int k = col_view(vc, cp), f = cp - vc.off[k];
-            const int fi = packed_to_exact(in, ip);
-            if (fi < 0 || f >= vc.width[k]) return;
-            const int T = meta[EAGCN_META_T];
-            G3Plan pl;
-            g3_plan((T + 63) / 64, (ld_in + 63) / 64, max(1, (fp + 15) / 16), ((ld_in + 63) / 64) * ((fp + 63) / 64),
-                    max(1, (T + 15) / 16), xk_G, pl);
-            float v[G3_XSEG];
-#pragma unroll
-            for (int x = 0; x < G3_XSEG; ++x) v[x] = pl.c[x + 1] > pl.c[x] ? dWcat[(size_t)x * slab + e] : 0.0f;
-            float t = 0.0f;
-#pragma unroll
-            for (int x = 0; x < G3_XSEG; ++x) t += v[x];
-            gp.dW[k][(size_t)fi * vc.width[k] + f] = T > 0 ? t : 0.0f;
-            return;
-        }
-        const int sub = tid & 3;
-        const int e = (tid >> 2) * 4;
-        if (e >= ld_in * fp) return;
-        const int ip = e / fp, cp = e % fp;
-        const int k = col_view(vc, cp), f = cp - vc.off[k];
-        const int fi = packed_to_exact(in, ip);
-        if (fi < 0 || f >= vc.width[k]) return;
-        float4 s0 = make_float4(0.f, 0.f, 0.f, 0.f), s1 = s0;
-        int z = sub;
-#pragma unroll 4
-        for (; z + 4 < nsplit; z += 8) {
-            const float4 a0 = *reinterpret_cast<const float4*>(dWcat + (size_t)z * slab + e);
-            const float4 a1 = *reinterpret_cast<const float4*>(dWcat + (size_t)(z + 4) * slab + e);
-            s0.x += a0.x; s0.y += a0.y; s0.z += a0.z; s0.w += a0.w;
-            s1.x += a1.x; s1.y += a1.y; s1.z += a1.z; s1.w += a1.w;
-        }
-        if (z < nsplit) {
-            const float4 a0 = *reinterpret_cast<const float4*>(dWcat + (size_t)z * slab + e);
-            s0.x += a0.x; s0.y += a0.y; s0.z += a0.z; s0.w += a0.w;
-        }
-        float t[4] = {s0.x + s1.x, s0.y + s1.y, s0.z + s1.z, s0.w + s1.w};
-#pragma unroll
-        for (int j = 0; j < 4; ++j) { t[j] += __shfl_xor(t[j], 1); t[j] += __shfl_xor(t[j], 2); }
-        const float tv = sub == 0 ? t[0] : sub == 1 ? t[1] : sub == 2 ? t[2] : t[3];
-        if (f + sub < vc.width[k]) gp.dW[k][(size_t)fi * vc.width[k] + f + sub] = tv;
-        return;
-    }
-    const int er = ((int)blockIdx.x - wblocks) * 16 + (threadIdx.x >> 4), sl = threadIdx.x & 15;
-    const int tot = vc.K * EDGE_SLAB;
-    const int e = min(er, tot - 1);
-    const int k = e / EDGE_SLAB, c = e % EDGE_SLAB;
-    const bool general = pp.rel_vec[k] != nullptr && c != 256;
-    double t = 0.0;
-    if (!general) {
-        for (int z0 = sl; z0 < nedge; z0 += 16 * 8) {
-            double v[8];
-#pragma unroll
-            for (int u = 0; u < 8; ++u) {
-                const int z = z0 + 16 * u;
-                v[u] = z < nedge ? datt[(size_t)z * tot + e] : 0.0;
-            }
-#pragma unroll
-            for (int u = 0; u < 8; ++u) t += v[u];
-            if (edge_drain && er < tot) {
-#pragma unroll
-                for (int u = 0; u < 8; ++u) {
-                    const int z = z0 + 16 * u;
-                    if (z < nedge) datt[(size_t)z * tot + e] = 0.0;
-                }
-            }
-        }
-    } else if (c >= 1 && c <= pp.rel_c[k]) {
-        const float* vec = pp.rel_vec[k];
-        const int C = pp.rel_c[k], D = pp.channels[k];
-        for (int z = sl; z < nedge; z += 16)
-            for (int code = 1; code <= D; ++code)
-                t += datt[(size_t)z * tot + k * EDGE_SLAB + code] * (double)vec[(size_t)(code - 1) * C + (c - 1)];
-    }
-#pragma unroll
-    for (int o = 8; o > 0; o >>= 1) t += __shfl_xor(t, o);
-    if (er >= tot || sl != 0) return;
-    if (c == 256) {
-        const double r = (double)rsig[k];
-        gp.dself_r[k][0] = (float)(t * r * (1.0 - r));
-    } else if (c >= 1 && c <= (pp.rel_vec[k] ? pp.rel_c[k] : pp.channels[k])) {
-        gp.datt_w[k][c - 1] = (float)t;
-    }
+    unpack_grads_body((int)blockIdx.x, gp, pp, vc, in, ld_in, fp, dWcat, nsplit, slab, datt, nedge, rsig, wblocks, meta, xk_G, edge_drain, bx_per, bx_wide);
 }
 
 __global__ __launch_bounds__(256) void attention_dense_kernel(eagcn_batch bt, ParamPtrs pp, float* __restrict__ out) {
@@ -730,6 +508,10 @@
     return d;
 }
 
+size_t layer_dw_slab_floats(const eagcn_batch* b, const eagcn_layer_params* p) {
+    const LayerDims d = layer_dims(b, p);
+    return d.wslab * std::max(std::max(d.nsplit, G3_XSEG), d.np ? d.bx_splits : 1);
+}
 static bool gemm3_layer(int ld_in) {
     static const bool on = [] { const char* v = getenv("EAGCN_NO_GEMM3"); return !(v && v[0] == '1'); }();
     return on && ld_in >= 128 && gemm_mode() != 2;
@@ -842,6 +624,9 @@
     return pp;
 }
 
+static int g_ride_along = [] { const char* v = getenv("EAGCN_RIDE_ALONG"); return v ? (atoi(v) & 3) : 3; }();
+int ride_along_mode() { return g_ride_along; }
+
 static inline int ew_grid(size_t n) { return (int)std::max<size_t>(1, std::min<size_t>((n + 255) / 256, 2048)); }
 
 }
@@ -852,6 +637,11 @@
 
 using namespace eagcn;
 
+extern "C" int eagcn_set_ride_along(int mode) {
+    const int old = eagcn::g_ride_along;
+    eagcn::g_ride_along = mode & 3;
+    return old;
+}
 extern "C" int eagcn_pad16(int w) { return pad16(w); }
 extern "C" int eagcn_layer_fp(const eagcn_layer_params* p) { return view_cols(p).off[p->K]; }
 extern "C" int eagcn_layer_out_ld(const eagcn_layer_params* p) {
@@ -878,6 +668,27 @@
         if (rc) return rc;
     }
     return layer_forward_impl(b, p, w, stream, false);
+}
+
+static int make_pack_job(const eagcn_batch* b, const eagcn_layer_params* p, void* packed, size_t packed_bytes, int l, PackJob* j,
+                         size_t* wslab, int* tiles) {
+    int rc = check_layer(b, p, "eagcn_model_forward");
+    if (rc) return rc;
+    const LayerDims d = layer_dims(b, p);
+    Packed pk;
+    const size_t pneed = carve_packed(packed, d, &pk);
+    if (pneed > packed_bytes) {
+        set_error("pack_params_all: packed buffer of layer %d too small (%zu < %zu)", l, packed_bytes, pneed);
+        return EAGCN_ERR_SCRATCH;
+    }
+    j->pp = param_ptrs(b, p); j->vc = d.vc; j->in = make_colmap(&p->in);
+    j->ld_in = d.ld_in; j->fp = d.fp;
+    j->Wcat = pk.Wcat; j->WcatT = pk.WcatT; j->colp = pk.colp; j->sig = pk.sig; j->rsig = pk.rsig;
+    j->wp = BxOut{d.np ? pk.Wp : nullptr, d.wpslab, d.np, d.ld_in};
+    j->wtp = BxOut{d.np ? pk.WTp : nullptr, d.wtpslab, d.np, d.fp};
+    if (wslab) *wslab = d.wslab;
+    if (tiles) *tiles = cdiv(d.ld_in, 32) * cdiv(d.fp, 32);
+    return EAGCN_OK;
 }
 
 int eagcn::pack_params_all(const eagcn_batch* b, const eagcn_layer_params* const* ps, void* const* packed,
@@ -888,21 +699,10 @@
     size_t wmax = 0;
     for (int l = 0; l < 4; ++l) {
         const int ll = l < n ? l : n - 1;
-        int rc = check_layer(b, ps[ll], "eagcn_model_forward");
+        size_t wslab = 0;
+        int rc = make_pack_job(b, ps[ll], packed[ll], packed_bytes[ll], ll, &jobs[l], &wslab, nullptr);
         if (rc) return rc;
-        const LayerDims d = layer_dims(b, ps[ll]);
-        Packed pk;
-        const size_t pneed = carve_packed(packed[ll], d, &pk);
-        if (pneed > packed_bytes[ll]) {
-            set_error("pack_params_all: packed buffer of layer %d too small (%zu < %zu)", ll, packed_bytes[ll], pneed);
-            return EAGCN_ERR_SCRATCH;
-        }
-        jobs[l].pp = param_ptrs(b, ps[ll]); jobs[l].vc = d.vc; jobs[l].in = make_colmap(&ps[ll]->in);
-        jobs[l].ld_in = d.ld_in; jobs[l].fp = d.fp;
-        jobs[l].Wcat = pk.Wcat; jobs[l].WcatT = pk.WcatT; jobs[l].colp = pk.colp; jobs[l].sig = pk.sig; jobs[l].rsig = pk.rsig;
-        jobs[l].wp = BxOut{d.np ? pk.Wp : nullptr, d.wpslab, d.np, d.ld_in};
-        jobs[l].wtp = BxOut{d.np ? pk.WTp : nullptr, d.wtpslab, d.np, d.fp};
-        if (l < n) wmax = std::max(wmax, d.wslab);
+        if (l < n) wmax = std::max(wmax, wslab);
     }
     PackJobs pj{jobs[0], jobs[1], jobs[2], jobs[3]};
     ProfScope ps_(PROF_PACK, s);
@@ -913,8 +713,39 @@
     return EAGCN_OK;
 }
 
+int eagcn::pack_ride_jobs(const eagcn_batch* b, const eagcn_layer_params* const* ps, void* const* packed, const size_t* packed_bytes,
+                          int lo, int n, PackRide* out) {
+    EAGCN_CHECK_ARG(out && lo >= 1 && n > lo && n - lo <= 4, "pack_ride_jobs: layers %d..%d", lo, n - 1);
+    PackJob jobs[4];
+    int per = 8;
+    for (int i = 0; i < 4; ++i) {
+        const int ll = lo + i < n ? lo + i : n - 1;
+        int tiles = 0;
+        int rc = make_pack_job(b, ps[ll], packed[ll], packed_bytes[ll], ll, &jobs[i], nullptr, &tiles);
+        if (rc) return rc;
+        if (lo + i < n) per = std::max(per, tiles);
+    }
+    out->jobs = PackJobs{jobs[0], jobs[1], jobs[2], jobs[3]};
+    out->n = n - lo;
+    out->per = std::min(per, 2048);
+    return EAGCN_OK;
+}
+
+static GemmDesc fwd_plain_desc(const eagcn_batch* b, const LayerDims& d, const float* x, const float* Wcat, float* P, double work) {
+    GemmDesc g{0, 0, b->T, d.fp, d.ld_in, x, d.ld_in, Wcat, d.fp, P, d.fp, 1, 0, work};
+    g.M_dev = b->meta + EAGCN_META_T;
+    return g;
+}
+bool eagcn::layer_fwd_carries_pack(const eagcn_batch* b, const eagcn_layer_params* p, const float* x) {
+    if (!b || !p || !x || b->T <= 0) return false;
+    const LayerDims d = layer_dims(b, p);
+    if (d.np || gemm3_layer(d.ld_in)) return false;
+    return gemm_pack_ok(fwd_plain_desc(b, d, x, reinterpret_cast<const float*>(static_cast<uintptr_t>(4096)),
+                                       reinterpret_cast<float*>(static_cast<uintptr_t>(4096)), 0.0));
+}
+
 int eagcn::layer_forward_impl(const eagcn_batch* b, const eagcn_layer_params* p, const eagcn_layer_bufs* w,
-                              void* stream, bool prepacked, bool skip_apply, bool planes_only) {
+                              void* stream, bool prepacked, bool skip_apply, bool planes_only, const PackRide* ride) {
     hipStream_t s = (hipStream_t)stream;
     int rc = check_layer(b, p, "eagcn_layer_forward");
     if (rc) return rc;
@@ -977,11 +808,15 @@
         } else if (gemm3_layer(d.ld_in) && gemm3_ok(g3)) {
             rc = launch_gemm3(g3, nullptr, sc.gws, gemm3_workspace_bytes(), s);
         } else {
-            GemmDesc g{0, 0, b->T, d.fp, d.ld_in, w->x, d.ld_in, sc.Wcat, d.fp, w->P, d.fp, 1, 0, gemm_work};
-            g.M_dev = b->meta + EAGCN_META_T;
-            rc = launch_gemm(g, s);
+            const GemmDesc g = fwd_plain_desc(b, d, w->x, sc.Wcat, w->P, gemm_work);
+            if (ride) { rc = launch_gemm_pack(g, *ride, s); ride = nullptr; }
+            else rc = launch_gemm(g, s);
         }
         if (rc) return rc;
+        if (ride) {
+            set_error("eagcn_layer_forward: the product that was to carry the packing of the layers above took another kernel");
+            return EAGCN_ERR_ARG;
+        }
         {
             AggArgs a;
             a.bt = *b; a.vc = d.vc; a.src = w->P; a.lds = d.fp; a.dst = w->Y; a.ldd = d.fp;
@@ -1103,7 +938,7 @@
 int eagcn::layer_backward_impl(const eagcn_batch* b, const eagcn_layer_params* p, const eagcn_layer_bufs* w,
                                const float* dxout, const ReadoutGrad* rg, const float* dpad_row, float* dx,
                                const eagcn_layer_grads* g, void* stream, bool dpad_views, const ZeroJob* zero_after,
-                               const EdgeDrain* drain_in, EdgeDrain* drain_out, bool input_only) {
+                               const PendingGrads* drain_in, PendingGrads* drain_out, bool input_only, float* dw_down) {
     if (drain_out) drain_out->eacc = nullptr;
     hipStream_t s = (hipStream_t)stream;
     int rc = check_layer(b, p, "eagcn_layer_backward");
@@ -1176,11 +1011,12 @@
     ba.seed_dev = p->seed_dev;
     ba.zero = zero_after ? zero_after->d : nullptr;
     ba.nzero = zero_after ? zero_after->nd : 0;
-    if (drain_in && drain_in->eacc) ba.drain = *drain_in; else memset(&ba.drain, 0, sizeof(ba.drain));
+    if (drain_in && drain_in->eacc) ba.pend = *drain_in; else memset(&ba.pend, 0, sizeof(ba.pend));
     const int rows = b->T + ba.nvirt;
     const int gxb = std::max(1, std::min(rows, d.gxb));
     bool fused_bn_apply = false, fused_w_apply = false, w_rows = false, fused_c_apply = false;
     bool lagg_bwd = false;
+    bool hand_ok = false, hand_w = false;
     {
         static const bool edge_atomic0 = [] { const char* v = getenv("EAGCN_EDGE_SLABS"); return !(v && v[0] == '1'); }();
         bool general0 = false;
@@ -1189,7 +1025,11 @@
         const bool absorbs = lagg_fuses_bn() && (!bn_bwd_two_pass(wt0) || (wt0 && lagg_wfuse()));
         lagg_bwd = b->T > 0 && edge_atomic0 && !general0 && lagg_use(b, 1, absorbs);
         if (input_only) lagg_bwd = b->T > 0 && lagg_use(b, 1, true);
-    }
+        static const bool defer_env = [] { const char* v = getenv("EAGCN_NO_EDGE_DEFER"); return !(v && v[0] == '1'); }();
+        hand_ok = defer_env && drain_out && !input_only && !w->aux_stream && w->packed && b->T > 0 && edge_atomic0 && !general0;
+        hand_w = hand_ok && (ride_along_mode() & 1) && dw_down && w->packed && !w->stats_hook;
+    }
+    float* const dWc = hand_w ? dw_down : sc.dWcat;
     const double M = (double)b->B * (double)b->N;
     const bool eval_in = input_only && !p->training;
     if (eval_in) {
@@ -1215,7 +1055,8 @@
         {
             const bool wt = p->structure == EAGCN_STRUCT_WEIGHTED, dr = ba.do_drop != 0;
             bool dg = ba.rg.dg != nullptr;
-            const dim3 grid(gxb, ny);
+            const dim3 grid(gxb + (ba.pend.eacc ? pending_blocks(ba.pend) : 0), ny);
+            ba.gxb = gxb;
             ba.cc = sc.cc;
             ba.store_dh = bn_bwd_two_pass(wt) ? 0 : 1;
             static const bool rows_first = [] { const char* v = getenv("EAGCN_W_ROWS_FIRST"); return !(v && v[0] == '0'); }();
@@ -1280,7 +1121,7 @@
             bx.A = BxPlanes{sc.dPp, pstride, d.fp, b->T}; bx.B = BxPlanes{sc.Wp, d.wpslab, d.fp, d.ld_in}; bx.C = dx; bx.ldc = d.ld_in;
             bx.M = b->T; bx.N = d.ld_in; bx.K = d.fp; bx.M_dev = b->meta + EAGCN_META_T; bx.tn = 0; bx.splits = 1;
             bw.A = BxPlanes{w->x_planes ? w->x_planes : sc.xp, xstride, d.ld_in, b->T}; bw.B = BxPlanes{sc.dPp, pstride, d.fp, b->T};
-            bw.C = sc.dWcat; bw.ldc = d.fp; bw.M = d.ld_in; bw.N = d.fp; bw.K = b->T; bw.K_dev = b->meta + EAGCN_META_T; bw.tn = 1;
+            bw.C = dWc; bw.ldc = d.fp; bw.M = d.ld_in; bw.N = d.fp; bw.K = b->T; bw.K_dev = b->meta + EAGCN_META_T; bw.tn = 1;
             bw.splits = d.bx_splits; bw.slab = d.wslab;
             use_bx = bx3_ok(bw) && (!dx || bx3_ok(bx));
         }
@@ -1347,7 +1188,7 @@
         }
         if (forked) { rc = stream_after(side, s); if (rc) return rc; }
         nsplit = d.nsplit;
-        GemmDesc gw{1, 0, d.ld_in, d.fp, b->T, w->x, d.ld_in, sc.dP, d.fp, sc.dWcat, d.fp, nsplit, d.wslab, gemm_work};
+        GemmDesc gw{1, 0, d.ld_in, d.fp, b->T, w->x, d.ld_in, sc.dP, d.fp, dWc, d.fp, nsplit, d.wslab, gemm_work};
         gw.K_dev = b->meta + EAGCN_META_T;
         GemmDesc gx{0, 1, b->T, d.ld_in, d.fp, sc.dP, d.fp, sc.Wcat, d.fp, dx, d.ld_in, 1, 0, gemm_work};
         gx.M_dev = b->meta + EAGCN_META_T;
@@ -1391,16 +1232,15 @@
         const int wblocks = nsplit > 0 ? cdiv((int)d.wslab, 256) : 0;
         double* edge_src = nedge == -EDGE_COPIES ? sc.eacc : sc.datt;
         const int edge_drain = edge_src == sc.eacc ? 1 : 0;
-        static const bool defer_env = [] { const char* v = getenv("EAGCN_NO_EDGE_DEFER"); return !(v && v[0] == '1'); }();
-        if (defer_env && drain_out && edge_drain && wblocks == 0 && !forked && b->T > 0) {
-            drain_out->eacc = sc.eacc; drain_out->K = p->K; drain_out->rsig = sc.rsig;
-            for (int k = 0; k < EAGCN_MAX_VIEWS; ++k) {
-                drain_out->datt_w[k] = gp.datt_w[k]; drain_out->dself_r[k] = gp.dself_r[k]; drain_out->channels[k] = pp.channels[k];
-            }
+        if (hand_ok && edge_drain && !forked && (wblocks == 0 || hand_w)) {
+            PendingGrads& pg = *drain_out;
+            pg.eacc = sc.eacc; pg.gp = gp; pg.pp = pp; pg.vc = d.vc; pg.in = in; pg.ld_in = d.ld_in; pg.fp = d.fp;
+            pg.dWcat = dWc; pg.nsplit = bx_slabs ? -nsplit : nsplit; pg.wslab = d.wslab; pg.nedge = nedge; pg.rsig = sc.rsig;
+            pg.wblocks = wblocks; pg.xk_G = xk_G; pg.edge_drain = edge_drain; pg.bx_per = bx_per; pg.bx_wide = bx_wide;
             return EAGCN_OK;
         }
         ProfScope psu(PROF_PACK, side);
-        unpack_grads_kernel<<<wblocks + cdiv(p->K * EDGE_SLAB, 16), 256, 0, side>>>(gp, pp, d.vc, in, d.ld_in, d.fp, sc.dWcat,
+        unpack_grads_kernel<<<wblocks + cdiv(p->K * EDGE_SLAB, 16), 256, 0, side>>>(gp, pp, d.vc, in, d.ld_in, d.fp, dWc,
                                                                                     bx_slabs ? -nsplit : nsplit, d.wslab, edge_src, nedge, sc.rsig,
                                                                                     wblocks, b->meta, xk_G, edge_drain, bx_per, bx_wide);
         EAGCN_LAUNCH_CHECK();
diff --git a/include/eagcn_hip.h b/include/eagcn_hip.h
--- a/include/eagcn_hip.h
+++ b/include/eagcn_hip.h
@@ -323,6 +323,7 @@
 int eagcn_bx3_split(const float* x, int rows, int ld, uint16_t* planes, size_t plane_stride, int rows_cap, int np, void* stream);
 int eagcn_bx3_used_splits(int splits, int M, int N, int K);
 int eagcn_set_bx3_wide(int mode);
+int eagcn_set_ride_along(int mode);
 int eagcn_bx3_pair_used_splits(int splits, int M, int N, int K, int M0, int N0, int K0);
 int eagcn_gemm_bx3(int tn, int M, int N, int K, const uint16_t* A, size_t a_pstride, int lda, int a_rows, const uint16_t* B,
                    size_t b_pstride, int ldb, int b_rows, float* C, int ldc, int splits, size_t slab, int np, void* stream);
```
